# MrOlm/inStrain

Hardware: AMD Instinct MI355X
Metric: Gbp profiled/s (higher is better)
Workload: dtype u32

## Files before the change

### include/instrain_amd.h

```cpp
#ifndef INSTRAIN_AMD_H
#define INSTRAIN_AMD_H

#include <stdint.h>

#ifdef __cplusplus
extern "C" {
#endif

#define ISX_OK 0
#define ISX_ERR_ARG (-1)
#define ISX_ERR_HIP (-2)
#define ISX_ERR_CAPACITY (-3)
#define ISX_ERR_MM_RANGE (-4)
#define ISX_ERR_IO (-5)
#define ISX_ERR_STATE (-6)

#define ISX_ABI_VERSION 5


typedef struct isx_ctx isx_ctx;
typedef struct isx_batch isx_batch;
typedef struct isx_bam isx_bam;
struct isx_bam_params_s;
struct isx_bam_info_s;

typedef struct {
    uint32_t gpos;
    uint16_t mm;
    uint8_t base;
    uint8_t flags;
} isx_obs;

typedef struct {
    int32_t min_cov;
    int32_t min_snp;
    double min_freq;
    int32_t rarefied_coverage;
    int32_t n_mm_bins;
    int32_t enable_linkage;
    int32_t linkage_mode;
    int32_t window;
    uint64_t seed;
    int32_t layout;
    int32_t reserved;
} isx_params;

#define ISX_LAYOUT_WIDE_RECORDS 1
#define ISX_LAYOUT_NO_SHORT_RECORDS 2
#define ISX_LAYOUT_NO_PACKED_COUNTERS 4
#define ISX_LAYOUT_SEG64_RECORDS 8

#define ISX_LAYOUT_MM_ENTRIES 16

#define ISX_LAYOUT_MM_DELTA_RECORDS 32

#define ISX_LAYOUT_NO_STRIPES 64

typedef struct {
    uint32_t gpos;
    uint16_t mm;
    uint16_t flags;
    uint32_t cnt[4];
    float clon;
    float clon_rarefied;
} isx_entry;

typedef struct {
    uint32_t gpos;
    uint16_t mm;
    uint8_t con_base, var_base;
    uint8_t allele_count;
    uint8_t cls;
    uint8_t cryptic;
    uint8_t ref_base;
    uint32_t cnt[4];
} isx_snv;

typedef struct {
    uint32_t gpos_a, gpos_b;
    uint16_t mm;
    uint8_t allele_A, allele_a, allele_B, allele_b;
    uint16_t pad;
    uint32_t total, countAB, countAb, countaB, countab;
    uint32_t pad2;
    double r2, d_prime;
    double r2_normalized, d_prime_normalized;
} isx_ld;

typedef struct {
// ... 205 lines not shown
    const void *lev_mask;
    const void *lev_cov;
    const uint32_t *lev_win_off;
    const isx_rare *lev_clon, *lev_rare;
    const isx_sat *lev_sat;
    int64_t n_lev, n_lev_clon, n_lev_rare, n_lev_sat;
    int32_t lev_mask_bytes, lev_cov_bytes, lev_window, n_lev_windows, lev_min_cov, pad_lev;
    uint64_t rows_checksum;
} isx_pipe_result;

int isx_levels_expand(const isx_pipe_result *r, int32_t host_threads, uint32_t *gpos, uint32_t *mm_cov, float *clon, float *clon_rarefied);

int isx_pipe_create(isx_ctx *ctx, const isx_params *params, const isx_pipe_params *pp, isx_pipe **out);
void isx_pipe_destroy(isx_pipe *p);
int isx_pipe_submit(isx_pipe *p, int64_t n_pos, const uint8_t *ref, int32_t n_splits, const int64_t *split_bounds,
                    int64_t n_obs, const isx_obs *obs, const uint32_t *pair, int64_t *ticket);
int isx_pipe_submit_bam(isx_pipe *p, isx_bam *bam, const struct isx_bam_params_s *bp, const int32_t *refs, int32_t n_refs,
                        const uint8_t *ref, int32_t n_splits, const int64_t *split_bounds, struct isx_bam_info_s *info,
                        int64_t *ticket);
int isx_pipe_collect(isx_pipe *p, int64_t ticket, isx_pipe_result *out);
int isx_pipe_release(isx_pipe *p, int64_t ticket);
int isx_pipe_fetch_entries(isx_pipe *p, int64_t ticket, isx_entry *out);
int isx_pipe_fetch_entries_shrunk(isx_pipe *p, int64_t ticket, uint32_t *gpos, uint32_t *mm_cov, float *clon, float *clon_rarefied);


#define ISX_SEG_BASES 150
#define ISX_SEG_WORDS 15
#define ISX_SEG_SKIP_WORD 0x24924924u
#define ISX_DREC_WORDS 8
#define ISX_DREC_EXC 6
#define ISX_DREC_EXC_FULL 3
#define ISX_DREC_DUAL 0x80000000u
#define ISX_DREC_NO_EXC 0x3FFFFFFFu

typedef struct {
    int64_t n_seg;
    const uint32_t *gpos;
    const uint8_t *len;
    const uint8_t *mm;
    const uint32_t *pair;
    const uint32_t *bases;
} isx_segs;

int isx_batch_create_reads(isx_ctx *ctx, const isx_params *params, int64_t n_pos, const uint8_t *ref, int32_t n_splits,
                           const int64_t *split_bounds, const isx_segs *segs, isx_batch **out);
int isx_pipe_submit_reads(isx_pipe *p, int64_t n_pos, const uint8_t *ref, int32_t n_splits, const int64_t *split_bounds,
                          const isx_segs *segs, int64_t *ticket);

typedef struct isx_wire isx_wire;
int isx_pipe_stage_reads(isx_pipe *p, int64_t n_pos, const uint8_t *ref, int32_t n_splits, const int64_t *split_bounds,
                         const isx_segs *segs, isx_wire **out);
int isx_pipe_submit_wire(isx_pipe *p, const isx_wire *wire, int64_t *ticket);
int64_t isx_wire_bytes(const isx_wire *wire);
void isx_wire_free(isx_wire *wire);
int isx_wire_keep_reference(isx_pipe *p, isx_wire *wire);

#define ISX_PLANE_WORDS 8
typedef struct {
    int64_t n_seg;
    const uint32_t *gpos;
    const uint8_t *len;
    const uint32_t *pair;
    const uint64_t *planes;
    const uint8_t *mm;
} isx_read_planes;

typedef struct {
    const uint8_t *plane2;
    const uint8_t *nplane;
    uint64_t key;
} isx_ref_planes;

int isx_pack_ref_planes(const uint8_t *ref, int64_t n_pos, int32_t host_threads, uint8_t *plane2, uint8_t *nplane, int32_t *has_n);
int isx_planes_from_segs(const isx_segs *segs, int32_t host_threads, uint64_t *planes);
int isx_pack_read_planes(int64_t n_reads, const int64_t *ref_start, const int64_t *clip_lo, const int64_t *clip_hi,
                         const uint32_t *cigar, const int64_t *cigar_off, const char *seq, const uint8_t *qual, const int64_t *seq_off,
                         const uint32_t *pair, int32_t min_base_quality, int64_t cap_seg, uint32_t *seg_gpos,
                         uint8_t *seg_len, uint32_t *seg_pair, uint64_t *seg_planes, int64_t *n_seg);
int isx_pipe_submit_planes(isx_pipe *p, int64_t n_pos, const isx_ref_planes *ref, int32_t n_splits, const int64_t *split_bounds,
                           const isx_read_planes *reads, int64_t *ticket);
int isx_pipe_stage_planes(isx_pipe *p, int64_t n_pos, const isx_ref_planes *ref, int32_t n_splits, const int64_t *split_bounds,
                          const isx_read_planes *reads, isx_wire **out);
int isx_pipe_set_reference_budget(isx_pipe *p, int64_t mib);
int isx_host_register(const void *ptr, int64_t bytes);
int isx_host_unregister(const void *ptr);
int isx_encode_planes(const isx_read_planes *reads, const isx_ref_planes *ref, int64_t n_pos, int32_t host_threads, int32_t slack_groups,
                      int64_t cap_rec, int64_t ring_records, uint32_t *rec, uint32_t *gbase, int64_t *n_rec, int64_t *need_slack);
int isx_encode_planes_mm(const isx_read_planes *reads, const isx_ref_planes *ref, int64_t n_pos, int32_t n_mm_bins, int32_t host_threads, int32_t slack_groups,
                         int64_t cap_rec, int64_t ring_records, uint32_t *rec, uint32_t *gbase, int64_t *n_rec, int64_t *need_slack);

int isx_count_read_segs(int64_t n_reads, const uint32_t *cigar, const int64_t *cigar_off, const int64_t *ref_start,
                        const int64_t *clip_lo, const int64_t *clip_hi, int64_t *n_seg);
int isx_pack_reads(int64_t n_reads, const int64_t *ref_start, const int64_t *clip_lo, const int64_t *clip_hi,
                   const uint32_t *cigar, const int64_t *cigar_off, const char *seq, const uint8_t *qual, const int64_t *seq_off,
                   const uint8_t *mm, const uint32_t *pair, int32_t min_base_quality, int64_t cap_seg, uint32_t *seg_gpos,
                   uint8_t *seg_len, uint8_t *seg_mm, uint32_t *seg_pair, uint32_t *seg_bases, int64_t *n_seg);

int isx_encode_segs(const isx_segs *segs, int64_t n_pos, int32_t n_mm_bins, int32_t host_threads, int64_t cap_rec, uint32_t *rec,
                    uint32_t *gbase, uint32_t *pair_out, int64_t *n_rec);
int64_t isx_seg_records_needed(const uint32_t *gpos, int64_t n_seg, int32_t host_threads);
int isx_encode_segs_ring(const isx_segs *segs, int64_t n_pos, int32_t n_mm_bins, int32_t host_threads, int64_t cap_rec, int64_t ring_records,
                         uint32_t *rec, uint32_t *gbase, uint32_t *pair_out, int64_t *n_rec);

int isx_encode_delta(const isx_segs *segs, const uint8_t *ref, int64_t n_pos, int32_t n_mm_bins, int32_t host_threads, int32_t slack_groups,
                     int64_t cap_rec, int64_t ring_records, uint32_t *rec, uint32_t *gbase, uint32_t *pair_out, int64_t *n_rec, int64_t *need_slack);
int64_t isx_delta_records_needed(const uint32_t *gpos, int64_t n_seg, int32_t host_threads, int32_t slack_groups);

int isx_encode_obs(const isx_obs *obs, const uint32_t *pair, int64_t n_obs, int64_t n_pos, int32_t record_bytes,
                   int32_t host_threads, double slack, int64_t cap_rec, void *rec, uint32_t *gbase, uint32_t *pair_out,
                   int64_t *n_rec, int32_t *passes);
int isx_encode_obs_ring(const isx_obs *obs, const uint32_t *pair, int64_t n_obs, int64_t n_pos, int32_t record_bytes,
                        int32_t host_threads, double slack, int64_t cap_rec, int64_t ring_records, void *rec,
                        uint32_t *gbase, uint32_t *pair_out, int64_t *n_rec, int32_t *passes);

typedef struct {
    int64_t in_off;
    int32_t in_len;
    int32_t out_len;
    int64_t out_off;
} isx_bgzf_block;
int isx_bgzf_index(const uint8_t *image, int64_t n_bytes, int64_t cap_blocks, isx_bgzf_block *blocks, int64_t *n_blocks, int64_t *out_bytes);
int isx_bgzf_inflate_device(isx_ctx *ctx, const uint8_t *image, int64_t n_bytes, const isx_bgzf_block *blocks, int64_t n_blocks,
// ... 68 lines not shown
```

### instrain_amd/_lib.py

```python
import ctypes as C
import os

import numpy as np

_HERE = os.path.dirname(os.path.abspath(__file__))
LIB_PATH = os.path.join(_HERE, "libinstrain_amd.so")
if os.environ.get("ISX_LIB"):
    LIB_PATH = os.path.abspath(os.environ["ISX_LIB"])

BGZF_BLOCK_DT = np.dtype([("in_off", np.int64), ("in_len", np.int32), ("out_len", np.int32), ("out_off", np.int64)])
OBS_DT = np.dtype([("gpos", "<u4"), ("mm", "<u2"), ("base", "u1"), ("flags", "u1")])
ENTRY_DT = np.dtype([("gpos", "<u4"), ("mm", "<u2"), ("flags", "<u2"), ("cnt", "<u4", (4,)), ("clon", "<f4"),
                     ("clon_rarefied", "<f4")])
SNV_DT = np.dtype([("gpos", "<u4"), ("mm", "<u2"), ("con_base", "u1"), ("var_base", "u1"),
                   ("allele_count", "u1"), ("cls", "u1"), ("cryptic", "u1"), ("ref_base", "u1"),
                   ("cnt", "<u4", (4,))])
LD_DT = np.dtype([("gpos_a", "<u4"), ("gpos_b", "<u4"), ("mm", "<u2"), ("allele_A", "u1"), ("allele_a", "u1"),
                  ("allele_B", "u1"), ("allele_b", "u1"), ("pad", "<u2"), ("total", "<u4"), ("countAB", "<u4"),
                  ("countAb", "<u4"), ("countaB", "<u4"), ("countab", "<u4"), ("pad2", "<u4"),
                  ("r2", "<f8"), ("d_prime", "<f8"), ("r2_normalized", "<f8"), ("d_prime_normalized", "<f8")])
AO_DT = np.dtype([("pair", "<u4"), ("gpos", "<u4"), ("order", "<u4"), ("mm", "<u2"), ("base", "u1"), ("pad", "u1")])
assert AO_DT.itemsize == 16
assert OBS_DT.itemsize == 8 and ENTRY_DT.itemsize == 32 and SNV_DT.itemsize == 28 and LD_DT.itemsize == 72


class Params(C.Structure):
    _fields_ = [("min_cov", C.c_int32), ("min_snp", C.c_int32), ("min_freq", C.c_double),
                ("rarefied_coverage", C.c_int32), ("n_mm_bins", C.c_int32), ("enable_linkage", C.c_int32),
                ("linkage_mode", C.c_int32), ("window", C.c_int32), ("seed", C.c_uint64), ("layout", C.c_int32),
                ("reserved", C.c_int32)]


LAYOUT_WIDE_RECORDS, LAYOUT_NO_SHORT_RECORDS, LAYOUT_NO_PACKED_COUNTERS, LAYOUT_SEG64_RECORDS = 1, 2, 4, 8


class PipeParams(C.Structure):
    _fields_ = [("max_pos", C.c_int64), ("max_obs", C.c_int64), ("max_splits", C.c_int32), ("depth", C.c_int32),
                ("host_threads", C.c_int32), ("pin_threads", C.c_int32), ("jump_slack", C.c_double),
                ("want_counts", C.c_int32), ("ring_kib", C.c_int32), ("stage_async", C.c_int32), ("lean_output", C.c_int32),
                ("max_segs", C.c_int64)]


SEG_BASES, SEG_WORDS, SEG_SKIP_WORD = 150, 15, 0x24924924


class Segs(C.Structure):
    _fields_ = [("n_seg", C.c_int64), ("gpos", C.c_void_p), ("len", C.c_void_p), ("mm", C.c_void_p), ("pair", C.c_void_p),
                ("bases", C.c_void_p)]


PLANE_WORDS = 8
LAYOUT_MM_ENTRIES = 16
LAYOUT_MM_DELTA_RECORDS = 32
ABI_VERSION = 5


class ReadPlanes(C.Structure):
    _fields_ = [("n_seg", C.c_int64), ("gpos", C.c_void_p), ("len", C.c_void_p), ("pair", C.c_void_p), ("planes", C.c_void_p), ("mm", C.c_void_p)]


class RefPlanes(C.Structure):
    _fields_ = [("plane2", C.c_void_p), ("nplane", C.c_void_p), ("key", C.c_uint64)]


RARE_DT = np.dtype([("gpos", "<u4"), ("clon_rarefied", "<f4")])
CLON_DT = np.dtype([("gpos", "<u4"), ("clon", "<f4")])
SAT_DT = np.dtype([("gpos", "<u4"), ("coverage", "<u4")])


class Sizes(C.Structure):
    _fields_ = [(n, C.c_int64) for n in ("n_entries", "n_snv", "n_sites", "n_allele_obs", "n_increments",
                                         "n_edges", "n_ld")]


class Timings(C.Structure):
    _fields_ = [(n, C.c_float) for n in ("pileup_ms", "sites_ms", "allele_ms", "group_ms", "incr_ms", "ld_ms",
                                         "total_ms")] + \
               [(n, C.c_int32) for n in ("pileup_blocks", "pileup_threads", "pileup_lds_bytes", "pileup_window")] + \
               [("mfma_ms", C.c_float), ("dense_tiles", C.c_int32), ("dense_macs", C.c_int64), ("dense_bytes", C.c_int64),
                ("record_bytes", C.c_int32), ("pad", C.c_int32)]


class PipeResult(C.Structure):
    _fields_ = [("ticket", C.c_int64), ("n_pos", C.c_int64), ("n_obs", C.c_int64), ("sizes", Sizes),
                ("coverage16", C.c_void_p), ("clon", C.c_void_p), ("rare", C.c_void_p), ("n_rare", C.c_int64),
                ("n_saturated", C.c_int64), ("counts", C.c_void_p), ("clon_rarefied", C.c_void_p), ("snv", C.c_void_p),
# ... 39 lines not shown
COMPARE_LEVEL_DT = np.dtype([("both", "<i8"), ("either", "<i8"), ("mm", "<i4"), ("present_a", "<i4"),
                             ("present_b", "<i4"), ("pad", "<i4"), ("consensus_snps", "<i8"), ("population_snps", "<i8")])
assert COMPARE_LEVEL_DT.itemsize == 48
COMPARE_SNP_DT = np.dtype([("gpos", "<u4"), ("mm", "<u2"), ("consensus_snp", "u1"), ("population_snp", "u1"),
                           ("has_a", "u1"), ("has_b", "u1"), ("con_a", "u1"), ("ref_a", "u1"), ("var_a", "u1"),
                           ("con_b", "u1"), ("ref_b", "u1"), ("var_b", "u1"), ("cnt_a", "<u4", (4,)), ("cnt_b", "<u4", (4,))])
assert COMPARE_SNP_DT.itemsize == 48


GENE_DT = np.dtype([("start", "<i8"), ("end", "<i8"), ("seq_off", "<i8"), ("strand", "<i4"), ("pad", "<i4")])
GENE_COV_DT = np.dtype([("sum_cov", "<u8"), ("nonzero", "<u4"), ("counted", "<u4"), ("sum_clon", "<f8")])
GENE_SNV_COUNT_DT = np.dtype([(n, "<u4") for n in ("divergent", "sns", "sns_n", "sns_s", "snv", "snv_n", "snv_s")])
GENE_MUTATION_DT = np.dtype([("gene", "<i4"), ("k", "<i4"), ("type", "u1"), ("aa_old", "u1"), ("aa_new", "u1"), ("n_genes", "u1"),
                             ("pad", "<u4")])
assert GENE_DT.itemsize == 32 and GENE_COV_DT.itemsize == 24 and GENE_SNV_COUNT_DT.itemsize == 28 and GENE_MUTATION_DT.itemsize == 16
GENE_LEVEL_PRESENT, GENE_COV_ANY, GENE_CLON_ANY = 1, 2, 4


ERR_CAPACITY = -3


class IsxError(RuntimeError):
    def __init__(self, code, msg):
        super().__init__("libinstrain_amd error %d: %s" % (code, msg))
        self.code = code


SYMBOLS = ["isx_last_error", "isx_abi_version", "isx_ctx_create", "isx_ctx_destroy", "isx_ctx_reserve_cus", "isx_set_null_model",
           "isx_batch_create", "isx_batch_create_reads", "isx_batch_destroy", "isx_batch_run", "isx_batch_launch", "isx_batch_wait", "isx_batch_sizes", "isx_batch_timings",
           "isx_batch_fetch_entries", "isx_batch_fetch_dense", "isx_batch_fetch_snv", "isx_batch_fetch_ld", "isx_batch_fetch_allele_obs",
           "isx_batch_summarize", "isx_batch_summarize_genomes", "isx_compare_coverage", "isx_compare_scaffolds", "isx_compare_fetch_snps",
           "isx_genes_create", "isx_genes_destroy", "isx_genes_sites", "isx_batch_profile_genes", "isx_genes_profile_snvs",
           "isx_pipe_create", "isx_pipe_destroy", "isx_pipe_submit", "isx_pipe_submit_reads", "isx_pipe_stage_reads", "isx_pipe_submit_wire", "isx_wire_bytes", "isx_wire_free", "isx_wire_keep_reference", "isx_pipe_submit_bam", "isx_encode_segs", "isx_encode_segs_ring", "isx_seg_records_needed", "isx_encode_delta", "isx_delta_records_needed", "isx_count_read_segs", "isx_pack_reads", "isx_pipe_collect", "isx_pipe_release", "isx_pipe_fetch_entries", "isx_pipe_fetch_entries_shrunk", "isx_levels_expand", "isx_encode_obs", "isx_encode_obs_ring",
           "isx_pack_ref_planes", "isx_planes_from_segs", "isx_pack_read_planes", "isx_pipe_submit_planes", "isx_pipe_stage_planes", "isx_encode_planes", "isx_encode_planes_mm", "isx_pipe_set_reference_budget", "isx_host_register", "isx_host_unregister",
           "isx_bgzf_index", "isx_bgzf_inflate_device", "isx_bgzf_inflate_host", "isx_bgzf_inflate_fast",
           "isx_bam_open", "isx_bam_close", "isx_bam_close_wait", "isx_bam_set_threads", "isx_bam_ref", "isx_bam_set_priority_reads", "isx_bam_scan", "isx_bam_scan_part",
           "isx_bam_insert_sizes", "isx_bam_set_wanted_refs", "isx_bam_pair_keys", "isx_bam_set_cross_names", "isx_bam_filter_insert_sizes", "isx_bam_filter", "isx_bam_set_r2m", "isx_bam_r2m", "isx_bam_drop_names", "isx_bam_batch_pair_names", "isx_bam_set_mm_cap", "isx_bam_mm_levels", "isx_bam_set_mm_levels", "isx_bam_ref_counts",
           "isx_bam_expand_refs", "isx_bam_segment_refs", "isx_bam_copy_segs", "isx_bam_copy_read_planes", "isx_bam_expand_region", "isx_bam_expand", "isx_bam_copy", "isx_bam_view"]

_lib = None


def load():
    global _lib
    if _lib is not None:
        return _lib
    if not os.path.exists(LIB_PATH):
        raise IsxError(-2, "%s not built: run `python -c 'import __graft_entry__ as g; g.build()'` "
                           "(hipcc --offload-arch=gfx950)" % LIB_PATH)
    lib = C.CDLL(LIB_PATH)
    vp, i32, i64 = C.c_void_p, C.c_int32, C.c_int64
    lib.isx_last_error.restype = C.c_char_p
    lib.isx_abi_version.restype = C.c_int
    if lib.isx_abi_version() != ABI_VERSION:
        raise IsxError(-6, "%s has ABI version %d, this package binds version %d: rebuild it (python -c 'import __graft_entry__ as g; g.build()')"
                       % (LIB_PATH, lib.isx_abi_version(), ABI_VERSION))
    lib.isx_ctx_create.argtypes = [C.c_int, C.POINTER(vp)]
    lib.isx_ctx_destroy.argtypes = [vp]
    lib.isx_ctx_reserve_cus.argtypes = [vp, C.c_int]
    lib.isx_bgzf_index.argtypes = [vp, i64, i64, vp, C.POINTER(i64), C.POINTER(i64)]
    lib.isx_bgzf_inflate_device.argtypes = [vp, vp, i64, vp, i64, vp, i64, C.POINTER(C.c_float)]
    lib.isx_bgzf_inflate_host.argtypes = [vp, i64, vp, i64, vp, i64]
    lib.isx_bgzf_inflate_fast.argtypes = [vp, i64, vp, i64, vp, i64]
    lib.isx_ctx_destroy.restype = None
    lib.isx_set_null_model.argtypes = [vp, vp, i64, i32]
    lib.isx_batch_create.argtypes = [vp, C.POINTER(Params), i64, vp, i32, vp, i64, vp, vp, C.POINTER(vp)]
    lib.isx_batch_create_reads.argtypes = [vp, C.POINTER(Params), i64, vp, i32, vp, C.POINTER(Segs), C.POINTER(vp)]
# ... 56 lines not shown
    lib.isx_bam_set_threads.argtypes = [vp, i32]
    lib.isx_bam_set_priority_reads.argtypes = [vp, i64, C.c_char_p, vp]
    lib.isx_bam_scan.argtypes = [vp, C.POINTER(BamInfo)]
    lib.isx_bam_scan_part.argtypes = [vp, i32, i32, C.POINTER(BamInfo)]
    lib.isx_bam_set_wanted_refs.argtypes = [vp, vp, i32]
    lib.isx_bam_insert_sizes.argtypes = [vp, vp, i64, C.POINTER(i64)]
    lib.isx_bam_filter_insert_sizes.argtypes = [vp, vp, i64, C.POINTER(i64)]
    lib.isx_bam_pair_keys.argtypes = [vp, vp, vp, vp, vp, i64, C.POINTER(i64)]
    lib.isx_bam_set_cross_names.argtypes = [vp, i64, vp, vp, vp]
    lib.isx_bam_filter.argtypes = [vp, C.POINTER(BamParams), C.c_double, C.POINTER(BamInfo)]
    lib.isx_bam_set_r2m.argtypes = [vp, i32, i64, C.c_char_p, vp, vp]
    lib.isx_bam_drop_names.argtypes = [vp]
    lib.isx_bam_r2m.argtypes = [vp, i32, C.POINTER(i64), C.POINTER(i64), vp, vp, vp]
    lib.isx_bam_batch_pair_names.argtypes = [vp, C.POINTER(i64), C.POINTER(i64), vp, vp]
    lib.isx_bam_set_mm_cap.argtypes = [vp, i32]
    lib.isx_bam_mm_levels.argtypes = [vp, vp, i32, vp]
    lib.isx_bam_set_mm_levels.argtypes = [vp, vp, i32]
    lib.isx_bam_ref_counts.argtypes = [vp, vp, vp]
    lib.isx_bam_expand_region.argtypes = [vp, C.POINTER(BamParams), i32, i64, i64, C.POINTER(BamInfo)]
    lib.isx_bam_expand_refs.argtypes = [vp, C.POINTER(BamParams), vp, i32, C.POINTER(BamInfo)]
    lib.isx_bam_segment_refs.argtypes = [vp, C.POINTER(BamParams), vp, i32, C.POINTER(BamInfo), C.POINTER(i64)]
    lib.isx_bam_copy_segs.argtypes = [vp, vp, vp, vp, vp, vp, vp, vp]
    lib.isx_bam_copy_read_planes.argtypes = [vp, vp]
    lib.isx_pack_ref_planes.argtypes = [vp, i64, i32, vp, vp, C.POINTER(i32)]
    lib.isx_planes_from_segs.argtypes = [C.POINTER(Segs), i32, vp]
    lib.isx_pack_read_planes.argtypes = [i64, vp, vp, vp, vp, vp, vp, vp, vp, vp, i32, i64, vp, vp, vp, vp, C.POINTER(i64)]
    lib.isx_pipe_submit_planes.argtypes = [vp, i64, C.POINTER(RefPlanes), i32, vp, C.POINTER(ReadPlanes), C.POINTER(i64)]
    lib.isx_pipe_set_reference_budget.argtypes = [vp, i64]
    lib.isx_host_register.argtypes = [vp, i64]
    lib.isx_host_unregister.argtypes = [vp]
    lib.isx_pipe_stage_planes.argtypes = [vp, i64, C.POINTER(RefPlanes), i32, vp, C.POINTER(ReadPlanes), C.POINTER(vp)]
    lib.isx_encode_planes.argtypes = [C.POINTER(ReadPlanes), C.POINTER(RefPlanes), i64, i32, i32, i64, i64, vp, vp, C.POINTER(i64), C.POINTER(i64)]
    lib.isx_encode_planes_mm.argtypes = [C.POINTER(ReadPlanes), C.POINTER(RefPlanes), i64, i32, i32, i32, i64, i64, vp, vp, C.POINTER(i64), C.POINTER(i64)]
    lib.isx_bam_ref.argtypes = [vp, i32, C.POINTER(C.c_char_p), C.POINTER(i64), C.POINTER(i64)]
    lib.isx_bam_copy.argtypes = [vp, vp, vp, vp, vp]
    lib.isx_bam_view.argtypes = [vp, C.POINTER(vp), C.POINTER(vp)]
    _lib = lib
    return lib


def check(rc):
    if rc != 0:
        raise IsxError(rc, load().isx_last_error().decode(errors="replace"))
```

### instrain_amd/csrc/isx_api.hip

```cpp
#include <algorithm>
#include <atomic>
#include <cmath>
#include <chrono>
#include <cstdlib>
#include <cstring>
#include <map>
#include <mutex>
#include <string>
#include <unordered_map>
#include <thread>
#include <type_traits>
#include <vector>
#include <unistd.h>
#include <sys/prctl.h>
#include <time.h>

#include "isx_batch.h"
#include "seg_encode.h"

static thread_local std::string g_err;
void isx_set_error(const std::string &msg) { g_err = msg; }

namespace {
struct BlockCache {
// ... 1215 lines not shown

    PileupArgs a{};
    a.seg = b->d_seg; a.drec = b->d_drec; a.dlt_off = b->dlt_off;
    a.rec = b->d_rec; a.rec32 = b->d_rec32; a.rec16 = b->d_rec16; a.gbase = b->d_gbase; a.win_range = b->d_win; a.ref = b->d_ref; a.ref_packed = b->ref_packed; a.ref_n = b->d_ref_n;
    a.pair = b->d_pair; a.pair_runs = b->d_pair_runs; a.run_index = b->d_run_index; a.n_runs = b->n_runs; a.gpos = b->d_gpos; a.gpos16 = b->d_gpos16; a.chunk_base = b->d_rec32 ? b->d_gbase : b->d_cbase; a.gpos16_shift = b->gpos16_shift; a.thr = b->d_thr; a.lut_n = c->lut_n; a.fallback = c->fallback; a.qcap = b->qcap; a.rqcap = b->rqcap; a.stage_off = b->stage_off;
    a.n_pos = (uint32_t)b->n_pos; a.W = b->W; a.logW = b->logW; a.M = b->M; a.n_win = b->n_win;
    a.min_cov = b->prm.min_cov; a.min_freq = b->prm.min_freq;
#ifdef ISX_TUNING
    if (const char *e = getenv("ISX_DEBUG_MODE")) a.debug_mode = atoi(e);
#endif
    a.counts = b->d_counts; a.clon = b->d_clon; a.clon_r = b->d_clon_r;
    a.min_cov_r = b->prm.rarefied_coverage;
    a.cov16 = b->d_cov16; a.rare = b->d_rare; a.cap_rare = (uint32_t)std::min<size_t>(b->cap_rare, 0xFFFFFFFFu);
    a.cov8 = b->sparse_out && b->cov8_out ? b->d_cov8 : nullptr;
    a.sat = b->d_sat; a.cap_sat = (uint32_t)std::min<size_t>(b->cap_sat, 0xFFFFFFFFu); a.sat_thr = a.cov8 ? 255u : 65535u;
    b->nib_pass = false;
    if (b->sparse_out && b->nib_out && b->lean && b->drec && b->packed && b->M == 1 && b->d_cov_row_win && b->d_cov8 &&
        (size_t)b->n_win <= b->cap_cov_row_win) {
        b->nib_pass = true;
        a.cov4 = b->d_cov8; a.cov_rows = b->d_cov16; a.cov_row_win = b->d_cov_row_win;
        a.cap_cov_rows = (uint32_t)std::min<uint64_t>((uint64_t)(b->cap_pos ? b->cap_pos : b->n_pos), 0xFFFFFFFFu);
        a.cov8 = nullptr; a.cov16 = nullptr; a.sat_thr = 65535u;
    }
    a.clon_list = b->sparse_out ? b->d_clon_list : nullptr; a.cap_clon = (uint32_t)std::min<size_t>(b->cap_clon, 0xFFFFFFFFu);
    if (b->lean && b->sparse_out) {
        if (!b->clon_dense) a.clon = nullptr;
        if (!b->rare_dense && a.rare) a.clon_r = nullptr;
        if (a.cov8) a.cov16 = nullptr;
    }
#ifdef ISX_TUNING
    if (getenv("ISX_NO_COUNTS")) { a.counts = nullptr; if (atoi(getenv("ISX_NO_COUNTS")) > 1) a.clon = nullptr; }
#endif
    a.stripe = (b->drec && b->packed && b->M == 1 && !a.counts && !(b->prm.layout & ISX_LAYOUT_NO_STRIPES)) ? 1 : 0;
    a.seed_lo = (uint32_t)b->prm.seed; a.seed_hi = (uint32_t)(b->prm.seed >> 32);
    a.entries = b->d_entries; a.slab = b->slab; a.cap_ovf = (uint32_t)b->cap_ovf;
    a.ovf0 = (uint64_t)b->n_win * b->slab; a.win_nent = b->d_win_nent;
    if (b->lev_sparse) {
        a.lev_mask = b->d_lev_mask; a.lev_cov = b->d_lev_cov; a.lev_win_off = b->d_lev_win_off;
        a.lev_mask_bytes = b->lev_mask_bytes; a.lev_cov_bytes = b->lev_cov_bytes;
        a.cap_lev = (uint32_t)std::min<size_t>(b->cap_lev, 0xFFFFFFFEu);
        a.sat_thr = b->lev_cov_bytes == 1 ? 255u : 65535u;
        a.clon_list = b->d_clon_list; a.cap_clon = (uint32_t)std::min<size_t>(b->cap_clon, 0xFFFFFFFFu);
        a.cov16 = nullptr; a.cov8 = nullptr; a.clon = nullptr; a.clon_r = nullptr;
    }
    a.slev = b->d_slev; a.cap_slev = (uint32_t)std::min<size_t>(b->cap_slev, 0xFFFFFFFFu);
    a.snv = b->d_snv; a.cap_snv = (uint32_t)std::min<size_t>(b->cap_snv, 0xFFFFFFFFu);
    a.sites = b->d_sites; a.cap_sites = (uint32_t)std::min<size_t>(b->cap_sites, 0xFFFFFFFFu);
    a.ao = b->d_ao; a.cap_ao = (uint32_t)std::min<size_t>(b->cap_ao, 0xFFFFFFFFu); a.enable_linkage = b->prm.enable_linkage;
    a.cursors = b->d_cursors; a.flags = b->d_flags; a.host_state = b->d_host_state;
    memcpy(a.base, b->base, sizeof(a.base));

    if (c->unpublished[b->ps] && c->unpublished[b->ps] != b) {
        isx_batch *u = c->unpublished[b->ps];
        a.pub_cursors = u->d_cursors; a.pub_host_state = u->d_host_state; a.pub_epoch = u->epoch;
        u->publish_enqueued = true;
        c->unpublished[b->ps] = nullptr;
    }
    b->ordered = false;
    if (b->M == 1) {
        auto grow = [&](auto **p, size_t *cap, size_t want, size_t elem) -> hipError_t {
            if (*cap >= want && *p) return hipSuccess;
            if (*p) isx_dev_free(*p);
            *p = nullptr; *cap = 0;
            const hipError_t e = isx_dev_malloc(reinterpret_cast<void **>(p), std::max<size_t>(want, 1) * elem);
            if (e == hipSuccess) *cap = want;
            return e;
// ... 519 lines not shown
```

### instrain_amd/csrc/isx_batch.h

```cpp
#pragma once
#include <vector>

#include "isx_internal.h"
#include "isx_linkage.h"
#include "isx_summary.h"

namespace isxenc { class HostPool; }

struct isx_ctx {
    int device = 0;
    hipStream_t stream = nullptr;
    hipStream_t pstream[2] = {nullptr, nullptr};
    uint32_t side_mask[8] = {0, 0, 0, 0, 0, 0, 0, 0};
    int pass_cus = 256;
    struct isx_batch *unpublished[2] = {nullptr, nullptr};
    unsigned n_created = 0;
    unsigned n_pipes = 0;
    uint8_t *d_lut = nullptr;
    std::vector<int32_t> h_lut;
    int32_t lut_n = 0, fallback = 0;
    void *pin[2] = {nullptr, nullptr};
    hipEvent_t pin_ev[2] = {nullptr, nullptr};
    size_t pin_bytes = 0;
};

hipError_t isx_side_stream_create(isx_ctx *c, hipStream_t *s);

struct isx_batch {
    isx_ctx *ctx = nullptr;
    isx_params prm{};
    int64_t n_pos = 0, n_obs = 0;
    int64_t cap_pos = 0, cap_obs = 0;
    size_t slab_region = 0;
    bool arena = false;
    bool segs = false;
    bool drec = false;
    uint64_t n_rec = 0;
    uint64_t n_pairs = 0;
    int32_t n_splits = 0;
    int W = 0, logW = 0, M = 1, n_win = 0, block = 1024, grid = 0, packed = 0;
    size_t lds = 0;
    uint2 *d_rec = nullptr;
    uint32_t *d_rec32 = nullptr, *d_gbase = nullptr;
    uint16_t *d_rec16 = nullptr;
    uint4 *d_seg = nullptr;
    uint4 *d_drec = nullptr;
    int dlt_off = 0;
    uint32_t *d_pair = nullptr, *d_gpos = nullptr, *d_cbase = nullptr;
    uint2 *d_pair_runs = nullptr;
    uint32_t *d_run_index = nullptr;
    uint32_t n_runs = 0;
    uint16_t *d_gpos16 = nullptr;
    int gpos16_shift = 7;
    uint8_t *d_ref = nullptr;
    int ref_packed = 0;
    uint8_t *d_ref_n = nullptr;
    uint2 *d_win = nullptr;
    uint16_t *d_thr = nullptr;
    int qcap = 1024, rqcap = 0, stage_off = 0;
    bool in_flight = false, publish_enqueued = true, tim_pending = false;
    int ps = 0;
    int64_t *d_bounds = nullptr;
    uint4 *d_counts = nullptr;
    float *d_clon = nullptr;
    float *d_clon_r = nullptr;
    uint16_t *d_cov16 = nullptr;
    uint2 *d_rare = nullptr;
    size_t cap_rare = 0;
    uint32_t n_rare = 0, n_sat = 0;
// ... 82 lines not shown
```

### instrain_amd/csrc/isx_internal.h

```cpp
#pragma once
#include <hip/hip_runtime.h>
#include <stdint.h>
#include <string>

#include "../../include/instrain_amd.h"

#define ISX_PAD32 0x0700FFFFu
#define ISX_GROUP16 512
#define ISX_GROUP 256
#define ISX_CHUNK 1024
#define ISX_DENSE_PAD 8
#define ISX_SEG_GROUP 16
#define ISX_SEG_PAD 32
#define ISX_SEG_LM 16
#define ISX_PK16_MAX_W 3264
#define ISX_PAD 2048
#define ISX_SENTINEL 0xFFFFFFFFu
#define ISX_TAIL_BYTES 65536
#define ISX_TAIL_GROUPS 256

void isx_set_error(const std::string &msg);

hipError_t isx_dev_malloc(void **p, size_t bytes);
void isx_dev_free(void *p);
// ... 155 lines not shown
    uint32_t cap_clon;
    uint2 *rare;
    uint32_t cap_rare;
    int32_t min_cov_r;
    uint32_t seed_lo, seed_hi;
    isx_entry *entries;
    uint32_t slab;
    uint32_t cap_ovf;
    uint64_t ovf0;
    uint32_t *win_nent;
    uint32_t *win_site_base, *win_site_cnt;
    isx_slev *slev;
    uint32_t cap_slev;
    isx_snv *snv;
    uint32_t cap_snv;
    isx_site *sites;
    uint32_t cap_sites;
    isx_ao *ao;
    uint32_t cap_ao;
    int32_t enable_linkage;
    uint32_t *win_rec;
    uint32_t *cursors;
    uint32_t *flags;
    uint32_t base[CUR_N];
    uint32_t *host_state;
    const uint32_t *pub_cursors;
    uint32_t *pub_host_state;
    uint32_t pub_epoch;
    void *lev_mask;
    void *lev_cov;
    uint32_t *lev_win_off;
    uint32_t cap_lev;
    int32_t lev_mask_bytes, lev_cov_bytes;
};

void launch_pileup(const PileupArgs &a, int block, size_t lds, int grid, int packed, hipStream_t s, hipEvent_t ev_start,
                   hipEvent_t ev_stop);
void launch_publish_state(const PileupArgs &a, uint32_t epoch, hipStream_t s);
void launch_win_order(const uint32_t *win_rec, uint32_t *win_out, int n_win, int W, const isx_snv *snv_raw, isx_snv *snv, const isx_site *sites_raw,
                      isx_site *sites, const uint2 *clon_raw, uint2 *clon, const uint2 *rare_raw, uint2 *rare, uint32_t *scan_state, uint32_t epoch, hipStream_t s);
void launch_extract_gpos(const uint2 *rec, const uint32_t *rec32, const uint32_t *gbase, uint32_t *gpos, uint16_t *gpos16,
                         const uint32_t *base16, uint32_t base16_records, uint64_t n_rec, hipStream_t s);
size_t pileup_lds_bytes(int W, int M, int qcap, int rqcap, int linkage, int packed, int block, int segs, int *stage_off, int *dlt_off = nullptr);

struct LinkageBuffers;
```

### instrain_amd/csrc/isx_pileup.hip

```cpp
#include <hip/hip_ext.h>
#include "isx_internal.h"

#pragma clang fp contract(off)

namespace {

typedef uint32_t u32x4 __attribute__((ext_vector_type(4)));

#define THR_LDS 1024

enum { S_NQ = 0, S_ROWS, S_SITES, S_ROW_BASE, S_SITE_BASE, S_ROW_RANK, S_NAO, S_AO_BASE, S_ENT_TOT, S_ENT_BASE, S_SLEV, S_SLEV_BASE, S_NRARE, S_RARE_BASE, S_RARE_RANK,
       S_NCLON, S_CLON_BASE, S_CLON_RANK, S_COVX, S_COVX_BASE, S_N = 20 };
#define S_RNG 128

__device__ __forceinline__ uint32_t cur_add(const PileupArgs &a, int which, uint32_t n)
{
    return atomicAdd(&a.cursors[which], n) - a.base[which];
}

__device__ __forceinline__ void flag_or(const PileupArgs &a, uint32_t bit)
{
    if (atomicOr(a.flags, bit) == 0xFFFFFFFFu) a.flags[3] = 1;
}

// ... 391 lines not shown
        }
        return *reinterpret_cast<const uint32_t *>(a.ref + gpos);
    }
    uint32_t r = 0;
    for (int k = 0; k < 4; k++) r |= (gpos + k < a.n_pos ? (uint32_t)ref_at(a, gpos + k) : 4u) << (8 * k);
    return r;
}

__device__ __forceinline__ void ref4_raw(const PileupArgs &a, uint32_t gpos, uint32_t &raw, uint32_t &rawn)
{
    rawn = 0;
    if (gpos + 3u < a.n_pos) {
        if (a.ref_packed == 2) {
            raw = a.ref[gpos >> 2];
            if (a.ref_n) rawn = a.ref_n[gpos >> 3];
        } else if (a.ref_packed) raw = *reinterpret_cast<const uint16_t *>(a.ref + (gpos >> 1));
        else raw = *reinterpret_cast<const uint32_t *>(a.ref + gpos);
    } else raw = ref4_at(a, gpos);
}
__device__ __forceinline__ uint32_t ref4_expand(const PileupArgs &a, uint32_t gpos, uint32_t raw, uint32_t rawn)
{
    if (gpos + 3u >= a.n_pos) return raw;
    if (a.ref_packed == 2) {
        uint32_t r = (raw & 3u) | ((raw & 0xCu) << 6) | ((raw & 0x30u) << 12) | ((raw & 0xC0u) << 18);
        const uint32_t nb = (rawn >> (gpos & 4u)) & 0xFu;
#pragma unroll
        for (int k = 0; k < 4; k++) r = ((nb >> k) & 1u) ? ((r & ~(0xFFu << (8 * k))) | (4u << (8 * k))) : r;
        return r;
    }
    if (a.ref_packed) return (raw & 0xFu) | ((raw & 0xF0u) << 4) | ((raw & 0xF00u) << 8) | ((raw & 0xF000u) << 12);
    return raw;
}

__device__ __forceinline__ void allele_pass_delta(const PileupArgs &a, uint32_t lo16, uint32_t hi16, uint32_t w0, int W,
                                                  const uint8_t *maskl, uint32_t *slabc, uint32_t ao_base, uint32_t *stage,
                                                  int tid, int nthr)
{
    const int lane = tid & 63;
    uint32_t *st = stage + (tid >> 6) * 128;
    uint32_t *sitebits = stage + (nthr >> 6) * 128;
    for (int p = tid; p < W; p += nthr) {
        const uint64_t bal = __ballot(maskl[p] != 0);
        if (lane == 0) { sitebits[p >> 5] = (uint32_t)bal; sitebits[(p >> 5) + 1] = (uint32_t)(bal >> 32); }
    }
    if (tid < 2) sitebits[(W >> 5) + tid] = 0;
    __syncthreads();
    uint32_t nst = 0;
    auto drain = [&]() {
        __builtin_amdgcn_fence(__ATOMIC_ACQ_REL, "wavefront");
        __builtin_amdgcn_wave_barrier();
        if ((uint32_t)lane < nst) {
            const uint32_t half = st[2 * lane], info = st[2 * lane + 1];
            const uint32_t rel = info & 0xFFFFu;
            const uint32_t slot = atomicAdd(&slabc[rel], 1u);
            isx_ao o;
            o.pair = reinterpret_cast<const uint32_t *>(a.drec)[(info >> 20) & 1u ? ((half | 1u) << 2) + 3u : (half << 2) + 1u];
            o.site = w0 + rel; o.obs_idx = half;
            o.mm = (uint16_t)(info >> 24); o.base = (uint8_t)((info >> 16) & 7u); o.pad = 0;
            a.ao[ao_base + slot] = o;
        }
        __builtin_amdgcn_fence(__ATOMIC_ACQ_REL, "wavefront");
        __builtin_amdgcn_wave_barrier();
    };
    const uint32_t odd = (uint32_t)tid & 1u;
    for (uint32_t i0 = lo16; i0 < hi16; i0 += (uint32_t)nthr) {
        const uint32_t i = i0 + (uint32_t)tid;
        if ((uint32_t)__builtin_amdgcn_readfirstlane(i) >= hi16) break;
        const u32x4 v = __builtin_nontemporal_load(reinterpret_cast<const u32x4 *>(a.drec) + i);
        const uint32_t gb = a.gbase[__builtin_amdgcn_readfirstlane(i >> 6)];
// ... 2 lines not shown
        const uint32_t hdr = dual ? v.x : hdr0;
        const uint32_t len = (hdr >> 16) & 0xFFu;
        const uint32_t w3 = pair_first(v.w);
        const uint32_t e_a = dual ? v.z : w3, e_b = dual ? v.w : ISX_DREC_NO_EXC;
        const int32_t s = (int32_t)(gb + (hdr & 0xFFFFu) - w0);
#pragma unroll
        for (int k = 0; k < 5; k++) {
            const uint32_t c0 = 32u * (uint32_t)k;
            const int32_t r = s + (int32_t)c0;
            const uint32_t skw = dual ? 0u : (k == 0 ? v.y : (k == 1 ? v.z : (k == 2 ? v.x : (k == 3 ? v.y : v.z))));
            const bool mine = dual || (odd != 0u) == (k >= 2);
            uint32_t bits = 0;
            if (len > c0 && mine && (uint32_t)(r + 31) < (uint32_t)(W + 31)) {
                const uint32_t ncol = min(len - c0, 32u);
                const int32_t base = r < 0 ? 0 : r;
                const uint32_t wi = (uint32_t)base >> 5;
                const uint64_t b64 = (uint64_t)sitebits[wi] | ((uint64_t)sitebits[wi + 1] << 32);
                bits = (uint32_t)(b64 >> (base & 31)) << (base - r);
                bits &= ~skw & (ncol == 32u ? 0xFFFFFFFFu : (1u << ncol) - 1u);
            }
            while (__ballot(bits != 0)) {
                const bool has = bits != 0;
                const int j = has ? __ffs((int)bits) - 1 : 0;
                bits &= bits - 1u;
                const uint32_t col = c0 + (uint32_t)j;
                const uint32_t rel = has ? (uint32_t)(r + j) : 0u;
                uint32_t code = 8u;
#pragma unroll
                for (int f = 0; f < 3; f++) {
                    const uint32_t x = (e_a >> (10 * f)) & 0x3FFu, y = (e_b >> (10 * f)) & 0x3FFu;
                    if ((x & 0xFFu) == col) code = x >> 8;
                    if ((y & 0xFFu) == col) code = y >> 8;
                }
                if (has && code == 8u) code = ref_at(a, w0 + rel);
                const bool cand = has && code < 4u && ((maskl[rel] >> code) & 1u);
                const uint64_t bal = __ballot(cand);
                if (bal == 0) continue;
                const uint32_t n = (uint32_t)__popcll(bal);
                if (nst + n > 64u) { drain(); nst = 0; }
                if (cand) {
                    const uint32_t at = nst + __builtin_amdgcn_mbcnt_hi((uint32_t)(bal >> 32), __builtin_amdgcn_mbcnt_lo((uint32_t)bal, 0u));
                    st[2 * at] = dual ? i : (i & ~1u);
                    st[2 * at + 1] = rel | (code << 16) | (dual ? 0u : 1u << 20) | (((hdr >> 24) & 0x7Fu) << 24);
                }
                nst += n;
            }
        }
    }
    if (nst) drain();
}

#ifndef ISX_LB_WAVES
#define ISX_LB_WAVES 8
#endif
#ifdef ISX_TUNING
__device__ unsigned long long g_isx_ts[32 * 16];
extern "C" int isx_debug_read_ts(unsigned long long *out) { return (int)hipMemcpyFromSymbol(out, HIP_SYMBOL(g_isx_ts), sizeof(g_isx_ts)); }
#define ISX_TS(k) do { if ((dbg & 4096) && blockIdx.x == 0 && tid == 0 && ts_w < 32) g_isx_ts[ts_w * 16 + (k)] = wall_clock64(); } while (0)
#else
#define ISX_TS(k) do { } while (0)
#endif
template <bool LINKAGE, int FMT, bool PK16 = false>
__global__ void __launch_bounds__(1024, ISX_LB_WAVES) k_pileup_dense(const PileupArgs a_kernarg)
{
    extern __shared__ __attribute__((aligned(16))) uint32_t lds[];
    typedef const __attribute__((address_space(4))) PileupArgs KernArgs;
    KernArgs *kargs = (KernArgs *)__builtin_amdgcn_kernarg_segment_ptr();
#define a (*(const PileupArgs *)kargs)
    int tid = threadIdx.x;
    const int nthr = blockDim.x;
#define ISX_ARGS_FRESH() asm volatile("" : "+s"(kargs), "+v"(tid))
    publish_previous(a, tid);
    const int W = a.W;
    constexpr bool SEGS = FMT == 64;
    constexpr bool DREC = FMT == 32;
    constexpr bool PKL = DREC && PK16;
    constexpr int NR = PKL ? 2 : 4;
    const int S = W + (SEGS ? ISX_SEG_PAD : ISX_DENSE_PAD);
    uint32_t *cnt = lds + (SEGS ? ISX_SEG_LM : 0);
    uint32_t *queue = lds + NR * S;
    uint32_t *scratch = queue + S;
    uint2 *rngl = reinterpret_cast<uint2 *>(scratch + S_N);
    uint16_t *thr_lds = reinterpret_cast<uint16_t *>(scratch + S_N + S_RNG);
    uint32_t *slabc = scratch + S_N + S_RNG + THR_LDS / 2;
    uint8_t *maskl = reinterpret_cast<uint8_t *>(slabc + W);
    uint32_t *dlt = PKL ? queue : lds + a.dlt_off;
    uint32_t *wtot = lds + a.dlt_off + (PKL ? 0 : S);
    uint8_t *refl = reinterpret_cast<uint8_t *>(wtot + 16);
    auto ld4 = [&](int p, uint32_t *c) {
        if (PKL) {
            const uint32_t x = cnt[p], y = cnt[S + p];
            c[0] = x & 0xFFFFu; c[1] = x >> 16; c[2] = y & 0xFFFFu; c[3] = y >> 16;
        } else { c[0] = cnt[p]; c[1] = cnt[S + p]; c[2] = cnt[2 * S + p]; c[3] = cnt[3 * S + p]; }
    };
    constexpr bool linkage = LINKAGE;
    const int grid = gridDim.x, per = grid >> 3;
    const int slot = (blockIdx.x & 7) * per + (blockIdx.x >> 3);
    constexpr bool COMPACT = FMT != 8;
    const u32x4 *rec4 = reinterpret_cast<const u32x4 *>(SEGS ? (const void *)a.seg : (DREC ? (const void *)a.drec : (FMT == 2 ? (const void *)a.rec16 : (FMT == 4 ? (const void *)a.rec32 : (const void *)a.rec))));
    constexpr int RSH = FMT == 2 ? 3 : (FMT == 4 ? 2 : 1);
    const int dbg = a.debug_mode;
    const bool stripe_k = PKL && a.stripe != 0;

    {
        const int n = min(THR_LDS, a.lut_n);
        for (int i = tid; i < n; i += nthr) thr_lds[i] = a.thr[i];
    }

    u32x4 v[4];
    uint32_t gb[4] = {0, 0, 0, 0};
    bool live[4] = {false, false, false, false};
    uint32_t lo = 0, hi = 0;
    const uint32_t lane16 = (uint32_t)tid;
    auto issue_one = [&](int u, uint32_t i0) {
        const uint32_t j = i0 + tid + u * nthr;
        const uint32_t jw = __builtin_amdgcn_readfirstlane(j);
        if (COMPACT) live[u] = jw < hi;
        if (COMPACT ? jw < hi : j < hi) {
            const uint64_t ub = reinterpret_cast<uint64_t>(rec4 + (i0 + (uint32_t)(u * nthr)));
            typedef __attribute__((address_space(1))) const u32x4 gvec;
            const gvec *sb = reinterpret_cast<const gvec *>(((uint64_t)(uint32_t)__builtin_amdgcn_readfirstlane((uint32_t)(ub >> 32)) << 32) |
// ... 20 lines not shown

#ifdef ISX_TUNING
    int ts_w = -1;
#endif
    for (int w = slot; w < a.n_win; w += grid) {
        const uint32_t w0 = (uint32_t)w * (uint32_t)W;
        const uint32_t cur_lo = lo, cur_hi = hi;
        const bool stripe = stripe_k && (cur_hi - cur_lo) * 8u <= (uint32_t)W;
#ifdef ISX_TUNING
        ++ts_w;
#endif
        ISX_TS(0);
        ISX_ARGS_FRESH();
        if ((win_it & 63) == 0 && tid < 64) {
            const int wn = w + (tid + 1) * grid;
            rngl[tid] = wn < a.n_win ? a.win_range[wn] : make_uint2(0, 0);
        }
        const uint32_t dummy = 4u * (uint32_t)S + (uint32_t)(tid & 63);
#ifdef ISX_TUNING
        uint32_t ablate_acc = 0;
#endif
        {
            uint4 *z = reinterpret_cast<uint4 *>(cnt);
            const int nz = ((NR + (DREC ? 1 : 0)) * S) >> 2;
            for (int i = tid; i < nz; i += nthr) z[i] = make_uint4(0, 0, 0, 0);
            if (DREC && !PKL) {
                uint4 *zd = reinterpret_cast<uint4 *>(dlt);
                for (int i = tid; i < (S >> 2); i += nthr) zd[i] = make_uint4(0, 0, 0, 0);
            }
            if (linkage) {
                uint4 *zm = reinterpret_cast<uint4 *>(maskl);
                for (int i = tid; i < (W >> 4); i += nthr) zm[i] = make_uint4(0, 0, 0, 0);
            }
            if (tid < S_N) scratch[tid] = 0;
        }
        uint32_t ref4 = 0x04040404u, ref4b = 0x04040404u;
        uint32_t ref4n = 0, ref4bn = 0;
        if (PKL) {
            if (4 * tid < W) ref4_raw(a, w0 + 4u * (uint32_t)tid, ref4, ref4n);
            if (4 * (tid + nthr) < W) ref4_raw(a, w0 + 4u * (uint32_t)(tid + nthr), ref4b, ref4bn);
        } else if (DREC && 4 * tid < W) ref4 = ref4_at(a, w0 + 4u * (uint32_t)tid);
        uint8_t ref_raw[2];
#pragma unroll
        for (int it = 0; it < 2; it++) {
            const uint32_t gp = w0 + tid + it * nthr;
            ref_raw[it] = (!PKL && tid + it * nthr < W && gp < a.n_pos) ? ref_at(a, gp) : (uint8_t)4;
        }
        __syncthreads();
        ISX_TS(1);
        ISX_ARGS_FRESH();

        auto count_slot = [&](int u) {
            if (COMPACT && !live[u]) return;
            if (DREC) {
                const uint32_t odd = (uint32_t)tid & 1u;
                const uint32_t hdr0 = pair_first(v[u].x);
                const bool dual = (hdr0 >> 31) != 0u;
                const uint32_t hdr = dual ? v[u].x : hdr0;
                const uint32_t len = (hdr >> 16) & 0xFFu;
                const int32_t s = (int32_t)(gb[u] + (hdr & 0xFFFFu) - w0);
                const uint32_t uW = (uint32_t)W;
#ifdef ISX_TUNING
                if (dbg & 64) { ablate_acc += v[u].x ^ v[u].y ^ v[u].z ^ v[u].w ^ hdr; return; }
#endif
                if ((dual || !odd) && len) {
                    const int32_t hi_c = s + (int32_t)len;
                    if (hi_c > 0 && s < W) {
                        atomicAdd(&dlt[s < 0 ? 0 : s], PKL ? 0x00010000u : 1u);
                        if (hi_c < W) atomicAdd(&dlt[hi_c], PKL ? 0xFFFF0000u : 0xFFFFFFFFu);
                    }
                }
                uint32_t sk[3] = {odd ? v[u].x : v[u].y, odd ? v[u].y : v[u].z, odd ? v[u].z : 0u};
                if (dual) sk[0] = sk[1] = sk[2] = 0;
#ifdef ISX_TUNING
                if (dbg & 8) sk[0] = sk[1] = sk[2] = 0;
#endif
                const int32_t c0 = s + (odd ? 64 : 0);
#pragma unroll
                for (int k = 0; k < 3; k++) {
                    const int32_t r = c0 + 32 * k;
                    uint32_t bits = skip_bits_in_window(sk[k], r, uW);
                    while (__ballot(bits != 0)) {
                        if (bits != 0) atomicAdd(&queue[r + (int32_t)__builtin_ctz(bits)], 1u);
                        bits &= bits - 1u;
                    }
                }
                const uint32_t exw[2] = {dual ? v[u].z : (odd ? ISX_DREC_NO_EXC : v[u].w), dual ? v[u].w : ISX_DREC_NO_EXC};
                const int nf = __ballot(exw[1] != ISX_DREC_NO_EXC) ? 6 : 3;
#pragma unroll
                for (int f = 0; f < 6; f++) {
                    if (f == 3 && nf == 3) break;
                    const uint32_t ex = exw[f / 3];
                    const uint32_t off = (ex >> (10 * (f % 3))) & 0xFFu, code = (ex >> (10 * (f % 3) + 8)) & 3u;
                    const uint32_t rel = (uint32_t)(s + (int32_t)off);
                    if (off < len && rel < uW) {
                        if (PKL) atomicAdd(&cnt[__umul24(code >> 1, (uint32_t)S) + rel], 1u << (16 * (code & 1u)));
                        else atomicAdd(&cnt[__umul24(code, (uint32_t)S) + rel], 1u);
                    }
                }
                return;
            }
            if (SEGS) {
                const uint32_t q = (uint32_t)tid & 3u;
                const uint32_t hdr = quad_first(v[u].x);
                const int32_t r0 = (int32_t)(gb[u] + (hdr & 0xFFFFu) - w0) + (int32_t)(q * 40u) - 10;
                const uint32_t wd[4] = {q ? v[u].x : SEG_SKIPW, v[u].y, v[u].z, v[u].w};
                char *lds_b = reinterpret_cast<char *>(lds);
                const uint32_t S4 = (uint32_t)S * 4u;
#ifdef ISX_TUNING
                if (dbg & 64) { ablate_acc += wd[0] ^ wd[1] ^ wd[2] ^ wd[3] ^ hdr; return; }
#endif
#pragma unroll
                for (int k = 0; k < 4; k++) {
                    const int32_t r = r0 + 10 * k;
                    uint32_t w = wd[k];
                    if (w == SEG_SKIPW || (uint32_t)(r + 9) >= (uint32_t)(W + 9)) continue;
                    const uint32_t m = w & SEG_SKIPW;
                    w &= ~((m >> 1) | (m >> 2));
                    const uint32_t a0 = (uint32_t)(r + ISX_SEG_LM) << 2;
#pragma unroll
                    for (int j = 0; j < 10; j++) {
                        const uint32_t code = __builtin_amdgcn_ubfe(w, 3 * j, 3);
#ifdef ISX_TUNING
                        if (dbg & 8) { ablate_acc += __umul24(code, S4) + a0 + 4u * (uint32_t)j; continue; }
                        if (dbg & 16) { atomicAdd(reinterpret_cast<uint32_t *>(lds_b + ((dummy + (code & 0u)) << 2)), 1u); continue; }
#endif
                        atomicAdd(reinterpret_cast<uint32_t *>(lds_b + (__umul24(code, S4) + a0 + 4u * (uint32_t)j)), 1u);
                    }
                }
                return;
// ... 42 lines not shown
                    atomicAdd(&cnt[(r < (uint32_t)W && bb < 4) ? __umul24(bb, (uint32_t)S) + r : dummy], 1u);
                }
            } else if (FMT == 4) {
                const uint32_t bw = gb[u] - w0;
                const uint32_t x[4] = {v[u].x, v[u].y, v[u].z, v[u].w};
#pragma unroll
                for (int h = 0; h < 4; h++) {
                    const uint32_t r = (x[h] & 0xFFFFu) + bw, bb = __builtin_amdgcn_ubfe(x[h], 24, 3);
                    atomicAdd(&cnt[(r < (uint32_t)W && bb < 4) ? __umul24(bb, (uint32_t)S) + r : dummy], 1u);
                }
            } else {
                const uint32_t g0 = v[u].x, a0 = v[u].y, g1 = v[u].z, a1 = v[u].w;
                const uint32_t r0 = g0 - w0, r1 = g1 - w0;
                const uint32_t b0 = (a0 >> 16) & 0xFFu, b1 = (a1 >> 16) & 0xFFu;
                if (r0 < (uint32_t)W && b0 < 4) atomicAdd(&cnt[b0 * S + r0], 1u);
                if (r1 < (uint32_t)W && b1 < 4) atomicAdd(&cnt[b1 * S + r1], 1u);
            }
        };
        if (DREC) {
            for (uint32_t i0 = lo; i0 < hi; i0 += 2 * nthr) {
                count_slot(0); count_slot(1);
                if (i0 + 2 * nthr < hi) { issue_one(0, i0 + 2 * nthr); issue_one(1, i0 + 2 * nthr); }
            }
        } else
        for (uint32_t i0 = lo; i0 < hi; i0 += 4 * nthr) {
            issue_one(2, i0); issue_one(3, i0);
            count_slot(0); count_slot(1);
            if (i0 + 4 * nthr < hi) { issue_one(0, i0 + 4 * nthr); issue_one(1, i0 + 4 * nthr); }
            count_slot(2); count_slot(3);
        }
#ifdef ISX_TUNING
        if (ablate_acc == 0xDEADBEEFu) cnt[dummy] = ablate_acc;
#endif
        if (PKL) {
            if (4 * tid < W) reinterpret_cast<uint32_t *>(refl)[tid] = ref4_expand(a, w0 + 4u * (uint32_t)tid, ref4, ref4n);
            if (4 * (tid + nthr) < W) reinterpret_cast<uint32_t *>(refl)[tid + nthr] = ref4_expand(a, w0 + 4u * (uint32_t)(tid + nthr), ref4b, ref4bn);
        }
        __syncthreads();
        ISX_TS(2);
        ISX_ARGS_FRESH();

        if (!linkage) { rng_next = rngl[win_it & 63]; prefetch_window(w + grid); }

        if (PKL && !stripe && !(dbg & 16)) {
            const int lane = tid & 63;
            const int PT = ((W + nthr - 1) / nthr) | 1, p0 = tid * PT;
            int32_t sum = 0;
            for (int k = 0; k < PT; k++) if (p0 + k < W) sum += (int32_t)dlt[p0 + k] >> 16;
            const int32_t inc = (int32_t)wave_scan_incl((uint32_t)sum);
            if (lane == 63) wtot[tid >> 6] = (uint32_t)inc;
            __syncthreads();
            ISX_TS(3);
            int32_t run = inc - sum;
            for (int k = 0; k < (tid >> 6); k++) run += (int32_t)wtot[k];
            bool beyond15 = false;
            for (int k = 0; k < PT; k++) {
                const int p = p0 + k;
                if (p >= W) break;
                const uint32_t x = dlt[p], a01 = cnt[p], a23 = cnt[S + p];
                run += (int32_t)x >> 16;
                beyond15 |= run - (int32_t)(x & 0xFFFFu) > 15;
                const uint32_t r = refl[p];
                if (r < 4u) {
                    const uint32_t v = (uint32_t)run - (x & 0xFFFFu) - ((a01 & 0xFFFFu) + (a01 >> 16) + (a23 & 0xFFFFu) + (a23 >> 16));
                    cnt[(r >> 1) * S + p] = ((r >> 1) ? a23 : a01) + (v << (16 * (r & 1u)));
                }
            }
            if (a.cov4 && __ballot(beyond15) && lane == 0) scratch[S_COVX] = 1u;
            __syncthreads();
            ISX_TS(4);
            ISX_ARGS_FRESH();
// ... 385 lines not shown
            const uint32_t e = q < nit ? queue[fl ? (uint32_t)flist[q] : q] : 0u;
            if (!((e >> 14) & 1u)) continue;
            const uint32_t my_row = atomicAdd(&scratch[S_ROW_RANK], 1u);
            const int p = (int)(e & 0x1FFFu);
            const uint32_t gpos = w0 + p;
            uint32_t c[4];
            ld4(p, c);
            const uint32_t total = c[0] + c[1] + c[2] + c[3];
            const int ref_base = PKL ? (int)refl[p] : (int)ref_at(a, gpos);
            const SiteCall sc = call_level(a, nullptr, c, total, ref_base, true);
            isx_snv r;
            r.gpos = gpos; r.mm = 0;
            r.con_base = (uint8_t)sc.snp; r.var_base = (uint8_t)sc.var;
            r.allele_count = (uint8_t)sc.morphia; r.cls = (uint8_t)sc.cls;
            r.cryptic = 0;
            r.ref_base = (uint8_t)ref_base;
            r.cnt[0] = c[0]; r.cnt[1] = c[1]; r.cnt[2] = c[2]; r.cnt[3] = c[3];
            a.snv[row_base + my_row] = r;
            const uint32_t ss = e >> 17;
            if (ss) {
                isx_site st;
                st.gpos = gpos; st.entry_off = row_base + my_row; st.n_levels = 1;
                st.mask = (uint8_t)((1u << sc.snp) | (1u << sc.var)); st.pad = 0;
                a.sites[site_base + ss - 1] = st;
            }
        }
        }
        ISX_TS(8);
        ISX_ARGS_FRESH();
        if (linkage) {
            if (ok && nao) {
                __syncthreads();
                if (SEGS) allele_pass_segs(a, cur_lo, cur_hi, w0, W, maskl, slabc, ao_base, lds + a.stage_off, tid, nthr);
                else if (DREC) allele_pass_delta(a, cur_lo, cur_hi, w0, W, maskl, slabc, ao_base, lds + a.stage_off, tid, nthr);
                else allele_pass(a, cur_lo << (RSH - 1), cur_hi << (RSH - 1), w0, W, maskl, slabc, ao_base, lds + a.stage_off, tid, nthr);
            }
            ISX_TS(9);
            rng_next = rngl[win_it & 63];
            prefetch_window(w + grid);
        }
        win_it++;
        __syncthreads();
        ISX_TS(10);
    }
}
#undef a
#undef ISX_ARGS_FRESH

template <bool PACKED, bool LINKAGE, bool COMPACT, bool SEGS = false, bool SPARSE = false, bool DREC = false>
__global__ void __launch_bounds__(1024) k_pileup_mm(const PileupArgs a_kernarg)
{
    extern __shared__ __attribute__((aligned(16))) uint32_t lds[];
    typedef const __attribute__((address_space(4))) PileupArgs KernArgs;
    KernArgs *kargs = (KernArgs *)__builtin_amdgcn_kernarg_segment_ptr();
#define a (*(const PileupArgs *)kargs)
    int tid = threadIdx.x;
    const int nthr = blockDim.x;
#define ISX_ARGS_FRESH() asm volatile("" : "+s"(kargs), "+v"(tid))
    publish_previous(a, tid);
    const int W = a.W, M = a.M;
#ifdef ISX_TUNING
    int ts_w = -1;
#endif
    const int n_cnt = M * (PACKED ? 2 : 4) * W + (DREC ? M * (PACKED ? 1 : 2) * W : 0);
    const int pres_words = (M + 31) >> 5;
    uint32_t *cnt = lds;
    uint32_t *aux = lds + M * (PACKED ? 2 : 4) * W;
// ... 755 lines not shown
        case 4: launch_one(k_pileup_mm<true, false, true, true, false, true>, a, l); break;
        case 5: launch_one(k_pileup_mm<true, true, true, true, false, true>, a, l); break;
        case 6: launch_one(k_pileup_mm<true, false, true, true, true, true>, a, l); break;
        default: launch_one(k_pileup_mm<true, true, true, true, true, true>, a, l); break;
        }
    } else if (a.M > 1 && a.seg && a.lev_cov) {
        switch (sel & 5) {
        case 0: launch_one(k_pileup_mm<false, false, true, true, true>, a, l); break;
        case 1: launch_one(k_pileup_mm<false, true, true, true, true>, a, l); break;
        case 4: launch_one(k_pileup_mm<true, false, true, true, true>, a, l); break;
        default: launch_one(k_pileup_mm<true, true, true, true, true>, a, l); break;
        }
    } else if (a.M > 1 && a.seg) {
        switch (sel & 5) {
        case 0: launch_one(k_pileup_mm<false, false, true, true>, a, l); break;
        case 1: launch_one(k_pileup_mm<false, true, true, true>, a, l); break;
        case 4: launch_one(k_pileup_mm<true, false, true, true>, a, l); break;
        default: launch_one(k_pileup_mm<true, true, true, true>, a, l); break;
        }
    } else if (a.M > 1) {
        switch (sel) {
        case 0: launch_one(k_pileup_mm<false, false, false>, a, l); break;
        case 1: launch_one(k_pileup_mm<false, true, false>, a, l); break;
        case 2: launch_one(k_pileup_mm<false, false, true>, a, l); break;
        case 3: launch_one(k_pileup_mm<false, true, true>, a, l); break;
        case 4: launch_one(k_pileup_mm<true, false, false>, a, l); break;
        case 5: launch_one(k_pileup_mm<true, true, false>, a, l); break;
        case 6: launch_one(k_pileup_mm<true, false, true>, a, l); break;
        default: launch_one(k_pileup_mm<true, true, true>, a, l); break;
        }
    } else {
        const bool link = a.enable_linkage != 0;
        if (a.seg) { if (link) launch_one(k_pileup_dense<true, 64>, a, l); else launch_one(k_pileup_dense<false, 64>, a, l); return; }
        if (a.drec && packed) { if (link) launch_one(k_pileup_dense<true, 32, true>, a, l); else launch_one(k_pileup_dense<false, 32, true>, a, l); return; }
        if (a.drec) { if (link) launch_one(k_pileup_dense<true, 32>, a, l); else launch_one(k_pileup_dense<false, 32>, a, l); return; }
#ifndef ISX_NO_PK16
        if (a.rec16 && a.W <= ISX_PK16_MAX_W) { if (link) launch_one(k_pileup_dense<true, 2, true>, a, l); else launch_one(k_pileup_dense<false, 2, true>, a, l); }
        else
#endif
        if (a.rec16) { if (link) launch_one(k_pileup_dense<true, 2>, a, l); else launch_one(k_pileup_dense<false, 2>, a, l); }
        else if (a.rec32) { if (link) launch_one(k_pileup_dense<true, 4>, a, l); else launch_one(k_pileup_dense<false, 4>, a, l); }
        else { if (link) launch_one(k_pileup_dense<true, 8>, a, l); else launch_one(k_pileup_dense<false, 8>, a, l); }
    }
}

__global__ void k_extract_gpos(const uint2 *rec, const uint32_t *rec32, const uint32_t *gbase, uint32_t *gpos, uint16_t *gpos16,
                               const uint32_t *base16, uint32_t base16_records, uint64_t n)
{
    const uint64_t i = (uint64_t)blockIdx.x * blockDim.x + threadIdx.x;
    if (i >= n) return;
    uint32_t g;
    if (rec32) { const uint32_t x = rec32[i]; g = x == ISX_PAD32 ? ISX_SENTINEL : gbase[i / ISX_GROUP] + (x & 0xFFFFu); }
    else g = rec[i].x;
    if (gpos16) gpos16[i] = g == ISX_SENTINEL ? (uint16_t)0xFFFFu : (uint16_t)(g - base16[i / base16_records]);
    else gpos[i] = g;
}

void launch_extract_gpos(const uint2 *rec, const uint32_t *rec32, const uint32_t *gbase, uint32_t *gpos, uint16_t *gpos16,
                         const uint32_t *base16, uint32_t base16_records, uint64_t n_rec, hipStream_t s)
{
    hipLaunchKernelGGL(k_extract_gpos, dim3((unsigned)((n_rec + 255) / 256)), dim3(256), 0, s, rec, rec32, gbase, gpos, gpos16,
                       base16, base16_records, n_rec);
}

void launch_win_order(const uint32_t *win_rec, uint32_t *win_out, int n_win, int W, const isx_snv *snv_raw, isx_snv *snv, const isx_site *sites_raw,
                      isx_site *sites, const uint2 *clon_raw, uint2 *clon, const uint2 *rare_raw, uint2 *rare, uint32_t *scan_state, uint32_t epoch, hipStream_t s)
// ... 12 lines not shown
```

### instrain_amd/csrc/isx_pipe.hip

```cpp
#include <atomic>
#include <algorithm>
#include <chrono>
#include <cmath>
#include <condition_variable>
#include <cstring>
#include <deque>
#include <mutex>
#include <memory>
#include <string>
#include <thread>
#include <vector>

#include "bam_front.h"
#include "isx_batch.h"
#include "obs_encode.h"
#include "seg_encode.h"
#include "isx_summary.h"
#include <unordered_map>

namespace {

constexpr size_t ALIGN = 256;
inline size_t up(size_t v, size_t a = ALIGN) { return (v + a - 1) / a * a; }

// ... 69 lines not shown
    std::string err;
    float finish_wait_ms = 0.f;
    float encode_ms = 0.f;
    int encode_passes = 0;
    int64_t h2d_bytes = 0, d2h_bytes = 0;
    uint16_t *d_gpos16 = nullptr;
};

static uint64_t bytes_checksum(const void *p, size_t bytes, uint64_t seed)
{
    const uint8_t *b = static_cast<const uint8_t *>(p);
    uint64_t a[4] = {seed ^ 0x9E3779B97F4A7C15ull, seed + 0xC2B2AE3D27D4EB4Full, seed ^ 0x165667B19E3779F9ull, seed + 0x27D4EB2F165667C5ull};
    const size_t n8 = bytes / 8;
    size_t i = 0;
    for (; i + 4 <= n8; i += 4) {
        uint64_t w[4];
        memcpy(w, b + 8 * i, 32);
        for (int k = 0; k < 4; k++) a[k] = a[k] * 0x100000001B3ull + w[k];
    }
    uint64_t h = (uint64_t)bytes;
    for (; i < n8; i++) { uint64_t w; memcpy(&w, b + 8 * i, 8); h = h * 0x100000001B3ull + w; }
    for (size_t j = n8 * 8; j < bytes; j++) h = h * 0x100000001B3ull + b[j];
    for (int k = 0; k < 4; k++) { h ^= a[k]; h *= 0xFF51AFD7ED558CCDull; h ^= h >> 33; }
    return h;
}

static inline size_t ref2_bytes(int64_t n_pos) { return (((size_t)n_pos + 3) / 4 + 15) & ~(size_t)15; }
static inline size_t refn_bytes(int64_t n_pos) { return (((size_t)n_pos + 7) / 8 + 15) & ~(size_t)15; }

static bool copy_ref_planes(isxenc::HostPool &pool, const isx_ref_planes *rp, int64_t n_pos, uint8_t *plane2, uint8_t *nplane)
{
    const size_t b2 = ((size_t)n_pos + 3) / 4, bn = ((size_t)n_pos + 7) / 8;
    const size_t piece = (size_t)1 << 20;
    const int t2 = (int)((b2 + piece - 1) / piece), tn = rp->nplane ? (int)((bn + piece - 1) / piece) : 0;
    std::atomic<int> any{0};
    pool.run(t2 + tn, [&](int t) {
        if (t < t2) { const size_t a = (size_t)t * piece; memcpy(plane2 + a, rp->plane2 + a, std::min(piece, b2 - a)); return; }
        const size_t a = (size_t)(t - t2) * piece, n = std::min(piece, bn - a);
        const uint8_t *src = rp->nplane + a;
        uint8_t acc = 0;
        for (size_t i = 0; i < n; i++) acc |= src[i];
        memcpy(nplane + a, src, n);
        if (acc) any.store(1, std::memory_order_relaxed);
    });
    return any.load() != 0;
}

static bool plane_any(isxenc::HostPool &pool, const uint8_t *pl, size_t bytes)
{
    const size_t piece = (size_t)1 << 20;
    const int nt = (int)((bytes + piece - 1) / piece);
    std::atomic<int> any{0};
    pool.run(nt, [&](int t) {
        const size_t a = (size_t)t * piece, n = std::min(piece, bytes - a);
        uint64_t acc = 0;
        size_t i = 0;
        for (; i + 8 <= n; i += 8) { uint64_t v; memcpy(&v, pl + a + i, 8); acc |= v; }
        for (; i < n; i++) acc |= pl[a + i];
        if (acc) any.store(1, std::memory_order_relaxed);
    });
    return any.load() != 0;
}

static uint64_t ref_plane_checksum(const uint8_t *plane2, int64_t n_pos)
{
    const size_t words = (((size_t)n_pos + 3) / 4) / 8;
    uint64_t h = 0x9E3779B97F4A7C15ull ^ (uint64_t)n_pos;
// ... 22 lines not shown

int gpu_numa_node(int device)
{
    char bus[64] = {0};
    if (hipDeviceGetPCIBusId(bus, sizeof bus, device) != hipSuccess) return -1;
    std::string id(bus);
    std::transform(id.begin(), id.end(), id.begin(), [](unsigned char ch) { return (char)std::tolower(ch); });
    int node = -1;
    if (FILE *f = fopen(("/sys/bus/pci/devices/" + id + "/numa_node").c_str(), "r")) {
        if (fscanf(f, "%d", &node) != 1) node = -1;
        fclose(f);
    }
    return node;
}

}

struct isx_pipe {
    isx_ctx *ctx = nullptr;
    isx_params prm{};
    isx_pipe_params pp{};
    std::unique_ptr<isxenc::HostPool> pool;
    std::vector<Slot> slots;
    hipStream_t s_h2d = nullptr, s_d2h = nullptr;
    hipStream_t s_h2d2 = nullptr;
    hipStream_t s_fin = nullptr;
    hipStream_t s_fin2 = nullptr;
    int64_t next_ticket = 0;
    int64_t cap_rec = 0;
    int64_t ring_half = 0;
    int rb = 2;
    bool segs = false;
    bool drec = false;
    int64_t dslack = 1;
    uint32_t G = ISX_GROUP16;
    size_t snv_prefix = 0;
    size_t rare_prefix = 0, cap_rare = 0;
    double slack = 0.0;
    std::thread finisher;
    std::thread finisher2;
    std::vector<std::thread> more_finishers;
    std::vector<hipStream_t> extra_fin;
    std::mutex bounce_mu;
    std::mutex mu;
    std::condition_variable cv_work, cv_done;
    std::deque<int64_t> work;
    bool stop = false;
    std::mutex launch_mu;
    uint8_t *bounce[2] = {nullptr, nullptr};
    hipEvent_t bounce_ev[2] = {nullptr, nullptr};
    size_t bounce_bytes = 0;
    std::unique_ptr<isxenc::HostPool> fin_pool;
    struct StageJob {
        int64_t ticket, n_pos;
        const uint8_t *ref;
        std::vector<int64_t> bounds;
        isx_segs segs;
        bool planes = false;
        isx_read_planes reads{};
        isx_ref_planes rp{};
    };
    struct RefEntry { uint8_t *d = nullptr; size_t bytes = 0; int64_t n_pos = 0; bool has_n = false; hipEvent_t ready = nullptr; uint64_t sum = 0; };
    std::unordered_map<uint64_t, RefEntry> ref_cache;
    size_t ref_cache_bytes = 0;
    std::atomic<size_t> ref_cache_budget{(size_t)4096 << 20};
    std::thread stager;
    std::deque<StageJob> stage_q;
    std::condition_variable cv_stage;
    int64_t next_promise = 0;
    bool stage_stop = false;
};

static int bounce_d2h(isx_pipe *p, void *hdst, const void *dsrc, size_t bytes, hipStream_t st)
{
    if (!bytes) return ISX_OK;
    std::lock_guard<std::mutex> bounce_lk(p->bounce_mu);
    const size_t piece = p->bounce_bytes;
    const size_t n_pieces = (bytes + piece - 1) / piece;
    auto issue = [&](size_t k) -> hipError_t {
        const size_t off = k * piece, len = std::min(piece, bytes - off);
        hipError_t e = isx_copy_to_host(p->bounce[k & 1], static_cast<const uint8_t *>(dsrc) + off, len, st);
        return e == hipSuccess ? hipEventRecord(p->bounce_ev[k & 1], st) : e;
    };
    HIP_TRY(issue(0));
    for (size_t k = 0; k < n_pieces; k++) {
        if (k + 1 < n_pieces) HIP_TRY(issue(k + 1));
        HIP_TRY(isx_wait_event(p->bounce_ev[k & 1]));
        const size_t off = k * piece, len = std::min(piece, bytes - off);
        const size_t sub = (size_t)1 << 20;
        const uint8_t *src = p->bounce[k & 1];
        uint8_t *dst = static_cast<uint8_t *>(hdst) + off;
        p->fin_pool->run((int)((len + sub - 1) / sub), [&](int t) {
            const size_t a = (size_t)t * sub;
            memcpy(dst + a, src + a, std::min(sub, len - a));
        });
    }
    return ISX_OK;
}

static void pipe_free(isx_pipe *p)
{
    if (!p) return;
    if (p->stager.joinable()) {
        { std::lock_guard<std::mutex> lk(p->mu); p->stage_stop = true; }
        p->cv_stage.notify_all();
        p->stager.join();
    }
    if (p->finisher.joinable()) {
        { std::lock_guard<std::mutex> lk(p->mu); p->stop = true; }
        p->cv_work.notify_all();
        p->finisher.join();
        if (p->finisher2.joinable()) p->finisher2.join();
        for (auto &t : p->more_finishers) if (t.joinable()) t.join();
    }
    (void)hipSetDevice(p->ctx->device);
    if (p->s_h2d) (void)isx_wait_stream(p->s_h2d);
    if (p->s_h2d2) (void)isx_wait_stream(p->s_h2d2);
    if (p->s_d2h) (void)isx_wait_stream(p->s_d2h);
    if (p->s_fin) (void)isx_wait_stream(p->s_fin);
    if (p->s_fin2) (void)isx_wait_stream(p->s_fin2);
    for (hipStream_t st : p->extra_fin) (void)isx_wait_stream(st);
    for (int i = 0; i < 2; i++) if (p->ctx->pstream[i]) (void)isx_wait_stream(p->ctx->pstream[i]);
    const double t_f0 = now_ms();
    double t_batch = 0, t_dev = 0, t_pin = 0;
    for (Slot &s : p->slots) {
        double t_x = now_ms();
        if (s.b) {
            isx_batch *b = s.b;
            b->d_seg = nullptr; b->d_drec = nullptr;
            b->d_rec = nullptr; b->d_rec32 = nullptr; b->d_rec16 = nullptr; b->d_gbase = nullptr; b->d_pair = nullptr;
            b->d_pair_runs = nullptr; b->d_run_index = nullptr;
            b->d_gpos = nullptr; b->d_gpos16 = nullptr; b->d_cbase = nullptr; b->d_ref = nullptr; b->d_win = nullptr;
            b->d_bounds = nullptr;
            isx_batch_destroy(b);
        }
        t_batch += now_ms() - t_x; t_x = now_ms();
        if (s.sort_temp) isx_dev_free(s.sort_temp);
        if (s.d_gpos16) isx_dev_free(s.d_gpos16);
        if (s.d_in) isx_dev_free(s.d_in);
// ... 400 lines not shown

static int submit_segs_common(isx_pipe *p, int64_t n_pos, const uint8_t *ref, int32_t n_splits, const int64_t *split_bounds,
                              isxenc::SegJob &J, int64_t *ticket, const isx_ref_planes *rp = nullptr);

static void stager_main(isx_pipe *p)
{
    for (;;) {
        isx_pipe::StageJob job;
        {
            std::unique_lock<std::mutex> lk(p->mu);
            p->cv_stage.wait(lk, [&] { return p->stage_stop || !p->stage_q.empty(); });
            if (p->stage_q.empty()) return;
            job = std::move(p->stage_q.front());
            p->stage_q.pop_front();
        }
        isxenc::SegJob J;
        if (job.planes) { J.in2 = job.reads; J.n_seg = job.reads.n_seg; }
        else { J.in = job.segs; J.n_seg = job.segs.n_seg; }
        int64_t got = -1;
        const int rc = submit_segs_common(p, job.n_pos, job.ref, (int32_t)job.bounds.size() - 1, job.bounds.data(), J, &got, job.planes ? &job.rp : nullptr);
        if (rc != ISX_OK) {
            Slot &s = p->slots[(size_t)(job.ticket % (int64_t)p->slots.size())];
            std::string err(isx_last_error());
            std::lock_guard<std::mutex> lk(p->mu);
            s.ticket = job.ticket; s.rc = rc; s.err.swap(err); s.state = 2;
            p->next_ticket = job.ticket + 1;
        }
        p->cv_done.notify_all();
    }
}

static void drain_stager(isx_pipe *p)
{
    if (!p->stager.joinable()) return;
    std::unique_lock<std::mutex> lk(p->mu);
    p->cv_done.wait(lk, [&] { return p->next_ticket == p->next_promise; });
}

extern "C" {

int isx_pipe_create(isx_ctx *c, const isx_params *prm, const isx_pipe_params *pp, isx_pipe **out)
{
    if (!c || !prm || !pp || !out) { isx_set_error("isx_pipe_create: bad argument"); return ISX_ERR_ARG; }
    *out = nullptr;
    if (!c->d_lut) { isx_set_error("isx_pipe_create: call isx_set_null_model first"); return ISX_ERR_STATE; }
    if (prm->n_mm_bins < 1 || prm->n_mm_bins > 128) { isx_set_error("n_mm_bins must be in [1, 128]"); return ISX_ERR_ARG; }
    if (pp->max_pos <= 0 || pp->max_obs < 0 || pp->max_splits <= 0 || pp->depth < 1 || pp->depth > 64 || pp->max_segs < 0) {
        isx_set_error("isx_pipe_create: max_pos > 0, max_obs >= 0, max_segs >= 0, max_splits > 0, 1 <= depth <= 64");
        return ISX_ERR_ARG;
    }
    if (pp->max_segs > 0 && prm->linkage_mode == 2) { isx_set_error("isx_pipe_create: the dense MFMA linkage path takes observation batches only"); return ISX_ERR_ARG; }
    if (pp->max_pos >= (int64_t)0xFFFF0000ll) { isx_set_error("flat position space must be < 2^32 - 65536"); return ISX_ERR_ARG; }
    if (prm->window && (prm->window < 64 || (prm->window & 63) || prm->window > 8192)) { isx_set_error("window must be a multiple of 64 in [64, 8192]"); return ISX_ERR_ARG; }
    if (prm->layout & ISX_LAYOUT_WIDE_RECORDS) { isx_set_error("a pipe streams 2- / 4-byte records only"); return ISX_ERR_ARG; }
    HIP_TRY(hipSetDevice(c->device));
    isx_pipe *p = new isx_pipe();
    p->ctx = c; p->prm = *prm; p->pp = *pp;
    p->segs = pp->max_segs > 0;
    p->drec = p->segs && !(prm->layout & ISX_LAYOUT_SEG64_RECORDS) && (prm->n_mm_bins == 1 || (prm->layout & ISX_LAYOUT_MM_DELTA_RECORDS));
    p->rb = p->segs ? (p->drec ? 32 : 64) : ((prm->n_mm_bins == 1 && !(prm->layout & ISX_LAYOUT_NO_SHORT_RECORDS)) ? 2 : 4);
    p->G = p->segs ? (p->drec ? ISX_DREC_GROUP : ISX_SEG_GROUP) : (p->rb == 2 ? ISX_GROUP16 : ISX_GROUP);
    const double js = pp->jump_slack > 0 ? pp->jump_slack : 0.25;
    if (p->segs) {
        if (p->pp.max_obs == 0) p->pp.max_obs = pp->max_segs * ISX_SEG_BASES;
        const uint64_t G = p->G;
        const uint64_t groups = (uint64_t)(pp->max_segs + G - 1) / G + (uint64_t)pp->max_segs / 4096 * (p->drec ? 3 : 1) + (uint64_t)pp->max_pos / 65536 +
                                (uint64_t)pp->max_splits + 64 + (uint64_t)((double)pp->max_segs / G * js * (p->drec ? 1.0 : 0.25));
        p->cap_rec = (int64_t)(groups * G);
        if ((uint64_t)p->cap_rec >= (1ull << 26)) { delete p; isx_set_error("more than 2^26 segment records in one batch (4 GiB of records)"); return ISX_ERR_ARG; }
        const size_t rec_bytes = (size_t)p->cap_rec * (size_t)p->rb;
        size_t ring = 0;
        if (pp->ring_kib > 0) ring = (size_t)pp->ring_kib << 10;
        else if (pp->ring_kib == 0 && rec_bytes > ((size_t)(pp->depth == 1 ? 96 : 256) << 20)) ring = (size_t)64 << 20;
        if (ring && ring < rec_bytes) {
            p->ring_half = (int64_t)(ring / 2 / (size_t)p->rb) / (int64_t)p->G * (int64_t)p->G;
            if (p->ring_half * p->rb < (4096 + 16 * ISX_SEG_GROUP) * 64) { delete p; isx_set_error("isx_pipe_create: ring_kib too small for a read-level pipe (at least 1024)"); return ISX_ERR_ARG; }
        }
    } else {
        const uint64_t want = (uint64_t)((double)pp->max_obs * (1.0 + js)) + 4 * ISX_PAD;
        p->cap_rec = (int64_t)((want + ISX_PAD - 1) / ISX_PAD * ISX_PAD);
        if ((uint64_t)p->cap_rec >= 0xFFFFFFFFull) { delete p; isx_set_error("more than 2^32 records in one batch"); return ISX_ERR_ARG; }
    }
    if (!p->segs) {
        const size_t rec_bytes = (size_t)p->cap_rec * p->rb;
        size_t ring = 0;
        if (pp->ring_kib > 0) ring = (size_t)pp->ring_kib << 10;
        else if (pp->ring_kib == 0 && pp->depth == 1 && rec_bytes > ((size_t)128 << 20)) ring = (size_t)64 << 20;
        else if (pp->ring_kib == 0 && rec_bytes > ((size_t)512 << 20)) ring = (size_t)256 << 20;
        if (ring && ring < rec_bytes) {
            p->ring_half = (int64_t)(ring / 2 / p->rb) / ISX_PAD * ISX_PAD;
            if (p->ring_half < 2 * ISX_PAD) { delete p; isx_set_error("isx_pipe_create: ring_kib too small (at least 32)"); return ISX_ERR_ARG; }
        }
// ... 118 lines not shown
        if (p->pp.want_counts) {
            HIP_TRY(isx_copy_to_host(s.h_out + s.o_counts, b->d_counts, (size_t)n_pos * 16, p->s_d2h));
            s.d2h_bytes += (int64_t)n_pos * 16;
            if (p->prm.rarefied_coverage > 0) {
                HIP_TRY(isx_copy_to_host(s.h_out + s.o_clonr, b->d_clon_r, (size_t)n_pos * 4, p->s_d2h));
                s.d2h_bytes += (int64_t)n_pos * 4;
            }
        }
    }
    HIP_TRY(hipEventRecord(s.ev_d2h1, p->s_d2h));
    launch_lk.unlock();
    {
        std::lock_guard<std::mutex> lk(p->mu);
        s.ticket = p->next_ticket++;
        if (p->next_promise < p->next_ticket) p->next_promise = p->next_ticket;
        s.state = 1; s.rc = ISX_OK;
        *ticket = s.ticket;
        p->work.push_back(s.ticket);
    }
    p->cv_work.notify_one();
    return ISX_OK;
}


static int check_capacity(const isx_pipe *p, const char *who, int64_t n_pos, int64_t n_items, int64_t max_items, int32_t n_splits)
{
    if (n_pos > p->pp.max_pos || n_items > max_items || n_splits > p->pp.max_splits) {
        isx_set_error(std::string(who) + ": batch larger than the pipe was created for");
        return ISX_ERR_CAPACITY;
    }
    return ISX_OK;
}

static int slot_acquire(isx_pipe *p, const char *who, Slot **out)
{
    Slot &s = p->slots[(size_t)(p->next_ticket % (int64_t)p->slots.size())];
    {
        std::lock_guard<std::mutex> lk(p->mu);
        if (s.state != 0) { isx_set_error(std::string(who) + ": every slot is in use (collect + release the oldest batch first)"); return ISX_ERR_STATE; }
    }
    HIP_TRY(hipSetDevice(p->ctx->device));
    *out = &s;
    return ISX_OK;
}

static int queue_for_stager(isx_pipe *p, isx_pipe::StageJob &&job, const char *who, int64_t *ticket)
{
    const int rc = check_capacity(p, who, job.n_pos, job.planes ? job.reads.n_seg : job.segs.n_seg, p->pp.max_segs, (int32_t)job.bounds.size() - 1);
    if (rc != ISX_OK) return rc;
    {
        std::lock_guard<std::mutex> lk(p->mu);
        const int64_t t = p->next_promise, n = (int64_t)p->slots.size();
        const Slot &s = p->slots[(size_t)(t % n)];
        if (t - n >= p->next_ticket || s.state != 0) { isx_set_error(std::string(who) + ": every slot is in use (collect + release the oldest batch first)"); return ISX_ERR_STATE; }
        job.ticket = t;
        p->next_promise = t + 1;
        *ticket = t;
        p->stage_q.push_back(std::move(job));
    }
    p->cv_stage.notify_one();
    return ISX_OK;
}

struct RingFeed { hipError_t err = hipSuccess; size_t bytes = 0; };

static int ring_feed_install(isx_pipe *p, Slot &s, RingFeed &r, int64_t &ring_groups, std::function<void(int)> &wave_begin,
                             std::function<void(int, int64_t, int64_t)> &wave_flush)
{
    if (p->ring_half <= 0) return ISX_OK;
    HIP_TRY(hipEventRecord(s.ev_h2d0, H2D(p, s)));
    const size_t half_bytes = (size_t)p->ring_half * (size_t)p->rb, grp_bytes = (size_t)p->G * (size_t)p->rb;
    uint8_t *d_rec = s.d_in + s.off_rec;
    ring_groups = p->ring_half / (int64_t)p->G;
    wave_begin = [&s, &r](int h) {
        if (s.ring_busy[h]) { const hipError_t e = isx_wait_event(s.ev_ring[h]); if (e != hipSuccess && r.err == hipSuccess) r.err = e; s.ring_busy[h] = false; }
// ... 63 lines not shown
    if (p->segs) {
        b->d_seg = p->drec ? nullptr : reinterpret_cast<uint4 *>(rec);
        b->d_drec = p->drec ? reinterpret_cast<uint4 *>(rec) : nullptr;
        b->d_pair = linkage && !p->drec ? reinterpret_cast<uint32_t *>(s.d_in + s.off_pairs) : nullptr;
        b->d_pair_runs = nullptr; b->d_run_index = nullptr; b->n_runs = 0;
    } else {
        b->d_pair = nullptr;
        b->d_pair_runs = linkage ? s.d_runs : nullptr;
        b->d_run_index = linkage ? reinterpret_cast<uint32_t *>(s.d_in + s.off_ridx) : nullptr;
        b->d_gpos16 = s.d_gpos16; b->gpos16_shift = 5;
    }
}

static void ref_cache_insert(isx_pipe *p, Slot &s, const isx_ref_planes *rp, int64_t n_pos)
{
    const size_t rb_all = ref2_bytes(n_pos) + (s.ref_has_n ? refn_bytes(n_pos) : 0);
    if (p->ref_cache_bytes + rb_all > p->ref_cache_budget.load(std::memory_order_relaxed)) return;
    isx_pipe::RefEntry e;
    bool ok = isx_dev_malloc(reinterpret_cast<void **>(&e.d), rb_all + 64) == hipSuccess && hipEventCreateWithFlags(&e.ready, hipEventDisableTiming) == hipSuccess;
    ok = ok && hipMemcpyAsync(e.d, s.d_in + s.off_ref, rb_all, hipMemcpyDeviceToDevice, H2D(p, s)) == hipSuccess && hipEventRecord(e.ready, H2D(p, s)) == hipSuccess;
    if (ok) {
        e.bytes = rb_all; e.n_pos = n_pos; e.has_n = s.ref_has_n; e.sum = ref_plane_checksum(rp->plane2, n_pos);
        p->ref_cache_bytes += rb_all;
        p->ref_cache.emplace(rp->key, e);
    } else {
        if (e.d) isx_dev_free(e.d);
        if (e.ready) (void)hipEventDestroy(e.ready);
        (void)hipGetLastError();
    }
}

struct RefStage {
    bool early = false;
    uint8_t *resident = nullptr;
    double host_ms = 0.0;
};

static int stage_reference(isx_pipe *p, Slot &s, int64_t n_pos, const uint8_t *ref, const isx_ref_planes *rp, isxenc::SegJob &J, RefStage *out)
{
    const bool ring = p->ring_half > 0;
    const double t_r = now_ms();
    const size_t b2 = ((size_t)n_pos + 3) / 4, bn = ((size_t)n_pos + 7) / 8;
    hipStream_t st = H2D(p, s);

    const auto hit = rp && rp->key ? p->ref_cache.find(rp->key) : p->ref_cache.end();
    if (hit != p->ref_cache.end()) {
        const isx_pipe::RefEntry &e = hit->second;
        if (e.n_pos != n_pos || e.has_n != (rp->nplane != nullptr && e.has_n) || e.sum != ref_plane_checksum(rp->plane2, n_pos)) {
            isx_set_error("isx_pipe_submit_planes: the reference key stands for other planes (positions / non-ACGT plane / content differ)");
            return ISX_ERR_ARG;
        }
        s.ref_has_n = e.has_n;
        J.ref2 = rp->plane2; J.refn = e.has_n ? rp->nplane : nullptr;
        out->resident = e.d;
        HIP_TRY(hipStreamWaitEvent(st, e.ready, 0));
        if (!ring) HIP_TRY(hipEventRecord(s.ev_h2d0, st));
        HIP_TRY(hipEventRecord(s.ev_h2da, st));
        out->early = true;
        out->host_ms = now_ms() - t_r;
        return ISX_OK;
    }

    const bool first_trip = rp && rp->key && p->ref_cache_budget.load(std::memory_order_relaxed) > 0;
    if (rp && !first_trip && isx_host_is_registered(rp->plane2, b2) && (!rp->nplane || isx_host_is_registered(rp->nplane, bn))) {
        const bool any_n = rp->nplane && plane_any(*p->pool, rp->nplane, bn);
        s.ref_has_n = any_n;
        J.ref2 = rp->plane2; J.refn = any_n ? rp->nplane : nullptr;
        out->host_ms = now_ms() - t_r;
        if (!ring) HIP_TRY(hipEventRecord(s.ev_h2d0, st));
        HIP_TRY(hipMemcpyAsync(s.d_in + s.off_ref, rp->plane2, b2, hipMemcpyHostToDevice, st));
        if (any_n) HIP_TRY(hipMemcpyAsync(s.d_in + s.off_ref + ref2_bytes(n_pos), rp->nplane, bn, hipMemcpyHostToDevice, st));
        if (!ring) HIP_TRY(hipEventRecord(s.ev_h2da, st));
        out->early = true;
        return ISX_OK;
    }

    uint8_t *h2 = s.h_in + s.off_ref, *hn = h2 + ref2_bytes(n_pos);
    s.ref_has_n = rp ? copy_ref_planes(*p->pool, rp, n_pos, h2, hn) : isxenc::pack_ref_planes(*p->pool, ref, n_pos, h2, hn);
    J.ref2 = h2; J.refn = s.ref_has_n ? hn : nullptr;
    out->host_ms = now_ms() - t_r;
    static const bool late_dma = getenv("ISX_PIPE_LATE_DMA") != nullptr;
    if (late_dma) return ISX_OK;
    if (!ring) HIP_TRY(hipEventRecord(s.ev_h2d0, st));
    HIP_TRY(hipMemcpyAsync(s.d_in + s.off_ref, h2, ref2_bytes(n_pos) + (s.ref_has_n ? refn_bytes(n_pos) : 0), hipMemcpyHostToDevice, st));
    if (!ring) HIP_TRY(hipEventRecord(s.ev_h2da, st));
    out->early = true;
    if (rp && rp->key) ref_cache_insert(p, s, rp, n_pos);
    return ISX_OK;
}

static int submit_common(isx_pipe *p, int64_t n_pos, const uint8_t *ref, int32_t n_splits, const int64_t *split_bounds,
                         int64_t n_obs, isxenc::EncodeJob &J, int64_t *ticket)
{
    static const char who[] = "isx_pipe_submit";
    int rc;
    if ((rc = check_capacity(p, who, n_pos, n_obs, p->pp.max_obs, n_splits)) != ISX_OK) return rc;
    if ((rc = check_split_bounds(n_pos, n_splits, split_bounds)) != ISX_OK) return rc;
    Slot *slot = nullptr;
    if ((rc = slot_acquire(p, who, &slot)) != ISX_OK) return rc;
    Slot &s = *slot;
    isx_batch *b = s.b;
    const bool linkage = p->prm.enable_linkage != 0;

    const double t0 = now_ms();
    const bool ring = p->ring_half > 0;
    uint8_t *d_rec = s.d_in + s.off_rec;
    RingFeed feed;
    J.n_obs = n_obs; J.n_pos = n_pos; J.record_bytes = p->rb;
    J.rec = s.h_in + s.off_rec; J.gbase = reinterpret_cast<uint32_t *>(s.h_in + s.off_gbase);
    J.pair_out = nullptr;
    J.cmin = s.cmin.data(); J.cmax = s.cmax.data(); J.cany = s.cany.data();
    J.cap_rec = p->cap_rec;
    if ((rc = ring_feed_install(p, s, feed, J.ring_groups, J.wave_begin, J.wave_flush)) != ISX_OK) return rc;
    int erc = 0;
    for (int attempt = 0;; attempt++) {
        if (linkage) {
            J.runs_out = s.h_runs; J.cap_runs = s.cap_runs;
            J.run_index_out = reinterpret_cast<uint32_t *>(s.h_in + s.off_ridx);
        }
        J.slack = p->slack;
        feed.bytes = 0;
        erc = isxenc::encode_obs(*p->pool, J);
        if (erc != isxenc::ENC_OK || !linkage || J.n_runs <= s.cap_runs || attempt == 1) break;
        HIP_TRY(isx_wait_stream(H2D(p, s)));
        host_block_free(s.h_runs, s.runs_pinned); s.h_runs = nullptr;
        isx_dev_free(s.d_runs); s.d_runs = nullptr;
        s.cap_runs = J.n_runs + J.n_runs / 4 + 4096;
        { const int hrc = host_block_alloc(reinterpret_cast<void **>(&s.h_runs), s.cap_runs * sizeof(isxenc::PairRun), s.runs_pinned); if (hrc != ISX_OK) return hrc; }
        HIP_TRY(isx_dev_malloc(reinterpret_cast<void **>(&s.d_runs), s.cap_runs * sizeof(uint2)));
    }
    const double t_enc = now_ms();
    if (feed.err != hipSuccess) { isx_set_error(std::string("isx_pipe_submit: staging ring: ") + hipGetErrorString(feed.err)); return ISX_ERR_HIP; }
    if (erc == isxenc::ENC_CAPACITY) { isx_set_error("isx_pipe_submit: the stream jumps too often for the pipe's record capacity (raise jump_slack)"); return ISX_ERR_CAPACITY; }
    if (erc == isxenc::ENC_MM_RANGE) { isx_set_error("an observation has mm >= 256"); return ISX_ERR_MM_RANGE; }
// ... 51 lines not shown

static int encode_reads(isx_pipe *p, Slot &s, isxenc::SegJob &J, bool planes_in, RingFeed &feed)
{
    s.encode_passes = 1;
    if (!p->drec) return isxenc::encode_segs(*p->pool, J);
    std::vector<int64_t> exact;
    for (int attempt = 0;; attempt++) {
        J.slack_groups = p->dslack;
        J.task_groups = exact.empty() ? nullptr : exact.data();
        feed.bytes = 0;
        const int erc = planes_in ? isxenc::encode_planes(*p->pool, J) : isxenc::encode_delta(*p->pool, J);
        if (erc != isxenc::SEG_CAPACITY || J.need_slack <= p->dslack || attempt != 0) return erc;
        exact = J.task_need;
        int64_t tot = 0;
        for (int64_t v : exact) tot += v;
        const int64_t n_t = (int64_t)exact.size(), base_tot = J.n_rec / ISX_DREC_GROUP - n_t * p->dslack;
        p->dslack = std::max<int64_t>(p->dslack, 1 + (tot - base_tot + n_t - 1) / std::max<int64_t>(n_t, 1));
        s.encode_passes = 2;
    }
}

static int submit_segs_common(isx_pipe *p, int64_t n_pos, const uint8_t *ref, int32_t n_splits, const int64_t *split_bounds,
                              isxenc::SegJob &J, int64_t *ticket, const isx_ref_planes *rp)
{
    static const char who[] = "isx_pipe_submit_reads";
    const bool planes_in = J.in2.planes != nullptr || (bool)J.produce_planes || (J.n_seg == 0 && rp != nullptr);
    int rc;
    if ((rc = check_capacity(p, who, n_pos, J.n_seg, p->pp.max_segs, n_splits)) != ISX_OK) return rc;
    if ((rc = check_split_bounds(n_pos, n_splits, split_bounds)) != ISX_OK) return rc;
    Slot *slot = nullptr;
    if ((rc = slot_acquire(p, who, &slot)) != ISX_OK) return rc;
    Slot &s = *slot;
    isx_batch *b = s.b;
    const bool linkage = p->prm.enable_linkage != 0;

    const double t0 = now_ms();
    J.n_pos = n_pos; J.n_mm_bins = b->M;
    J.rec = reinterpret_cast<uint32_t *>(s.h_in + s.off_rec);
    J.gbase = reinterpret_cast<uint32_t *>(s.h_in + s.off_gbase);
    J.pair_out = linkage && !p->drec ? reinterpret_cast<uint32_t *>(s.h_in + s.off_pairs) : nullptr;
    J.cmin = s.cmin.data(); J.cmax = s.cmax.data(); J.cany = s.cany.data();
    J.cap_rec = p->cap_rec;
    const bool ring = p->ring_half > 0;
    RingFeed feed;
    if ((rc = ring_feed_install(p, s, feed, J.ring_groups, J.wave_begin, J.wave_flush)) != ISX_OK) return rc;
    RefStage rs;
    if (planes_in) {
        if (!p->drec) { isx_set_error("bit-plane reads need a pipe whose batches travel as reference-delta records (one mm bin, or ISX_LAYOUT_MM_DELTA_RECORDS)"); return ISX_ERR_STATE; }
        if ((rc = stage_reference(p, s, n_pos, ref, rp, J, &rs)) != ISX_OK) return rc;
    }
    if (p->drec) J.ref = ref;
    const int erc = encode_reads(p, s, J, planes_in, feed);
    const double t_enc = now_ms();
    if (feed.err != hipSuccess) { isx_set_error(std::string("isx_pipe_submit_reads: staging ring: ") + hipGetErrorString(feed.err)); return ISX_ERR_HIP; }
    if ((rc = seg_status_error(erc, "isx_pipe_submit_reads: the stream jumps too often for the pipe's record capacity (raise jump_slack)", ISX_ERR_CAPACITY)) != ISX_OK) return rc;
    if (J.n_bases > p->pp.max_obs) { isx_set_error("isx_pipe_submit_reads: more bases than the pipe's max_obs"); return ISX_ERR_CAPACITY; }
    bool early_rec = false;
    if (rs.early && !ring) {
        const size_t gb_bytes0 = (size_t)(J.n_rec / (int64_t)p->G) * sizeof(uint32_t), rec_bytes0 = (size_t)J.n_rec * (size_t)p->rb;
        HIP_TRY(hipEventRecord(s.ev_h2db, H2D(p, s)));
        if (s.off_pairs == s.off_rec && s.off_ridx == s.off_rec && s.off_rec - s.off_gbase < ((size_t)2 << 20)) {
            HIP_TRY(hipMemcpyAsync(s.d_in + s.off_gbase, s.h_in + s.off_gbase, (s.off_rec - s.off_gbase) + rec_bytes0, hipMemcpyHostToDevice, H2D(p, s)));
        } else {
            HIP_TRY(hipMemcpyAsync(s.d_in + s.off_gbase, s.h_in + s.off_gbase, gb_bytes0, hipMemcpyHostToDevice, H2D(p, s)));
            HIP_TRY(hipMemcpyAsync(s.d_in + s.off_rec, s.h_in + s.off_rec, rec_bytes0, hipMemcpyHostToDevice, H2D(p, s)));
        }
        early_rec = true;
    }
    if (!planes_in) s.ref_has_n = isxenc::pack_ref_planes(*p->pool, ref, n_pos, s.h_in + s.off_ref, s.h_in + s.off_ref + ref2_bytes(n_pos));
    const double t_ref = now_ms();
    memcpy(s.h_in + s.off_bounds, split_bounds, (size_t)(n_splits + 1) * sizeof(int64_t));

    b->n_pos = n_pos; b->n_obs = J.n_bases; b->n_splits = n_splits; b->n_rec = (uint64_t)J.n_rec;
    b->n_pairs = (uint64_t)J.max_pair + 1;
    if ((rc = slot_choose_windows(p, s, p->G, true)) != ISX_OK) return rc;
    if ((rc = slot_shape_pass(p, s)) != ISX_OK) return rc;
    slot_bind_inputs(p, s, rs.resident);
    s.encode_ms = (float)(now_ms() - t0);
    if (pipe_timing)
        fprintf(stderr, "[isx_pipe_submit_reads] records %.2f ms, reference %.2f ms, bounds + windows %.2f ms; %lld segments, %lld records%s\n",
                t_enc - t0 - rs.host_ms, t_ref - t_enc + rs.host_ms, now_ms() - t_ref, (long long)J.n_seg, (long long)J.n_rec, planes_in ? " (bit planes)" : "");
    const double t_q0 = now_ms();

    if (!ring && !rs.early) HIP_TRY(hipEventRecord(s.ev_h2d0, H2D(p, s)));
    const size_t ref_bytes = ref2_bytes(n_pos) + (s.ref_has_n ? refn_bytes(n_pos) : 0);
    const size_t head = (size_t)(n_splits + 1) * sizeof(int64_t) + s.win.size() * sizeof(uint2) + ref_bytes;
    const size_t gb_bytes = (size_t)(b->n_rec / p->G) * sizeof(uint32_t), rec_bytes = (size_t)b->n_rec * (size_t)p->rb;
    if (s.off_win - s.off_bounds < ((size_t)1 << 20)) {
        HIP_TRY(hipMemcpyAsync(s.d_in + s.off_bounds, s.h_in + s.off_bounds, (s.off_win - s.off_bounds) + s.win.size() * sizeof(uint2), hipMemcpyHostToDevice, H2D(p, s)));
    } else {
        HIP_TRY(hipMemcpyAsync(s.d_in + s.off_bounds, s.h_in + s.off_bounds, (size_t)(n_splits + 1) * sizeof(int64_t), hipMemcpyHostToDevice, H2D(p, s)));
        HIP_TRY(hipMemcpyAsync(s.d_in + s.off_win, s.h_in + s.off_win, s.win.size() * sizeof(uint2), hipMemcpyHostToDevice, H2D(p, s)));
    }
    if (!rs.early) HIP_TRY(hipMemcpyAsync(s.d_in + s.off_ref, s.h_in + s.off_ref, ref_bytes, hipMemcpyHostToDevice, H2D(p, s)));
    if (!early_rec) HIP_TRY(hipMemcpyAsync(s.d_in + s.off_gbase, s.h_in + s.off_gbase, gb_bytes, hipMemcpyHostToDevice, H2D(p, s)));
    if (ring) { if (feed.bytes != rec_bytes) { isx_set_error("internal: the staging ring did not carry the whole stream"); return ISX_ERR_STATE; } }
    else if (!early_rec) HIP_TRY(hipMemcpyAsync(s.d_in + s.off_rec, s.h_in + s.off_rec, rec_bytes, hipMemcpyHostToDevice, H2D(p, s)));
    s.h2d_bytes = (int64_t)(head + gb_bytes + rec_bytes) - (rs.resident ? (int64_t)ref_bytes : 0);
    if (linkage && !p->drec) {
        HIP_TRY(hipMemcpyAsync(s.d_in + s.off_pairs, s.h_in + s.off_pairs, (size_t)b->n_rec * sizeof(uint32_t), hipMemcpyHostToDevice, H2D(p, s)));
        s.h2d_bytes += (int64_t)b->n_rec * 4;
    }
    HIP_TRY(hipEventRecord(s.ev_h2d1, H2D(p, s)));
    s.h2d_split = early_rec;
    const double t_q1 = now_ms();
    rc = enqueue_pass(p, s, n_pos, ticket);
    if (pipe_timing) fprintf(stderr, "[isx_pipe_submit_reads] copy-in queue %.2f ms, pass + copy-out queue %.2f ms\n", t_q1 - t_q0, now_ms() - t_q1);
    return rc;
}

struct isx_wire {
    isx_pipe *pipe = nullptr;
    uint8_t *h = nullptr;
    size_t bytes = 0;
    size_t o_bounds = 0, o_win = 0, o_ref = 0, o_gbase = 0, o_pairs = 0, o_rec = 0;
    size_t bounds_bytes = 0, win_bytes = 0, ref_bytes = 0, gbase_bytes = 0, pairs_bytes = 0, rec_bytes = 0;
    int64_t n_pos = 0, n_bases = 0, n_rec = 0, n_seg = 0;
    int32_t n_splits = 0;
    uint64_t n_pairs = 0;
    int W = 0, packed = 0;
    bool ref_has_n = false;
    float stage_ms = 0.f;
    int encode_passes = 1;
    uint8_t *d_ref = nullptr;
    int device = 0;
};

static int stage_common(isx_pipe *p, int64_t n_pos, const uint8_t *ref, const isx_ref_planes *rp, int32_t n_splits, const int64_t *split_bounds,
                        const isx_segs *segs, const isx_read_planes *reads, isx_wire **out)
{
    isx_segs as_segs{};
    if (reads) { as_segs.n_seg = reads->n_seg; as_segs.gpos = reads->gpos; as_segs.len = reads->len; as_segs.pair = reads->pair; segs = &as_segs; }
    *out = nullptr;
    if (!p->segs) { isx_set_error("isx_pipe_stage_reads: not a read-level pipe (isx_pipe_params.max_segs == 0)"); return ISX_ERR_STATE; }
    const bool linkage = p->prm.enable_linkage != 0;
    if (linkage && segs->n_seg && !segs->pair) { isx_set_error("linkage needs the pair array"); return ISX_ERR_ARG; }
    int rc;
    if ((rc = check_capacity(p, "isx_pipe_stage_reads", n_pos, segs->n_seg, p->pp.max_segs, n_splits)) != ISX_OK) return rc;
    if ((rc = check_split_bounds(n_pos, n_splits, split_bounds)) != ISX_OK) return rc;
    HIP_TRY(hipSetDevice(p->ctx->device));
    const double t0 = now_ms();
    std::unique_ptr<isx_wire, void (*)(isx_wire *)> w(new isx_wire(), isx_wire_free);
    w->pipe = p; w->n_pos = n_pos; w->n_splits = n_splits; w->n_seg = segs->n_seg;
    const isx_batch *b0 = p->slots[0].b;
    const int M = b0->M;
    const size_t G = p->G, rb = (size_t)p->rb;
    auto up = [](size_t v) { return (v + 255) & ~(size_t)255; };
    isxenc::SegJob J;
    std::vector<uint32_t> cmin, cmax;
    std::vector<uint8_t> cany;
    std::vector<int64_t> exact;
    for (int attempt = 0;; attempt++) {
        int64_t cap = p->drec ? isxenc::delta_groups_needed(*p->pool, segs->gpos, segs->n_seg, p->dslack) * ISX_DREC_GROUP
                              : isxenc::seg_groups_needed(*p->pool, segs->gpos, segs->n_seg) * ISX_SEG_GROUP;
        if (!exact.empty()) { cap = 0; for (int64_t v : exact) cap += std::max<int64_t>(v, 1) * ISX_DREC_GROUP; }
        if (cap > p->cap_rec) { isx_set_error("isx_pipe_stage_reads: the stream needs more records than the pipe's capacity (raise jump_slack)"); return ISX_ERR_CAPACITY; }
        const size_t n_groups = (size_t)cap / G;
        w->bounds_bytes = (size_t)(n_splits + 1) * sizeof(int64_t);
        w->ref_bytes = ref2_bytes(n_pos) + refn_bytes(n_pos);
        const size_t win_cap = ((size_t)n_pos / 64 + 2) * sizeof(uint2);
        size_t o = 0;
        w->o_bounds = o; o = up(o + w->bounds_bytes);
        w->o_win = o; o = up(o + win_cap);
        w->o_ref = o; o = up(o + w->ref_bytes);
        w->o_gbase = o; o = up(o + n_groups * sizeof(uint32_t));
        w->o_pairs = o; if (linkage && !p->drec) o = up(o + (size_t)cap * sizeof(uint32_t));
        w->o_rec = o; o = up(o + (size_t)cap * rb);
        if (w->h) { isx_pin_free(w->h); w->h = nullptr; }
        HIP_TRY(isx_pin_malloc(reinterpret_cast<void **>(&w->h), o));
        w->bytes = o;
        cmin.assign(n_groups + 2, 0xFFFFFFFFu); cmax.assign(n_groups + 2, 0u); cany.assign(n_groups + 2, 0);
        J = isxenc::SegJob();
        J.n_seg = segs->n_seg; J.n_pos = n_pos; J.n_mm_bins = M;
        if (reads) { J.in2 = *reads; if (!linkage) J.in2.pair = nullptr; }
        else { J.in = *segs; if (!linkage) J.in.pair = nullptr; }
        J.rec = reinterpret_cast<uint32_t *>(w->h + w->o_rec);
        J.gbase = reinterpret_cast<uint32_t *>(w->h + w->o_gbase);
        J.pair_out = linkage && !p->drec ? reinterpret_cast<uint32_t *>(w->h + w->o_pairs) : nullptr;
        J.cmin = cmin.data(); J.cmax = cmax.data(); J.cany = cany.data();
        J.cap_rec = cap;
        int erc;
        if (reads) {
            uint8_t *h2 = w->h + w->o_ref, *hn = h2 + ref2_bytes(n_pos);
            w->ref_has_n = rp ? copy_ref_planes(*p->pool, rp, n_pos, h2, hn) : isxenc::pack_ref_planes(*p->pool, ref, n_pos, h2, hn);
            J.ref2 = h2; J.refn = w->ref_has_n ? hn : nullptr;
        }
        if (p->drec) {
            J.ref = ref; J.slack_groups = p->dslack;
            J.task_groups = exact.empty() ? nullptr : exact.data();
            erc = reads ? isxenc::encode_planes(*p->pool, J) : isxenc::encode_delta(*p->pool, J);
            if (erc == isxenc::SEG_CAPACITY && J.need_slack > p->dslack && attempt == 0) { exact = J.task_need; w->encode_passes = 2; continue; }
        } else erc = isxenc::encode_segs(*p->pool, J);
        if ((rc = seg_status_error(erc, "isx_pipe_stage_reads: the stream does not fit the record capacity", ISX_ERR_CAPACITY)) != ISX_OK) return rc;
        break;
    }
    if (J.n_bases > p->pp.max_obs) { isx_set_error("isx_pipe_stage_reads: more bases than the pipe's max_obs"); return ISX_ERR_CAPACITY; }
    w->n_rec = J.n_rec; w->n_bases = J.n_bases; w->n_pairs = (uint64_t)J.max_pair + 1;
    w->gbase_bytes = (size_t)(J.n_rec / (int64_t)G) * sizeof(uint32_t);
    w->rec_bytes = (size_t)J.n_rec * rb;
    w->pairs_bytes = linkage && !p->drec ? (size_t)J.n_rec * sizeof(uint32_t) : 0;
    if (!reads) w->ref_has_n = isxenc::pack_ref_planes(*p->pool, ref, n_pos, w->h + w->o_ref, w->h + w->o_ref + ref2_bytes(n_pos));
    if (!w->ref_has_n) w->ref_bytes = ref2_bytes(n_pos);
    memcpy(w->h + w->o_bounds, split_bounds, w->bounds_bytes);
    {
        std::vector<uint2> win;
        std::vector<uint32_t> dir_pmax, dir_smin;
        DirThreads mt{*p->pool, dir_pmax, dir_smin};
        w->W = choose_windows(b0, n_pos, ChunkDir{cmin.data(), cmax.data(), cany.data(), (uint64_t)J.n_rec / G, (uint32_t)G}, &mt, win, &w->packed);
        w->win_bytes = win.size() * sizeof(uint2);
        if (w->win_bytes > ((size_t)n_pos / 64 + 2) * sizeof(uint2) || win.size() > (size_t)p->pp.max_pos / 64 + 2) { isx_set_error("internal: window directory larger than its region"); return ISX_ERR_STATE; }
        memcpy(w->h + w->o_win, win.data(), w->win_bytes);
    }
    w->stage_ms = (float)(now_ms() - t0);
    *out = w.release();
    return ISX_OK;
}

int isx_pipe_stage_reads(isx_pipe *p, int64_t n_pos, const uint8_t *ref, int32_t n_splits, const int64_t *split_bounds,
                         const isx_segs *segs, isx_wire **out)
{
    if (!p || !ref || !split_bounds || !out || n_pos <= 0 || n_splits <= 0 || !segs || segs->n_seg < 0 ||
        (segs->n_seg && (!segs->gpos || !segs->len || !segs->bases))) {
        isx_set_error("isx_pipe_stage_reads: bad argument");
        return ISX_ERR_ARG;
    }
    return stage_common(p, n_pos, ref, nullptr, n_splits, split_bounds, segs, nullptr, out);
}

int isx_pipe_stage_planes(isx_pipe *p, int64_t n_pos, const isx_ref_planes *ref, int32_t n_splits, const int64_t *split_bounds,
                          const isx_read_planes *reads, isx_wire **out)
{
    if (!p || !ref || !ref->plane2 || !split_bounds || !out || n_pos <= 0 || n_splits <= 0 || !reads || reads->n_seg < 0 ||
        (reads->n_seg && (!reads->gpos || !reads->len || !reads->planes))) {
        isx_set_error("isx_pipe_stage_planes: bad argument");
        return ISX_ERR_ARG;
    }
    if (!p->drec) { isx_set_error("isx_pipe_stage_planes: bit-plane reads need a read-level pipe with one mm bin or ISX_LAYOUT_MM_DELTA_RECORDS"); return ISX_ERR_STATE; }
    return stage_common(p, n_pos, nullptr, ref, n_splits, split_bounds, nullptr, reads, out);
}

void isx_wire_free(isx_wire *w)
{
    if (!w) return;
    if (w->h) isx_pin_free(w->h);
    if (w->d_ref) { (void)hipSetDevice(w->device); isx_dev_free(w->d_ref); }
    delete w;
}

int isx_wire_keep_reference(isx_pipe *p, isx_wire *w)
{
    if (!p || !w || w->pipe != p) { isx_set_error("isx_wire_keep_reference: bad argument"); return ISX_ERR_ARG; }
    if (w->d_ref || !w->ref_bytes) return ISX_OK;
    isx_ctx *c = p->ctx;
    HIP_TRY(hipSetDevice(c->device));
    uint8_t *d = nullptr;
    HIP_TRY(isx_dev_malloc(reinterpret_cast<void **>(&d), w->ref_bytes + 64));
    const hipError_t e = hipMemcpy(d, w->h + w->o_ref, w->ref_bytes, hipMemcpyHostToDevice);
    if (e != hipSuccess) { isx_dev_free(d); isx_set_error(std::string("isx_wire_keep_reference: ") + hipGetErrorString(e)); return ISX_ERR_HIP; }
    w->d_ref = d; w->device = c->device;
    return ISX_OK;
}

int64_t isx_wire_bytes(const isx_wire *w) { return w ? (int64_t)(w->bounds_bytes + w->win_bytes + (w->d_ref ? 0 : w->ref_bytes) + w->gbase_bytes + w->pairs_bytes + w->rec_bytes) : 0; }

int isx_pipe_submit_wire(isx_pipe *p, const isx_wire *w, int64_t *ticket)
{
    if (!p || !w || !ticket) { isx_set_error("isx_pipe_submit_wire: bad argument"); return ISX_ERR_ARG; }
    if (w->pipe != p) { isx_set_error("isx_pipe_submit_wire: the batch was staged for another pipe"); return ISX_ERR_ARG; }
    drain_stager(p);
    Slot *slot = nullptr;
    int rc = slot_acquire(p, "isx_pipe_submit_wire", &slot);
    if (rc != ISX_OK) return rc;
    Slot &s = *slot;
    isx_batch *b = s.b;
    const double t0 = now_ms();
    b->n_pos = w->n_pos; b->n_obs = w->n_bases; b->n_splits = w->n_splits; b->n_rec = (uint64_t)w->n_rec;
    b->n_pairs = w->n_pairs;
    s.ref_has_n = w->ref_has_n;
    b->packed = w->packed; b->W = w->W;
    b->n_win = (int)(w->win_bytes / sizeof(uint2));
    if ((rc = slot_shape_pass(p, s)) != ISX_OK) return rc;
    slot_bind_inputs(p, s, w->d_ref);
    HIP_TRY(hipEventRecord(s.ev_h2d0, H2D(p, s)));
    HIP_TRY(hipMemcpyAsync(s.d_in + s.off_bounds, w->h + w->o_bounds, w->bounds_bytes, hipMemcpyHostToDevice, H2D(p, s)));
    HIP_TRY(hipMemcpyAsync(s.d_in + s.off_win, w->h + w->o_win, w->win_bytes, hipMemcpyHostToDevice, H2D(p, s)));
    if (!w->d_ref) HIP_TRY(hipMemcpyAsync(s.d_in + s.off_ref, w->h + w->o_ref, w->ref_bytes, hipMemcpyHostToDevice, H2D(p, s)));
    HIP_TRY(hipMemcpyAsync(s.d_in + s.off_gbase, w->h + w->o_gbase, w->gbase_bytes, hipMemcpyHostToDevice, H2D(p, s)));
    if (w->pairs_bytes) HIP_TRY(hipMemcpyAsync(s.d_in + s.off_pairs, w->h + w->o_pairs, w->pairs_bytes, hipMemcpyHostToDevice, H2D(p, s)));
    HIP_TRY(hipMemcpyAsync(s.d_in + s.off_rec, w->h + w->o_rec, w->rec_bytes, hipMemcpyHostToDevice, H2D(p, s)));
    HIP_TRY(hipEventRecord(s.ev_h2d1, H2D(p, s)));
    s.h2d_split = false;
    s.h2d_bytes = isx_wire_bytes(w);
    s.encode_ms = (float)(now_ms() - t0);
    s.encode_passes = 0;
    return enqueue_pass(p, s, w->n_pos, ticket);
}

int isx_pipe_submit_reads(isx_pipe *p, int64_t n_pos, const uint8_t *ref, int32_t n_splits, const int64_t *split_bounds,
                          const isx_segs *segs, int64_t *ticket)
{
    if (!p || !ref || !split_bounds || !ticket || n_pos <= 0 || n_splits <= 0 || !segs || segs->n_seg < 0 ||
        (segs->n_seg && (!segs->gpos || !segs->len || !segs->bases))) {
        isx_set_error("isx_pipe_submit_reads: bad argument");
        return ISX_ERR_ARG;
    }
    if (!p->segs) { isx_set_error("isx_pipe_submit_reads: not a read-level pipe (isx_pipe_params.max_segs == 0)"); return ISX_ERR_STATE; }
    if (p->prm.enable_linkage && segs->n_seg && !segs->pair) { isx_set_error("linkage needs the pair array"); return ISX_ERR_ARG; }
    if (p->stager.joinable()) {
        isx_pipe::StageJob job;
        job.n_pos = n_pos; job.ref = ref; job.segs = *segs;
        if (!p->prm.enable_linkage) job.segs.pair = nullptr;
        job.bounds.assign(split_bounds, split_bounds + n_splits + 1);
        return queue_for_stager(p, std::move(job), "isx_pipe_submit_reads", ticket);
    }
    isxenc::SegJob J;
    J.in = *segs; J.n_seg = segs->n_seg;
    if (!p->prm.enable_linkage) J.in.pair = nullptr;
    return submit_segs_common(p, n_pos, ref, n_splits, split_bounds, J, ticket);
}
// ... 298 lines not shown
```

### instrain_amd/csrc/seg_encode.cpp

```cpp
#include "seg_encode.h"

#include <immintrin.h>

#include <algorithm>
#include <atomic>
#include <cstdlib>
#include <cstring>
#include <string>
#include <vector>

void isx_set_error(const std::string &msg);

namespace isxenc {

namespace {

constexpr int64_t TASK = 4096;
constexpr uint32_t SPAN = 65535u;

inline int64_t count_groups(const uint32_t *gpos, int64_t a, int64_t e, int64_t group = ISX_SEG_GROUP)
{
    int64_t n = 0;
    for (int64_t i = a; i < e;) {
        uint32_t lo = gpos[i], hi = gpos[i];
// ... 998 lines not shown
int isx_pack_ref_planes(const uint8_t *ref, int64_t n_pos, int32_t host_threads, uint8_t *plane2, uint8_t *nplane, int32_t *has_n)
{
    if (!ref || n_pos <= 0 || !plane2 || !nplane) { isx_set_error("isx_pack_ref_planes: bad argument"); return ISX_ERR_ARG; }
    isxenc::HostPool pool(std::max(1, host_threads), -1, false);
    const bool any = isxenc::pack_ref_planes(pool, ref, n_pos, plane2, nplane);
    if (has_n) *has_n = any ? 1 : 0;
    return ISX_OK;
}

int isx_planes_from_segs(const isx_segs *segs, int32_t host_threads, uint64_t *planes)
{
    if (!segs || segs->n_seg < 0 || (segs->n_seg && (!segs->len || !segs->bases || !planes))) { isx_set_error("isx_planes_from_segs: bad argument"); return ISX_ERR_ARG; }
    const int64_t n = segs->n_seg, piece = 8192;
    std::atomic<bool> bad{false};
    isxenc::HostPool pool(std::max(1, host_threads), -1, false);
    pool.run((int)((n + piece - 1) / piece), [&](int t) {
        const int64_t a = (int64_t)t * piece, e = std::min<int64_t>(n, a + piece);
        for (int64_t i = a; i < e; i++) {
            const uint32_t L = segs->len[i];
            if (L == 0 || L > ISX_SEG_BASES) { bad.store(true); return; }
            isxenc::planes_from_words(segs->bases + (size_t)i * ISX_SEG_WORDS, L, planes + (size_t)i * ISX_PLANE_WORDS);
        }
    });
    if (bad.load()) { isx_set_error("a segment's length is not in [1, 150]"); return ISX_ERR_ARG; }
    return ISX_OK;
}

int isx_encode_planes(const isx_read_planes *reads, const isx_ref_planes *ref, int64_t n_pos, int32_t host_threads, int32_t slack_groups,
                      int64_t cap_rec, int64_t ring_records, uint32_t *rec, uint32_t *gbase, int64_t *n_rec, int64_t *need_slack)
{
    return isx_encode_planes_mm(reads, ref, n_pos, 1, host_threads, slack_groups, cap_rec, ring_records, rec, gbase, n_rec, need_slack);
}

int isx_encode_planes_mm(const isx_read_planes *reads, const isx_ref_planes *ref, int64_t n_pos, int32_t n_mm_bins, int32_t host_threads, int32_t slack_groups,
                         int64_t cap_rec, int64_t ring_records, uint32_t *rec, uint32_t *gbase, int64_t *n_rec, int64_t *need_slack)
{
    if (n_mm_bins < 1 || n_mm_bins > 128) { isx_set_error("isx_encode_planes: n_mm_bins must be in [1, 128]"); return ISX_ERR_ARG; }
    if (!reads || !ref || !ref->plane2 || !rec || !gbase || !n_rec || reads->n_seg < 0 || cap_rec < ISX_DREC_GROUP || (cap_rec % ISX_DREC_GROUP) || n_pos <= 0 ||
        (reads->n_seg && (!reads->gpos || !reads->len || !reads->planes)) || ring_records < 0 ||
        (ring_records % (2 * ISX_DREC_GROUP)) || slack_groups < 0) {
        isx_set_error("isx_encode_planes: bad argument");
        return ISX_ERR_ARG;
    }
    std::vector<uint32_t> ring;
    isxenc::HostPool pool(std::max(1, host_threads), -1, false);
    std::vector<uint32_t> cmin((size_t)(cap_rec / ISX_DREC_GROUP)), cmax(cmin.size());
    std::vector<uint8_t> cany(cmin.size());
    isxenc::SegJob J;
    J.in2 = *reads; J.n_seg = reads->n_seg; J.n_pos = n_pos; J.n_mm_bins = n_mm_bins;
    J.ref2 = ref->plane2; J.refn = ref->nplane; J.slack_groups = std::max(1, slack_groups);
    J.rec = rec; J.gbase = gbase; J.pair_out = nullptr;
    J.cmin = cmin.data(); J.cmax = cmax.data(); J.cany = cany.data(); J.cap_rec = cap_rec;
    if (ring_records) {
        const int64_t half = ring_records / 2;
        ring.assign((size_t)ring_records * ISX_DREC_WORDS + 16, 0xABABABABu);
        uint32_t *r0 = reinterpret_cast<uint32_t *>((reinterpret_cast<uintptr_t>(ring.data()) + 63) & ~(uintptr_t)63);
        J.rec = r0;
        J.ring_groups = half / ISX_DREC_GROUP;
        J.wave_begin = [](int) {};
        J.wave_flush = [&, r0](int h, int64_t g0, int64_t g1) {
            const size_t gw = (size_t)ISX_DREC_GROUP * ISX_DREC_WORDS;
            memcpy(rec + (size_t)g0 * gw, r0 + (size_t)h * half * ISX_DREC_WORDS, (size_t)(g1 - g0) * gw * 4);
            std::fill_n(r0 + (size_t)h * half * ISX_DREC_WORDS, (size_t)half * ISX_DREC_WORDS, 0xABABABABu);
        };
    }
    const int rc = isxenc::encode_planes(pool, J);
    if (need_slack) *need_slack = J.need_slack;
    *n_rec = J.n_rec;
    if (rc == isxenc::SEG_CAPACITY) {
        isx_set_error(J.need_slack > J.slack_groups ? "isx_encode_planes: a task needs more spare groups than slack_groups (see *need_slack)"
                                                    : "isx_encode_planes: the stream does not fit cap_rec records");
        return ISX_ERR_CAPACITY;
    }
    if (rc == isxenc::SEG_BAD_POS) { isx_set_error("a segment reaches beyond n_pos"); return ISX_ERR_ARG; }
    if (rc == isxenc::SEG_BAD_LEN) { isx_set_error("a segment's length is not in [1, 150]"); return ISX_ERR_ARG; }
    if (rc == isxenc::SEG_MM_RANGE) { isx_set_error("a segment has mm >= n_mm_bins"); return ISX_ERR_MM_RANGE; }
    return ISX_OK;
}

int isx_pack_read_planes(int64_t n_reads, const int64_t *ref_start, const int64_t *clip_lo, const int64_t *clip_hi,
                         const uint32_t *cigar, const int64_t *cigar_off, const char *seq, const uint8_t *qual, const int64_t *seq_off,
                         const uint32_t *pair, int32_t min_base_quality, int64_t cap_seg, uint32_t *seg_gpos,
                         uint8_t *seg_len, uint32_t *seg_pair, uint64_t *seg_planes, int64_t *n_seg)
// ... 43 lines not shown
```

### instrain_amd/csrc/seg_encode.h

```cpp
#pragma once
#include <stdint.h>

#include <functional>
#include <vector>

#include "../../include/instrain_amd.h"
#include "obs_encode.h"

#define ISX_SEG_GROUP 16
#define ISX_SEG_REC_WORDS 16
#define ISX_DREC_GROUP 32

namespace isxenc {

struct SegJob {
    isx_segs in{};
    std::function<void(int64_t first, int64_t count, uint32_t *gpos, uint8_t *len, uint8_t *mm, uint32_t *pair, uint32_t *bases)> produce;
    const uint32_t *gpos_all = nullptr;
    isx_read_planes in2{};
    std::function<void(int64_t first, int64_t count, uint32_t *gpos, uint8_t *len, uint8_t *mm, uint32_t *pair, uint64_t *planes)> produce_planes;
    const uint8_t *ref2 = nullptr, *refn = nullptr;
    int64_t n_seg = 0, n_pos = 0;
    int n_mm_bins = 1;
    bool want_pairs = false;
    uint32_t *rec = nullptr;
    uint32_t *gbase = nullptr;
    uint32_t *pair_out = nullptr;
    uint32_t *cmin = nullptr, *cmax = nullptr;
    uint8_t *cany = nullptr;
    int64_t cap_rec = 0;
    int64_t ring_groups = 0;
    std::function<void(int half)> wave_begin;
    std::function<void(int half, int64_t g0, int64_t g1)> wave_flush;
    const uint8_t *ref = nullptr;
    int64_t slack_groups = 1;
    int64_t need_slack = 0;
    std::vector<int64_t> task_need;
    const int64_t *task_groups = nullptr;
    int64_t n_pieces = 0;
    int64_t n_rec = 0;
    int64_t n_bases = 0;
    uint32_t max_pair = 0;
};

enum { SEG_OK = 0, SEG_CAPACITY = 1, SEG_MM_RANGE = 2, SEG_BAD_POS = 3, SEG_BAD_LEN = 4 };

int encode_segs(HostPool &pool, SegJob &job);
int encode_delta(HostPool &pool, SegJob &job);
int encode_planes(HostPool &pool, SegJob &job);
int64_t delta_groups_needed(HostPool &pool, const uint32_t *gpos, int64_t n, int64_t slack_groups);
int64_t seg_groups_needed(HostPool &pool, const uint32_t *gpos, int64_t n);
bool pack_ref_planes(HostPool &pool, const uint8_t *ref, int64_t n_pos, uint8_t *plane2, uint8_t *nplane);
void planes_from_words(const uint32_t *words, uint32_t len, uint64_t *planes);

// ... 2 lines not shown
```

### instrain_amd/csrc/seg_planes.inc

```

#if ISX_PLANES_VARIANT == 2
static inline __attribute__((always_inline)) __m256i ISX_DIFFERS_FN(const uint8_t *q, uint32_t sh, __m512i P)
{
    const __m512i lo = _mm512_maskz_loadu_epi64((__mmask8)0x1F, q), hi = _mm512_maskz_loadu_epi64((__mmask8)0x1F, q + 8);
    const __m512i r = _mm512_shrdv_epi64(lo, hi, _mm512_set1_epi64((long long)sh));
    const __m512i x = _mm512_xor_si512(r, P);
    const __m512i m = _mm512_or_si512(x, _mm512_srli_epi64(x, 1));
    const __m512i nib = _mm512_gf2p8affine_epi64_epi8(m, _mm512_set1_epi64((long long)0x0104104000000000ull), 0);
    const __m512i t = _mm512_or_si512(nib, _mm512_srli_epi16(nib, 4));
    return _mm512_cvtepi16_epi8(t);
}
#else
static inline __attribute__((always_inline)) void ISX_DIFFERS_FN(const uint8_t *q, uint32_t sh, const uint64_t *P, uint64_t d[3])
{
    uint64_t w[6];
    memcpy(w, q, 48);
    uint64_t e[5];
    for (int i = 0; i < 5; i++) {
        const uint64_t r = (w[i] >> sh) | ((w[i + 1] << 1) << (63 - sh));
        const uint64_t x = r ^ P[i];
        const uint64_t m = x | (x >> 1);
#if ISX_PLANES_VARIANT == 1
        e[i] = _pext_u64(m, 0x5555555555555555ull);
#else
// ... 35 lines not shown
#define ISX_TZ64(x) ((uint32_t)_tzcnt_u64(x))
#endif
static void ISX_PLANES_FN(SegJob &J, std::atomic<int> &err, PlaneTask &K)
{
    static const LenMasks LM;
    PlaneGroup G;
    G.g = K.ga;
    const uint8_t *const ref2 = J.ref2, *const refn = J.refn;
    const int64_t n_pos = J.n_pos;
    const int64_t safe_pos = n_pos - 200;
    const uint32_t *const gp = K.gp, *const pr = K.pr, *const ga = K.gpos_all;
    const uint8_t *const ln = K.ln;
    int64_t nb = 0, np = 0;
    uint32_t maxp = 0;
    auto place = [&](uint32_t start, uint32_t len, bool plain, bool &fill) __attribute__((always_inline)) -> uint32_t * {
        fill = plain && G.open >= 0;
        if (G.n) {
            const uint32_t nlo = std::min(G.lo, start), nhi = std::max(G.hi, start);
            if (__builtin_expect(nhi - nlo > SPAN || (!fill && G.n == ISX_DREC_GROUP), 0)) { ISX_CLOSE_FN(J, K, G); fill = false; }
        }
        if (!G.n) { G.lo = G.hi = start; G.last = start + len - 1; }
        else {
            if (__builtin_expect(start < G.lo, 0)) rebase_drecs(G, start);
            G.hi = std::max(G.hi, start); G.last = std::max(G.last, start + len - 1);
        }
        np++;
        if (fill) { uint32_t *o = G.rec[G.open] + 4; G.open = -1; return o; }
        uint32_t *o = G.rec[G.n];
        G.open = plain ? G.n : -1;
        G.n++;
        return o;
    };
    uint32_t hdr_hi = 0;
    auto add_full = [&](uint32_t start, uint32_t len, uint32_t pid, uint64_t s0, uint64_t s1, uint64_t s2, uint32_t exc) __attribute__((always_inline)) {
        bool fill;
        uint32_t *o = place(start, len, false, fill);
        const uint64_t v0 = (uint64_t)((start - G.lo) | (len << 16) | hdr_hi) | (s0 << 32), v1 = (s0 >> 32) | ((uint64_t)exc << 32);
        const uint64_t v3 = (s2 & 0xFFFFFFFFull) | ((uint64_t)pid << 32);
        memcpy(o, &v0, 8); memcpy(o + 2, &v1, 8); memcpy(o + 4, &s1, 8); memcpy(o + 6, &v3, 8);
    };
    auto add_plain = [&](uint32_t start, uint32_t len, uint32_t pid, uint32_t exc0, uint32_t exc1) __attribute__((always_inline)) {
        bool fill;
        uint32_t *o = place(start, len, true, fill);
        const uint64_t v0 = (uint64_t)((start - G.lo) | (len << 16) | hdr_hi | ISX_DREC_DUAL) | ((uint64_t)pid << 32), v1 = (uint64_t)exc0 | ((uint64_t)exc1 << 32);
        memcpy(o, &v0, 8); memcpy(o + 2, &v1, 8);
        if (!fill) {
            const uint64_t v2 = (uint64_t)ISX_DREC_DUAL, v3 = (uint64_t)ISX_DREC_NO_EXC | ((uint64_t)ISX_DREC_NO_EXC << 32);
            memcpy(o + 4, &v2, 8); memcpy(o + 6, &v3, 8);
        }
    };
#if ISX_PLANES_VARIANT == 2
    const __m256i rec_idx = _mm256_setr_epi32(8, 0, 1, 8, 2, 3, 4, 8);
#endif
    const bool mm_on = J.n_mm_bins > 1;
    const int64_t pf_end = K.e - PLANES_PREFETCH;
    for (int64_t s = K.a; s < K.e; s++) {
        const uint32_t L = ln[s], p = gp[s];
        const uint64_t *P = K.pl + (size_t)s * ISX_PLANE_WORDS;
        if (s < pf_end) {
            _mm_prefetch(reinterpret_cast<const char *>(P + (size_t)PLANES_PREFETCH * ISX_PLANE_WORDS), _MM_HINT_T0);
            _mm_prefetch(reinterpret_cast<const char *>(ref2 + (gp[s + PLANES_PREFETCH] >> 2) + 40), _MM_HINT_T0);
        }
        if (__builtin_expect(L == 0 || L > ISX_SEG_BASES, 0)) { err.store(SEG_BAD_LEN); return; }
        if (__builtin_expect((int64_t)p + (int64_t)L > n_pos || p != ga[s], 0)) { err.store(SEG_BAD_POS); return; }
        const uint32_t pid = pr ? pr[s] : 0u;
        maxp = pid > maxp ? pid : maxp;
        nb += L;
        const uint64_t *lm = LM.m[L];
        uint64_t s0, s1, s2, ex[3];
        bool n_marked = false;
        if (mm_on) {
            const uint32_t mv = K.mm ? K.mm[s] : 0u;
            if (__builtin_expect((int)mv >= J.n_mm_bins || mv > 127u, 0)) { err.store(SEG_MM_RANGE); return; }
            hdr_hi = mv << 24;
            n_marked = (P[7] >> 63) != 0;
        }
#if ISX_PLANES_VARIANT == 2
        __m256i skv = _mm256_setzero_si256();
        const bool in_regs = (int64_t)p < safe_pos && !refn && !n_marked;
        if (__builtin_expect(in_regs, 1)) {
            const __m512i Pv = _mm512_loadu_si512(P);
            const __m256i lmv = _mm256_loadu_si256(reinterpret_cast<const __m256i *>(lm));
            skv = _mm256_and_si256(_mm256_maskz_loadu_epi64((__mmask8)0x7, P + 5), lmv);
            const __m256i dv = ISX_DIFFERS_FN(ref2 + (p >> 2), (p & 3u) * 2u, Pv);
            const __m256i exv = _mm256_and_si256(dv, _mm256_xor_si256(skv, lmv));
            alignas(32) uint64_t t[8];
            _mm256_store_si256(reinterpret_cast<__m256i *>(t), skv);
// ... 23 lines not shown
                        bits160(bn, p & 7u, nn);
                    }
                    d[0] |= nn[0]; d[1] |= nn[1]; d[2] |= nn[2];
                }
            } else {
                alignas(64) uint8_t buf[64] = {0};
                const int64_t have2 = (n_pos + 3) / 4 - (int64_t)(p >> 2);
                memcpy(buf, ref2 + (p >> 2), (size_t)std::min<int64_t>(48, have2));
                ISX_DIFFERS_AT(buf, (p & 3u) * 2u);
                if (refn) {
                    uint8_t bn[32] = {0};
                    const int64_t haven = (n_pos + 7) / 8 - (int64_t)(p >> 3);
                    memcpy(bn, refn + (p >> 3), (size_t)std::min<int64_t>(32, haven));
                    uint64_t nn[3];
                    bits160(bn, p & 7u, nn);
                    d[0] |= nn[0]; d[1] |= nn[1]; d[2] |= nn[2];
                }
            }
#undef ISX_DIFFERS_AT
            ex[0] = d[0] & (lm[0] ^ s0); ex[1] = d[1] & (lm[1] ^ s1); ex[2] = d[2] & (lm[2] ^ s2);
            if (__builtin_expect(n_marked, 0)) {
                ex[0] |= (even_bits_portable(P[0]) | (even_bits_portable(P[1]) << 32)) & s0;
                ex[1] |= (even_bits_portable(P[2]) | (even_bits_portable(P[3]) << 32)) & s1;
                ex[2] |= even_bits_portable(P[4]) & s2;
            }
        }
        const bool plain = (s0 | s1 | s2) == 0;
        const uint32_t n_exc = (uint32_t)(__builtin_popcountll(ex[0]) + __builtin_popcountll(ex[1]) + __builtin_popcountll(ex[2]));
        if (__builtin_expect(n_exc <= 1, 1)) {
            const uint32_t t0 = ISX_TZ64(ex[0]), t1 = ISX_TZ64(ex[1]), t2 = ISX_TZ64(ex[2] | ((uint64_t)1 << 63));
            const uint32_t m0 = 0u - (uint32_t)(ex[0] == 0), m01 = m0 & (0u - (uint32_t)(ex[1] == 0));
            const uint32_t col = t0 + (t1 & m0) + (t2 & m01);
            const uint32_t code = (uint32_t)(P[col >> 5] >> (2 * (col & 31u))) & 3u;
            const uint32_t w0 = 0x3FFFFC00u | ((col | (code << 8) | (0u - (uint32_t)(n_exc == 0))) & 0x3FFu);
            if (__builtin_expect(plain, 0)) { add_plain(p, L, pid, w0, ISX_DREC_NO_EXC); continue; }
#if ISX_PLANES_VARIANT == 2
            if (__builtin_expect(in_regs, 1)) {
                bool fill;
                uint32_t *o = place(p, L, false, fill);
                __m256i v = _mm256_permutex2var_epi32(skv, rec_idx, _mm256_set1_epi32((int)w0));
                v = _mm256_mask_set1_epi32(v, (__mmask8)0x01, (int)((p - G.lo) | (L << 16) | hdr_hi));
                v = _mm256_mask_set1_epi32(v, (__mmask8)0x80, (int)pid);
                _mm256_store_si256(reinterpret_cast<__m256i *>(o), v);
                continue;
            }
#endif
            add_full(p, L, pid, s0, s1, s2, w0);
            continue;
        }
        const uint32_t max_exc = plain ? ISX_DREC_EXC : ISX_DREC_EXC_FULL;
        if (__builtin_expect(n_exc <= max_exc, 1)) {
            uint64_t fields = 0;
            for (uint32_t i = 0; i < n_exc; i++) {
                const int k = ex[0] ? 0 : (ex[1] ? 1 : 2);
                const uint32_t col = (uint32_t)(64 * k + __builtin_ctzll(ex[k]));
                ex[k] &= ex[k] - 1;
                const uint64_t code = (P[col >> 5] >> (2 * (col & 31u))) & 3u;
                fields |= ((uint64_t)col | (code << 8)) << (10 * i);
            }
            const uint64_t all = (fields | (0x0FFFFFFFFFFFFFFFull << (10 * n_exc))) & 0x0FFFFFFFFFFFFFFFull;
            const uint32_t w0 = (uint32_t)all & ISX_DREC_NO_EXC, w1 = (uint32_t)(all >> 30) & ISX_DREC_NO_EXC;
            if (plain) add_plain(p, L, pid, w0, w1);
            else add_full(p, L, pid, s0, s1, s2, w0);
            continue;
        }
        const uint64_t sk[3] = {s0, s1, s2};
        uint32_t b = 0;
        while (b < L) {
            uint32_t w[2] = {ISX_DREC_NO_EXC, ISX_DREC_NO_EXC};
            uint32_t nf = 0, end = L;
            for (int k = 0; k < 3; k++) {
                while (ex[k]) {
                    const uint32_t col = (uint32_t)(64 * k + __builtin_ctzll(ex[k]));
                    if (nf == max_exc) { end = col; goto cut; }
                    ex[k] &= ex[k] - 1;
                    const uint32_t code = (uint32_t)(P[col >> 5] >> (2 * (col & 31u))) & 3u;
                    const uint32_t f = ((col - b) & 0xFFu) | (code << 8);
                    const int wi = (int)(nf / 3), shf = 10 * (int)(nf % 3);
                    w[wi] = (w[wi] & ~(0x3FFu << shf)) | (f << shf);
                    nf++;
                }
            }
        cut:
            if (plain) add_plain(p + b, end - b, pid, w[0], w[1]);
            else if (b == 0 && end == L) add_full(p, L, pid, s0, s1, s2, w[0]);
            else {
                uint64_t msk[3];
                window160(sk, b, end - b, msk);
                add_full(p + b, end - b, pid, msk[0], msk[1], msk[2], w[0]);
            }
            b = end;
        }
    }
    ISX_CLOSE_FN(J, K, G);
    for (; G.g < K.ge; G.g++) {
        uint32_t *o = K.rec0 + (size_t)(G.g - K.g0) * (size_t)ISX_DREC_GROUP * ISX_DREC_WORDS;
        for (int r = 0; r < ISX_DREC_GROUP; r++) put_empty_drec(o + (size_t)r * ISX_DREC_WORDS);
        J.gbase[G.g] = 0; J.cmin[G.g] = 0xFFFFFFFFu; J.cmax[G.g] = 0; J.cany[G.g] = 0;
    }
    if (K.fast_store) _mm_sfence();
    K.used = G.used; K.np = np; K.nb = nb; K.maxp = maxp;
}
#undef ISX_TZ64
```

### instrain_amd/engine.py

```python
import ctypes as C
import os

import numpy as np

from . import _lib
from ._lib import (ENTRY_DT, LD_DT, OBS_DT, SNV_DT, BamInfo, BamParams, IsxError, Params, Sizes,
                   Timings, check)


def pack_obs(gpos, base, mm):
    o = np.empty(len(gpos), dtype=OBS_DT)
    o["gpos"] = gpos
    o["mm"] = mm
    o["base"] = base
    o["flags"] = 0
    return o


class SegBatch:

    def __init__(self, gpos, length, bases, mm=None, pair=None):
        self.gpos = np.ascontiguousarray(gpos, dtype=np.uint32)
        self.len = np.ascontiguousarray(length, dtype=np.uint8)
        self.bases = np.ascontiguousarray(bases, dtype=np.uint32).reshape(-1, _lib.SEG_WORDS)
# ... 709 lines not shown
    lib = _lib.load()
    if cap_rec is None:
        cap_rec = int(lib.isx_seg_records_needed(segs.gpos.ctypes.data if segs.n_seg else None, segs.n_seg, int(threads)))
    rec = np.empty((cap_rec, 16), dtype=np.uint32)
    gbase = np.empty(cap_rec // 16, dtype=np.uint32)
    pout = np.empty(cap_rec, dtype=np.uint32) if segs.pair is not None else None
    n_rec = C.c_int64(0)
    cs = segs.c()
    check(lib.isx_encode_segs_ring(C.byref(cs), int(n_pos), int(n_mm_bins), int(threads), int(cap_rec), int(ring_records), rec.ctypes.data,
                                   gbase.ctypes.data, pout.ctypes.data if pout is not None else None, C.byref(n_rec)))
    n = n_rec.value
    return rec[:n], gbase[:n // 16], (pout[:n] if pout is not None else None)


def encode_delta(segs, ref_codes, n_mm_bins=1, threads=1, slack_groups=1, cap_rec=None, ring_records=0, retry=True):
    lib = _lib.load()
    ref = np.ascontiguousarray(ref_codes, dtype=np.uint8)
    while True:
        cap = cap_rec if cap_rec is not None else int(lib.isx_delta_records_needed(segs.gpos.ctypes.data if segs.n_seg else None, segs.n_seg, int(threads), int(slack_groups)))
        rec = np.empty((cap, 8), dtype=np.uint32)
        gbase = np.empty(cap // 32, dtype=np.uint32)
        n_rec, need = C.c_int64(0), C.c_int64(0)
        cs = segs.c()
        rc = lib.isx_encode_delta(C.byref(cs), ref.ctypes.data, len(ref), int(n_mm_bins), int(threads), int(slack_groups), cap, int(ring_records),
                                  rec.ctypes.data, gbase.ctypes.data, None, C.byref(n_rec), C.byref(need))
        if rc == _lib.ERR_CAPACITY and retry and need.value > slack_groups and cap_rec is None:
            slack_groups = int(need.value)
            continue
        check(rc)
        n = n_rec.value
        return rec[:n], gbase[:n // 32], None, slack_groups


def encode_planes(reads, ref_planes, threads=1, slack_groups=1, cap_rec=None, ring_records=0, retry=True, n_mm_bins=1):
    lib = _lib.load()
    while True:
        cap = cap_rec if cap_rec is not None else int(lib.isx_delta_records_needed(reads.gpos.ctypes.data if reads.n_seg else None, reads.n_seg, int(threads), int(slack_groups)))
        rec = _aligned((cap, 8), np.uint32)
        gbase = np.empty(cap // 32, dtype=np.uint32)
        n_rec, need = C.c_int64(0), C.c_int64(0)
        cr, cf = reads.c(), ref_planes.c()
        rc = lib.isx_encode_planes_mm(C.byref(cr), C.byref(cf), ref_planes.n_pos, int(n_mm_bins), int(threads), int(slack_groups), cap, int(ring_records),
                                      rec.ctypes.data, gbase.ctypes.data, C.byref(n_rec), C.byref(need))
        if rc == _lib.ERR_CAPACITY and retry and need.value > slack_groups and cap_rec is None:
            slack_groups = int(need.value)
            continue
        check(rc)
        n = n_rec.value
        return rec[:n], gbase[:n // 32], None, slack_groups


def dense_cov(res, n_pos=None):
    if "cov16" in res:
        return res["cov16"]
    if "cov8" in res:
        cov = res["cov8"].astype(np.uint16)
    else:
        nib = res["cov4"]
        n_pos = 2 * len(nib) if n_pos is None else int(n_pos)
        cov = np.empty(2 * len(nib), dtype=np.uint16)
        cov[0::2] = nib & 15
        cov[1::2] = nib >> 4
        cov = cov[:n_pos]
        W = int(res["cov_window"])
        for k, w in enumerate(res["cov_row_win"].tolist()):
            lo = w * W
            hi = min(lo + W, n_pos)
            cov[lo:hi] = res["cov_rows"][k, :hi - lo]
    if "saturated" in res:
        cov[res["saturated"]["gpos"]] = np.minimum(res["saturated"]["coverage"], 65535)
    return cov


DREC_DUAL = 0x80000000
DREC_NO_EXC = 0x3FFFFFFF

# ... 374 lines not shown
```

Before: 169.7.

## Embed reference codes in delta records instead of uploading reference plane

Measured after the change: 152.0. 0.896x the previous value.

```diff
diff --git a/include/instrain_amd.h b/include/instrain_amd.h
--- a/include/instrain_amd.h
+++ b/include/instrain_amd.h
@@ -55,6 +55,8 @@
 #define ISX_LAYOUT_MM_DELTA_RECORDS 32
 
 #define ISX_LAYOUT_NO_STRIPES 64
+
+#define ISX_LAYOUT_REF_PLANE 128
 
 typedef struct {
     uint32_t gpos;
@@ -326,6 +328,11 @@
 #define ISX_DREC_EXC_FULL 3
 #define ISX_DREC_DUAL 0x80000000u
 #define ISX_DREC_NO_EXC 0x3FFFFFFFu
+#define ISX_DREC_EXC_REF 5
+#define ISX_DREC_REF_SHIFT0 30
+#define ISX_DREC_REF_SHIFT1 24
+#define ISX_DREC_REF_SHIFT2 26
+#define ISX_DREC_REF_SHIFT4 28
 
 typedef struct {
     int64_t n_seg;
@@ -382,6 +389,8 @@
                       int64_t cap_rec, int64_t ring_records, uint32_t *rec, uint32_t *gbase, int64_t *n_rec, int64_t *need_slack);
 int isx_encode_planes_mm(const isx_read_planes *reads, const isx_ref_planes *ref, int64_t n_pos, int32_t n_mm_bins, int32_t host_threads, int32_t slack_groups,
                          int64_t cap_rec, int64_t ring_records, uint32_t *rec, uint32_t *gbase, int64_t *n_rec, int64_t *need_slack);
+int isx_encode_planes_ref(const isx_read_planes *reads, const isx_ref_planes *ref, int64_t n_pos, int32_t host_threads, int32_t slack_groups,
+                          int64_t cap_rec, int64_t ring_records, uint32_t *rec, uint32_t *gbase, int64_t *n_rec, int64_t *need_slack);
 
 int isx_count_read_segs(int64_t n_reads, const uint32_t *cigar, const int64_t *cigar_off, const int64_t *ref_start,
                         const int64_t *clip_lo, const int64_t *clip_hi, int64_t *n_seg);
diff --git a/instrain_amd/_lib.py b/instrain_amd/_lib.py
--- a/instrain_amd/_lib.py
+++ b/instrain_amd/_lib.py
@@ -52,6 +52,7 @@
 PLANE_WORDS = 8
 LAYOUT_MM_ENTRIES = 16
 LAYOUT_MM_DELTA_RECORDS = 32
+LAYOUT_REF_PLANE = 128
 ABI_VERSION = 5
 
 
@@ -157,7 +158,7 @@
            "isx_batch_summarize", "isx_batch_summarize_genomes", "isx_compare_coverage", "isx_compare_scaffolds", "isx_compare_fetch_snps",
            "isx_genes_create", "isx_genes_destroy", "isx_genes_sites", "isx_batch_profile_genes", "isx_genes_profile_snvs",
            "isx_pipe_create", "isx_pipe_destroy", "isx_pipe_submit", "isx_pipe_submit_reads", "isx_pipe_stage_reads", "isx_pipe_submit_wire", "isx_wire_bytes", "isx_wire_free", "isx_wire_keep_reference", "isx_pipe_submit_bam", "isx_encode_segs", "isx_encode_segs_ring", "isx_seg_records_needed", "isx_encode_delta", "isx_delta_records_needed", "isx_count_read_segs", "isx_pack_reads", "isx_pipe_collect", "isx_pipe_release", "isx_pipe_fetch_entries", "isx_pipe_fetch_entries_shrunk", "isx_levels_expand", "isx_encode_obs", "isx_encode_obs_ring",
-           "isx_pack_ref_planes", "isx_planes_from_segs", "isx_pack_read_planes", "isx_pipe_submit_planes", "isx_pipe_stage_planes", "isx_encode_planes", "isx_encode_planes_mm", "isx_pipe_set_reference_budget", "isx_host_register", "isx_host_unregister",
+           "isx_pack_ref_planes", "isx_planes_from_segs", "isx_pack_read_planes", "isx_pipe_submit_planes", "isx_pipe_stage_planes", "isx_encode_planes", "isx_encode_planes_mm", "isx_encode_planes_ref", "isx_pipe_set_reference_budget", "isx_host_register", "isx_host_unregister",
            "isx_bgzf_index", "isx_bgzf_inflate_device", "isx_bgzf_inflate_host", "isx_bgzf_inflate_fast",
            "isx_bam_open", "isx_bam_close", "isx_bam_close_wait", "isx_bam_set_threads", "isx_bam_ref", "isx_bam_set_priority_reads", "isx_bam_scan", "isx_bam_scan_part",
            "isx_bam_insert_sizes", "isx_bam_set_wanted_refs", "isx_bam_pair_keys", "isx_bam_set_cross_names", "isx_bam_filter_insert_sizes", "isx_bam_filter", "isx_bam_set_r2m", "isx_bam_r2m", "isx_bam_drop_names", "isx_bam_batch_pair_names", "isx_bam_set_mm_cap", "isx_bam_mm_levels", "isx_bam_set_mm_levels", "isx_bam_ref_counts",
@@ -280,6 +281,7 @@
     lib.isx_pipe_stage_planes.argtypes = [vp, i64, C.POINTER(RefPlanes), i32, vp, C.POINTER(ReadPlanes), C.POINTER(vp)]
     lib.isx_encode_planes.argtypes = [C.POINTER(ReadPlanes), C.POINTER(RefPlanes), i64, i32, i32, i64, i64, vp, vp, C.POINTER(i64), C.POINTER(i64)]
     lib.isx_encode_planes_mm.argtypes = [C.POINTER(ReadPlanes), C.POINTER(RefPlanes), i64, i32, i32, i32, i64, i64, vp, vp, C.POINTER(i64), C.POINTER(i64)]
+    lib.isx_encode_planes_ref.argtypes = [C.POINTER(ReadPlanes), C.POINTER(RefPlanes), i64, i32, i32, i64, i64, vp, vp, C.POINTER(i64), C.POINTER(i64)]
     lib.isx_bam_ref.argtypes = [vp, i32, C.POINTER(C.c_char_p), C.POINTER(i64), C.POINTER(i64)]
     lib.isx_bam_copy.argtypes = [vp, vp, vp, vp, vp]
     lib.isx_bam_view.argtypes = [vp, C.POINTER(vp), C.POINTER(vp)]
diff --git a/instrain_amd/csrc/isx_api.hip b/instrain_amd/csrc/isx_api.hip
--- a/instrain_amd/csrc/isx_api.hip
+++ b/instrain_amd/csrc/isx_api.hip
@@ -1271,6 +1271,11 @@
     if (getenv("ISX_NO_COUNTS")) { a.counts = nullptr; if (atoi(getenv("ISX_NO_COUNTS")) > 1) a.clon = nullptr; }
 #endif
     a.stripe = (b->drec && b->packed && b->M == 1 && !a.counts && !(b->prm.layout & ISX_LAYOUT_NO_STRIPES)) ? 1 : 0;
+    if (b->ref_inline && !(b->drec && b->packed && b->M == 1 && !a.counts)) {
+        isx_set_error("internal: records with reference codes need packed reference-delta rows without a count table");
+        return ISX_ERR_STATE;
+    }
+    a.ref_inline = b->ref_inline ? 1 : 0;
     a.seed_lo = (uint32_t)b->prm.seed; a.seed_hi = (uint32_t)(b->prm.seed >> 32);
     a.entries = b->d_entries; a.slab = b->slab; a.cap_ovf = (uint32_t)b->cap_ovf;
     a.ovf0 = (uint64_t)b->n_win * b->slab; a.win_nent = b->d_win_nent;
diff --git a/instrain_amd/csrc/isx_batch.h b/instrain_amd/csrc/isx_batch.h
--- a/instrain_amd/csrc/isx_batch.h
+++ b/instrain_amd/csrc/isx_batch.h
@@ -35,6 +35,7 @@
     bool arena = false;
     bool segs = false;
     bool drec = false;
+    bool ref_inline = false;
     uint64_t n_rec = 0;
     uint64_t n_pairs = 0;
     int32_t n_splits = 0;
diff --git a/instrain_amd/csrc/isx_internal.h b/instrain_amd/csrc/isx_internal.h
--- a/instrain_amd/csrc/isx_internal.h
+++ b/instrain_amd/csrc/isx_internal.h
@@ -211,6 +211,7 @@
     uint32_t *lev_win_off;
     uint32_t cap_lev;
     int32_t lev_mask_bytes, lev_cov_bytes;
+    int32_t ref_inline;
 };
 
 void launch_pileup(const PileupArgs &a, int block, size_t lds, int grid, int packed, hipStream_t s, hipEvent_t ev_start,
diff --git a/instrain_amd/csrc/isx_pileup.hip b/instrain_amd/csrc/isx_pileup.hip
--- a/instrain_amd/csrc/isx_pileup.hip
+++ b/instrain_amd/csrc/isx_pileup.hip
@@ -447,9 +447,10 @@
     return raw;
 }
 
+template <bool ONE_BIN = false, bool RX = false>
 __device__ __forceinline__ void allele_pass_delta(const PileupArgs &a, uint32_t lo16, uint32_t hi16, uint32_t w0, int W,
                                                   const uint8_t *maskl, uint32_t *slabc, uint32_t ao_base, uint32_t *stage,
-                                                  int tid, int nthr)
+                                                  int tid, int nthr, const uint8_t *refl = nullptr)
 {
     const int lane = tid & 63;
     uint32_t *st = stage + (tid >> 6) * 128;
@@ -518,7 +519,7 @@
                     if ((x & 0xFFu) == col) code = x >> 8;
                     if ((y & 0xFFu) == col) code = y >> 8;
                 }
-                if (has && code == 8u) code = ref_at(a, w0 + rel);
+                if (has && code == 8u) code = RX ? (uint32_t)refl[rel] : (uint32_t)ref_at(a, w0 + rel);
                 const bool cand = has && code < 4u && ((maskl[rel] >> code) & 1u);
                 const uint64_t bal = __ballot(cand);
                 if (bal == 0) continue;
@@ -527,7 +528,7 @@
                 if (cand) {
                     const uint32_t at = nst + __builtin_amdgcn_mbcnt_hi((uint32_t)(bal >> 32), __builtin_amdgcn_mbcnt_lo((uint32_t)bal, 0u));
                     st[2 * at] = dual ? i : (i & ~1u);
-                    st[2 * at + 1] = rel | (code << 16) | (dual ? 0u : 1u << 20) | (((hdr >> 24) & 0x7Fu) << 24);
+                    st[2 * at + 1] = rel | (code << 16) | (dual ? 0u : 1u << 20) | (ONE_BIN ? 0u : ((hdr >> 24) & 0x7Fu) << 24);
                 }
                 nst += n;
             }
@@ -546,7 +547,7 @@
 #else
 #define ISX_TS(k) do { } while (0)
 #endif
-template <bool LINKAGE, int FMT, bool PK16 = false>
+template <bool LINKAGE, int FMT, bool PK16 = false, bool RX = false>
 __global__ void __launch_bounds__(1024, ISX_LB_WAVES) k_pileup_dense(const PileupArgs a_kernarg)
 {
     extern __shared__ __attribute__((aligned(16))) uint32_t lds[];
@@ -573,6 +574,7 @@
     uint32_t *dlt = PKL ? queue : lds + a.dlt_off;
     uint32_t *wtot = lds + a.dlt_off + (PKL ? 0 : S);
     uint8_t *refl = reinterpret_cast<uint8_t *>(wtot + 16);
+    static_assert(!RX || (DREC && PK16), "reference codes beside the exceptions: packed reference-delta rows only");
     auto ld4 = [&](int p, uint32_t *c) {
         if (PKL) {
             const uint32_t x = cnt[p], y = cnt[S + p];
@@ -659,11 +661,20 @@
                 uint4 *zm = reinterpret_cast<uint4 *>(maskl);
                 for (int i = tid; i < (W >> 4); i += nthr) zm[i] = make_uint4(0, 0, 0, 0);
             }
+            if (RX) {
+                uint4 *zr = reinterpret_cast<uint4 *>(refl);
+                for (int i = tid; i < (W >> 4); i += nthr) zr[i] = make_uint4(0, 0, 0, 0);
+            }
             if (tid < S_N) scratch[tid] = 0;
         }
         uint32_t ref4 = 0x04040404u, ref4b = 0x04040404u;
         uint32_t ref4n = 0, ref4bn = 0;
-        if (PKL) {
+        if (RX) {
+            if (a.ref_n) {
+                if (4 * tid < W && w0 + 4u * (uint32_t)tid < a.n_pos) ref4n = a.ref_n[(w0 + 4u * (uint32_t)tid) >> 3];
+                if (4 * (tid + nthr) < W && w0 + 4u * (uint32_t)(tid + nthr) < a.n_pos) ref4bn = a.ref_n[(w0 + 4u * (uint32_t)(tid + nthr)) >> 3];
+            }
+        } else if (PKL) {
             if (4 * tid < W) ref4_raw(a, w0 + 4u * (uint32_t)tid, ref4, ref4n);
             if (4 * (tid + nthr) < W) ref4_raw(a, w0 + 4u * (uint32_t)(tid + nthr), ref4b, ref4bn);
         } else if (DREC && 4 * tid < W) ref4 = ref4_at(a, w0 + 4u * (uint32_t)tid);
@@ -723,6 +734,8 @@
                     if (off < len && rel < uW) {
                         if (PKL) atomicAdd(&cnt[__umul24(code >> 1, (uint32_t)S) + rel], 1u << (16 * (code & 1u)));
                         else atomicAdd(&cnt[__umul24(code, (uint32_t)S) + rel], 1u);
+                        if (RX) refl[rel] = (uint8_t)(((f % 3 == 0) ? ex >> ISX_DREC_REF_SHIFT0
+                                                                    : hdr >> (f == 1 ? ISX_DREC_REF_SHIFT1 : (f == 2 ? ISX_DREC_REF_SHIFT2 : ISX_DREC_REF_SHIFT4))) & 3u);
                     }
                 }
                 return;
@@ -831,11 +844,19 @@
 #ifdef ISX_TUNING
         if (ablate_acc == 0xDEADBEEFu) cnt[dummy] = ablate_acc;
 #endif
-        if (PKL) {
+        if (PKL && !RX) {
             if (4 * tid < W) reinterpret_cast<uint32_t *>(refl)[tid] = ref4_expand(a, w0 + 4u * (uint32_t)tid, ref4, ref4n);
             if (4 * (tid + nthr) < W) reinterpret_cast<uint32_t *>(refl)[tid + nthr] = ref4_expand(a, w0 + 4u * (uint32_t)(tid + nthr), ref4b, ref4bn);
         }
         __syncthreads();
+        if (RX && (ref4n | ref4bn)) {
+            const uint32_t nb = (ref4n >> ((w0 + 4u * (uint32_t)tid) & 4u)) & 0xFu, nbb = (ref4bn >> ((w0 + 4u * (uint32_t)(tid + nthr)) & 4u)) & 0xFu;
+#pragma unroll
+            for (int k = 0; k < 4; k++) {
+                if ((nb >> k) & 1u) refl[4 * tid + k] = 4;
+                if ((nbb >> k) & 1u) refl[4 * (tid + nthr) + k] = 4;
+            }
+        }
         ISX_TS(2);
         ISX_ARGS_FRESH();
 
@@ -1287,7 +1308,7 @@
             if (ok && nao) {
                 __syncthreads();
                 if (SEGS) allele_pass_segs(a, cur_lo, cur_hi, w0, W, maskl, slabc, ao_base, lds + a.stage_off, tid, nthr);
-                else if (DREC) allele_pass_delta(a, cur_lo, cur_hi, w0, W, maskl, slabc, ao_base, lds + a.stage_off, tid, nthr);
+                else if (DREC) allele_pass_delta<true, RX>(a, cur_lo, cur_hi, w0, W, maskl, slabc, ao_base, lds + a.stage_off, tid, nthr, refl);
                 else allele_pass(a, cur_lo << (RSH - 1), cur_hi << (RSH - 1), w0, W, maskl, slabc, ao_base, lds + a.stage_off, tid, nthr);
             }
             ISX_TS(9);
@@ -2109,6 +2130,7 @@
     } else {
         const bool link = a.enable_linkage != 0;
         if (a.seg) { if (link) launch_one(k_pileup_dense<true, 64>, a, l); else launch_one(k_pileup_dense<false, 64>, a, l); return; }
+        if (a.drec && packed && a.ref_inline) { if (link) launch_one(k_pileup_dense<true, 32, true, true>, a, l); else launch_one(k_pileup_dense<false, 32, true, true>, a, l); return; }
         if (a.drec && packed) { if (link) launch_one(k_pileup_dense<true, 32, true>, a, l); else launch_one(k_pileup_dense<false, 32, true>, a, l); return; }
         if (a.drec) { if (link) launch_one(k_pileup_dense<true, 32>, a, l); else launch_one(k_pileup_dense<false, 32>, a, l); return; }
 #ifndef ISX_NO_PK16
diff --git a/instrain_amd/csrc/isx_pipe.hip b/instrain_amd/csrc/isx_pipe.hip
--- a/instrain_amd/csrc/isx_pipe.hip
+++ b/instrain_amd/csrc/isx_pipe.hip
@@ -125,7 +125,7 @@
 {
     const size_t b2 = ((size_t)n_pos + 3) / 4, bn = ((size_t)n_pos + 7) / 8;
     const size_t piece = (size_t)1 << 20;
-    const int t2 = (int)((b2 + piece - 1) / piece), tn = rp->nplane ? (int)((bn + piece - 1) / piece) : 0;
+    const int t2 = plane2 ? (int)((b2 + piece - 1) / piece) : 0, tn = rp->nplane ? (int)((bn + piece - 1) / piece) : 0;
     std::atomic<int> any{0};
     pool.run(t2 + tn, [&](int t) {
         if (t < t2) { const size_t a = (size_t)t * piece; memcpy(plane2 + a, rp->plane2 + a, std::min(piece, b2 - a)); return; }
@@ -214,6 +214,7 @@
     int rb = 2;
     bool segs = false;
     bool drec = false;
+    bool ref_codes = false;
     int64_t dslack = 1;
     uint32_t G = ISX_GROUP16;
     size_t snv_prefix = 0;
@@ -251,6 +252,20 @@
     std::condition_variable cv_stage;
     int64_t next_promise = 0;
     bool stage_stop = false;
+    struct TailJob {
+        int64_t ticket = -1, n_pos = 0, n_rec = 0, n_bases = 0, n_seg = 0;
+        int32_t n_splits = 0;
+        uint32_t max_pair = 0;
+        bool planes_in = false, ref_codes = false, early_rec = false, early_ref = false;
+        const uint8_t *plane2 = nullptr;
+        uint8_t *resident = nullptr;
+        size_t ring_bytes = 0;
+        double t0 = 0, t_front = 0, ref_ms = 0, rec_ms = 0;
+    };
+    std::thread tailer;
+    std::deque<TailJob> tail_q;
+    std::condition_variable cv_tail;
+    bool tail_stop = false;
 };
 
 static int bounce_d2h(isx_pipe *p, void *hdst, const void *dsrc, size_t bytes, hipStream_t st)
@@ -287,6 +302,11 @@
         { std::lock_guard<std::mutex> lk(p->mu); p->stage_stop = true; }
         p->cv_stage.notify_all();
         p->stager.join();
+    }
+    if (p->tailer.joinable()) {
+        { std::lock_guard<std::mutex> lk(p->mu); p->tail_stop = true; }
+        p->cv_tail.notify_all();
+        p->tailer.join();
     }
     if (p->finisher.joinable()) {
         { std::lock_guard<std::mutex> lk(p->mu); p->stop = true; }
@@ -753,7 +773,7 @@
 
 static void drain_stager(isx_pipe *p)
 {
-    if (!p->stager.joinable()) return;
+    if (!p->stager.joinable() && !p->tailer.joinable()) return;
     std::unique_lock<std::mutex> lk(p->mu);
     p->cv_done.wait(lk, [&] { return p->next_ticket == p->next_promise; });
 }
@@ -779,6 +799,7 @@
     p->ctx = c; p->prm = *prm; p->pp = *pp;
     p->segs = pp->max_segs > 0;
     p->drec = p->segs && !(prm->layout & ISX_LAYOUT_SEG64_RECORDS) && (prm->n_mm_bins == 1 || (prm->layout & ISX_LAYOUT_MM_DELTA_RECORDS));
+    p->ref_codes = p->drec && prm->n_mm_bins == 1 && pp->lean_output != 0 && !pp->want_counts && !(prm->layout & ISX_LAYOUT_REF_PLANE);
     p->rb = p->segs ? (p->drec ? 32 : 64) : ((prm->n_mm_bins == 1 && !(prm->layout & ISX_LAYOUT_NO_SHORT_RECORDS)) ? 2 : 4);
     p->G = p->segs ? (p->drec ? ISX_DREC_GROUP : ISX_SEG_GROUP) : (p->rb == 2 ? ISX_GROUP16 : ISX_GROUP);
     const double js = pp->jump_slack > 0 ? pp->jump_slack : 0.25;
@@ -963,15 +984,17 @@
     return ISX_OK;
 }
 
-static int slot_acquire(isx_pipe *p, const char *who, Slot **out)
-{
-    Slot &s = p->slots[(size_t)(p->next_ticket % (int64_t)p->slots.size())];
+static int slot_acquire(isx_pipe *p, const char *who, Slot **out, bool ahead = false)
+{
+    Slot *s = nullptr;
     {
         std::lock_guard<std::mutex> lk(p->mu);
-        if (s.state != 0) { isx_set_error(std::string(who) + ": every slot is in use (collect + release the oldest batch first)"); return ISX_ERR_STATE; }
+        const int64_t t = ahead ? p->next_promise : p->next_ticket, n = (int64_t)p->slots.size();
+        s = &p->slots[(size_t)(t % n)];
+        if (s->state != 0 || (ahead && t - n >= p->next_ticket)) { isx_set_error(std::string(who) + ": every slot is in use (collect + release the oldest batch first)"); return ISX_ERR_STATE; }
     }
     HIP_TRY(hipSetDevice(p->ctx->device));
-    *out = &s;
+    *out = s;
     return ISX_OK;
 }
 
@@ -1101,6 +1124,7 @@
 
 struct RefStage {
     bool early = false;
+    const uint8_t *plane2 = nullptr;
     uint8_t *resident = nullptr;
     double host_ms = 0.0;
 };
@@ -1158,6 +1182,30 @@
     return ISX_OK;
 }
 
+static int stage_reference_codes(isx_pipe *p, Slot &s, int64_t n_pos, const isx_ref_planes *rp, isxenc::SegJob &J, RefStage *out)
+{
+    const bool ring = p->ring_half > 0;
+    const double t_r = now_ms();
+    const size_t b2 = ((size_t)n_pos + 3) / 4, bn = ((size_t)n_pos + 7) / 8;
+    hipStream_t st = H2D(p, s);
+    uint8_t *h2 = s.h_in + s.off_ref, *hn = h2 + ref2_bytes(n_pos);
+    const uint8_t *np = rp->nplane;
+    if (isx_host_is_registered(rp->plane2, b2) && (!rp->nplane || isx_host_is_registered(rp->nplane, bn))) {
+        s.ref_has_n = rp->nplane && plane_any(*p->pool, rp->nplane, bn);
+        out->plane2 = rp->plane2;
+    } else {
+        s.ref_has_n = copy_ref_planes(*p->pool, rp, n_pos, h2, hn);
+        out->plane2 = h2; np = hn;
+    }
+    J.ref2 = out->plane2; J.refn = s.ref_has_n ? np : nullptr; J.ref_codes = true;
+    out->host_ms = now_ms() - t_r;
+    if (!ring) HIP_TRY(hipEventRecord(s.ev_h2d0, st));
+    if (s.ref_has_n) HIP_TRY(hipMemcpyAsync(s.d_in + s.off_ref + ref2_bytes(n_pos), np, bn, hipMemcpyHostToDevice, st));
+    if (!ring) HIP_TRY(hipEventRecord(s.ev_h2da, st));
+    out->early = true;
+    return ISX_OK;
+}
+
 static int submit_common(isx_pipe *p, int64_t n_pos, const uint8_t *ref, int32_t n_splits, const int64_t *split_bounds,
                          int64_t n_obs, isxenc::EncodeJob &J, int64_t *ticket)
 {
@@ -1169,6 +1217,7 @@
     if ((rc = slot_acquire(p, who, &slot)) != ISX_OK) return rc;
     Slot &s = *slot;
     isx_batch *b = s.b;
+    b->ref_inline = false;
     const bool linkage = p->prm.enable_linkage != 0;
 
     const double t0 = now_ms();
@@ -1286,7 +1335,9 @@
     if ((rc = slot_acquire(p, who, &slot)) != ISX_OK) return rc;
     Slot &s = *slot;
     isx_batch *b = s.b;
+    b->ref_inline = false;
     const bool linkage = p->prm.enable_linkage != 0;
+    const bool ref_codes = planes_in && rp && p->ref_codes;
 
     const double t0 = now_ms();
     J.n_pos = n_pos; J.n_mm_bins = b->M;
@@ -1301,7 +1352,7 @@
     RefStage rs;
     if (planes_in) {
         if (!p->drec) { isx_set_error("bit-plane reads need a pipe whose batches travel as reference-delta records (one mm bin, or ISX_LAYOUT_MM_DELTA_RECORDS)"); return ISX_ERR_STATE; }
-        if ((rc = stage_reference(p, s, n_pos, ref, rp, J, &rs)) != ISX_OK) return rc;
+        if ((rc = ref_codes ? stage_reference_codes(p, s, n_pos, rp, J, &rs) : stage_reference(p, s, n_pos, ref, rp, J, &rs)) != ISX_OK) return rc;
     }
     if (p->drec) J.ref = ref;
     const int erc = encode_reads(p, s, J, planes_in, feed);
@@ -1328,6 +1379,7 @@
     b->n_pos = n_pos; b->n_obs = J.n_bases; b->n_splits = n_splits; b->n_rec = (uint64_t)J.n_rec;
     b->n_pairs = (uint64_t)J.max_pair + 1;
     if ((rc = slot_choose_windows(p, s, p->G, true)) != ISX_OK) return rc;
+    b->ref_inline = ref_codes && b->packed != 0;
     if ((rc = slot_shape_pass(p, s)) != ISX_OK) return rc;
     slot_bind_inputs(p, s, rs.resident);
     s.encode_ms = (float)(now_ms() - t0);
@@ -1337,7 +1389,7 @@
     const double t_q0 = now_ms();
 
     if (!ring && !rs.early) HIP_TRY(hipEventRecord(s.ev_h2d0, H2D(p, s)));
-    const size_t ref_bytes = ref2_bytes(n_pos) + (s.ref_has_n ? refn_bytes(n_pos) : 0);
+    const size_t ref_bytes = (b->ref_inline ? 0 : ref2_bytes(n_pos)) + (s.ref_has_n ? refn_bytes(n_pos) : 0);
     const size_t head = (size_t)(n_splits + 1) * sizeof(int64_t) + s.win.size() * sizeof(uint2) + ref_bytes;
     const size_t gb_bytes = (size_t)(b->n_rec / p->G) * sizeof(uint32_t), rec_bytes = (size_t)b->n_rec * (size_t)p->rb;
     if (s.off_win - s.off_bounds < ((size_t)1 << 20)) {
@@ -1347,6 +1399,7 @@
         HIP_TRY(hipMemcpyAsync(s.d_in + s.off_win, s.h_in + s.off_win, s.win.size() * sizeof(uint2), hipMemcpyHostToDevice, H2D(p, s)));
     }
     if (!rs.early) HIP_TRY(hipMemcpyAsync(s.d_in + s.off_ref, s.h_in + s.off_ref, ref_bytes, hipMemcpyHostToDevice, H2D(p, s)));
+    if (ref_codes && !b->ref_inline) HIP_TRY(hipMemcpyAsync(s.d_in + s.off_ref, rs.plane2, ((size_t)n_pos + 3) / 4, hipMemcpyHostToDevice, H2D(p, s)));
     if (!early_rec) HIP_TRY(hipMemcpyAsync(s.d_in + s.off_gbase, s.h_in + s.off_gbase, gb_bytes, hipMemcpyHostToDevice, H2D(p, s)));
     if (ring) { if (feed.bytes != rec_bytes) { isx_set_error("internal: the staging ring did not carry the whole stream"); return ISX_ERR_STATE; } }
     else if (!early_rec) HIP_TRY(hipMemcpyAsync(s.d_in + s.off_rec, s.h_in + s.off_rec, rec_bytes, hipMemcpyHostToDevice, H2D(p, s)));
@@ -1374,6 +1427,7 @@
     uint64_t n_pairs = 0;
     int W = 0, packed = 0;
     bool ref_has_n = false;
+    bool ref_inline = false;
     float stage_ms = 0.f;
     int encode_passes = 1;
     uint8_t *d_ref = nullptr;
@@ -1388,6 +1442,7 @@
     *out = nullptr;
     if (!p->segs) { isx_set_error("isx_pipe_stage_reads: not a read-level pipe (isx_pipe_params.max_segs == 0)"); return ISX_ERR_STATE; }
     const bool linkage = p->prm.enable_linkage != 0;
+    const bool ref_codes = reads && rp && p->ref_codes;
     if (linkage && segs->n_seg && !segs->pair) { isx_set_error("linkage needs the pair array"); return ISX_ERR_ARG; }
     int rc;
     if ((rc = check_capacity(p, "isx_pipe_stage_reads", n_pos, segs->n_seg, p->pp.max_segs, n_splits)) != ISX_OK) return rc;
@@ -1434,7 +1489,11 @@
         J.cmin = cmin.data(); J.cmax = cmax.data(); J.cany = cany.data();
         J.cap_rec = cap;
         int erc;
-        if (reads) {
+        if (reads && ref_codes) {
+            uint8_t *hn = w->h + w->o_ref + ref2_bytes(n_pos);
+            w->ref_has_n = copy_ref_planes(*p->pool, rp, n_pos, nullptr, hn);
+            J.ref2 = rp->plane2; J.refn = w->ref_has_n ? hn : nullptr; J.ref_codes = true;
+        } else if (reads) {
             uint8_t *h2 = w->h + w->o_ref, *hn = h2 + ref2_bytes(n_pos);
             w->ref_has_n = rp ? copy_ref_planes(*p->pool, rp, n_pos, h2, hn) : isxenc::pack_ref_planes(*p->pool, ref, n_pos, h2, hn);
             J.ref2 = h2; J.refn = w->ref_has_n ? hn : nullptr;
@@ -1465,6 +1524,10 @@
         if (w->win_bytes > ((size_t)n_pos / 64 + 2) * sizeof(uint2) || win.size() > (size_t)p->pp.max_pos / 64 + 2) { isx_set_error("internal: window directory larger than its region"); return ISX_ERR_STATE; }
         memcpy(w->h + w->o_win, win.data(), w->win_bytes);
     }
+    if (ref_codes) {
+        w->ref_inline = w->packed != 0;
+        if (!w->ref_inline) { isx_ref_planes only2 = *rp; only2.nplane = nullptr; (void)copy_ref_planes(*p->pool, &only2, n_pos, w->h + w->o_ref, nullptr); }
+    }
     w->stage_ms = (float)(now_ms() - t0);
     *out = w.release();
     return ISX_OK;
@@ -1504,7 +1567,7 @@
 int isx_wire_keep_reference(isx_pipe *p, isx_wire *w)
 {
     if (!p || !w || w->pipe != p) { isx_set_error("isx_wire_keep_reference: bad argument"); return ISX_ERR_ARG; }
-    if (w->d_ref || !w->ref_bytes) return ISX_OK;
+    if (w->d_ref || !w->ref_bytes || w->ref_inline) return ISX_OK;
     isx_ctx *c = p->ctx;
     HIP_TRY(hipSetDevice(c->device));
     uint8_t *d = nullptr;
@@ -1515,7 +1578,8 @@
     return ISX_OK;
 }
 
-int64_t isx_wire_bytes(const isx_wire *w) { return w ? (int64_t)(w->bounds_bytes + w->win_bytes + (w->d_ref ? 0 : w->ref_bytes) + w->gbase_bytes + w->pairs_bytes + w->rec_bytes) : 0; }
+static size_t wire_ref_bytes(const isx_wire *w) { return w->ref_inline ? (w->ref_has_n ? refn_bytes(w->n_pos) : 0) : (w->d_ref ? 0 : w->ref_bytes); }
+int64_t isx_wire_bytes(const isx_wire *w) { return w ? (int64_t)(w->bounds_bytes + w->win_bytes + wire_ref_bytes(w) + w->gbase_bytes + w->pairs_bytes + w->rec_bytes) : 0; }
 
 int isx_pipe_submit_wire(isx_pipe *p, const isx_wire *w, int64_t *ticket)
 {
@@ -1532,13 +1596,16 @@
     b->n_pairs = w->n_pairs;
     s.ref_has_n = w->ref_has_n;
     b->packed = w->packed; b->W = w->W;
+    b->ref_inline = w->ref_inline;
     b->n_win = (int)(w->win_bytes / sizeof(uint2));
     if ((rc = slot_shape_pass(p, s)) != ISX_OK) return rc;
     slot_bind_inputs(p, s, w->d_ref);
     HIP_TRY(hipEventRecord(s.ev_h2d0, H2D(p, s)));
     HIP_TRY(hipMemcpyAsync(s.d_in + s.off_bounds, w->h + w->o_bounds, w->bounds_bytes, hipMemcpyHostToDevice, H2D(p, s)));
     HIP_TRY(hipMemcpyAsync(s.d_in + s.off_win, w->h + w->o_win, w->win_bytes, hipMemcpyHostToDevice, H2D(p, s)));
-    if (!w->d_ref) HIP_TRY(hipMemcpyAsync(s.d_in + s.off_ref, w->h + w->o_ref, w->ref_bytes, hipMemcpyHostToDevice, H2D(p, s)));
+    if (w->ref_inline) {
+        if (w->ref_has_n) HIP_TRY(hipMemcpyAsync(s.d_in + s.off_ref + ref2_bytes(w->n_pos), w->h + w->o_ref + ref2_bytes(w->n_pos), refn_bytes(w->n_pos), hipMemcpyHostToDevice, H2D(p, s)));
+    } else if (!w->d_ref) HIP_TRY(hipMemcpyAsync(s.d_in + s.off_ref, w->h + w->o_ref, w->ref_bytes, hipMemcpyHostToDevice, H2D(p, s)));
     HIP_TRY(hipMemcpyAsync(s.d_in + s.off_gbase, w->h + w->o_gbase, w->gbase_bytes, hipMemcpyHostToDevice, H2D(p, s)));
     if (w->pairs_bytes) HIP_TRY(hipMemcpyAsync(s.d_in + s.off_pairs, w->h + w->o_pairs, w->pairs_bytes, hipMemcpyHostToDevice, H2D(p, s)));
     HIP_TRY(hipMemcpyAsync(s.d_in + s.off_rec, w->h + w->o_rec, w->rec_bytes, hipMemcpyHostToDevice, H2D(p, s)));
diff --git a/instrain_amd/csrc/seg_encode.cpp b/instrain_amd/csrc/seg_encode.cpp
--- a/instrain_amd/csrc/seg_encode.cpp
+++ b/instrain_amd/csrc/seg_encode.cpp
@@ -1054,8 +1054,23 @@
     return isx_encode_planes_mm(reads, ref, n_pos, 1, host_threads, slack_groups, cap_rec, ring_records, rec, gbase, n_rec, need_slack);
 }
 
+static int encode_planes_host(const isx_read_planes *reads, const isx_ref_planes *ref, int64_t n_pos, int32_t n_mm_bins, bool ref_codes, int32_t host_threads,
+                              int32_t slack_groups, int64_t cap_rec, int64_t ring_records, uint32_t *rec, uint32_t *gbase, int64_t *n_rec, int64_t *need_slack);
+
 int isx_encode_planes_mm(const isx_read_planes *reads, const isx_ref_planes *ref, int64_t n_pos, int32_t n_mm_bins, int32_t host_threads, int32_t slack_groups,
                          int64_t cap_rec, int64_t ring_records, uint32_t *rec, uint32_t *gbase, int64_t *n_rec, int64_t *need_slack)
+{
+    return encode_planes_host(reads, ref, n_pos, n_mm_bins, false, host_threads, slack_groups, cap_rec, ring_records, rec, gbase, n_rec, need_slack);
+}
+
+int isx_encode_planes_ref(const isx_read_planes *reads, const isx_ref_planes *ref, int64_t n_pos, int32_t host_threads, int32_t slack_groups,
+                          int64_t cap_rec, int64_t ring_records, uint32_t *rec, uint32_t *gbase, int64_t *n_rec, int64_t *need_slack)
+{
+    return encode_planes_host(reads, ref, n_pos, 1, true, host_threads, slack_groups, cap_rec, ring_records, rec, gbase, n_rec, need_slack);
+}
+
+static int encode_planes_host(const isx_read_planes *reads, const isx_ref_planes *ref, int64_t n_pos, int32_t n_mm_bins, bool ref_codes, int32_t host_threads,
+                              int32_t slack_groups, int64_t cap_rec, int64_t ring_records, uint32_t *rec, uint32_t *gbase, int64_t *n_rec, int64_t *need_slack)
 {
     if (n_mm_bins < 1 || n_mm_bins > 128) { isx_set_error("isx_encode_planes: n_mm_bins must be in [1, 128]"); return ISX_ERR_ARG; }
     if (!reads || !ref || !ref->plane2 || !rec || !gbase || !n_rec || reads->n_seg < 0 || cap_rec < ISX_DREC_GROUP || (cap_rec % ISX_DREC_GROUP) || n_pos <= 0 ||
@@ -1071,6 +1086,7 @@
     isxenc::SegJob J;
     J.in2 = *reads; J.n_seg = reads->n_seg; J.n_pos = n_pos; J.n_mm_bins = n_mm_bins;
     J.ref2 = ref->plane2; J.refn = ref->nplane; J.slack_groups = std::max(1, slack_groups);
+    J.ref_codes = ref_codes;
     J.rec = rec; J.gbase = gbase; J.pair_out = nullptr;
     J.cmin = cmin.data(); J.cmax = cmax.data(); J.cany = cany.data(); J.cap_rec = cap_rec;
     if (ring_records) {
diff --git a/instrain_amd/csrc/seg_encode.h b/instrain_amd/csrc/seg_encode.h
--- a/instrain_amd/csrc/seg_encode.h
+++ b/instrain_amd/csrc/seg_encode.h
@@ -20,6 +20,7 @@
     isx_read_planes in2{};
     std::function<void(int64_t first, int64_t count, uint32_t *gpos, uint8_t *len, uint8_t *mm, uint32_t *pair, uint64_t *planes)> produce_planes;
     const uint8_t *ref2 = nullptr, *refn = nullptr;
+    bool ref_codes = false;
     int64_t n_seg = 0, n_pos = 0;
     int n_mm_bins = 1;
     bool want_pairs = false;
diff --git a/instrain_amd/csrc/seg_planes.inc b/instrain_amd/csrc/seg_planes.inc
--- a/instrain_amd/csrc/seg_planes.inc
+++ b/instrain_amd/csrc/seg_planes.inc
@@ -91,17 +91,17 @@
         return o;
     };
     uint32_t hdr_hi = 0;
-    auto add_full = [&](uint32_t start, uint32_t len, uint32_t pid, uint64_t s0, uint64_t s1, uint64_t s2, uint32_t exc) __attribute__((always_inline)) {
+    auto add_full = [&](uint32_t start, uint32_t len, uint32_t pid, uint64_t s0, uint64_t s1, uint64_t s2, uint32_t exc, uint32_t hx) __attribute__((always_inline)) {
         bool fill;
         uint32_t *o = place(start, len, false, fill);
-        const uint64_t v0 = (uint64_t)((start - G.lo) | (len << 16) | hdr_hi) | (s0 << 32), v1 = (s0 >> 32) | ((uint64_t)exc << 32);
+        const uint64_t v0 = (uint64_t)((start - G.lo) | (len << 16) | hdr_hi | hx) | (s0 << 32), v1 = (s0 >> 32) | ((uint64_t)exc << 32);
         const uint64_t v3 = (s2 & 0xFFFFFFFFull) | ((uint64_t)pid << 32);
         memcpy(o, &v0, 8); memcpy(o + 2, &v1, 8); memcpy(o + 4, &s1, 8); memcpy(o + 6, &v3, 8);
     };
-    auto add_plain = [&](uint32_t start, uint32_t len, uint32_t pid, uint32_t exc0, uint32_t exc1) __attribute__((always_inline)) {
+    auto add_plain = [&](uint32_t start, uint32_t len, uint32_t pid, uint32_t exc0, uint32_t exc1, uint32_t hx) __attribute__((always_inline)) {
         bool fill;
         uint32_t *o = place(start, len, true, fill);
-        const uint64_t v0 = (uint64_t)((start - G.lo) | (len << 16) | hdr_hi | ISX_DREC_DUAL) | ((uint64_t)pid << 32), v1 = (uint64_t)exc0 | ((uint64_t)exc1 << 32);
+        const uint64_t v0 = (uint64_t)((start - G.lo) | (len << 16) | hdr_hi | hx | ISX_DREC_DUAL) | ((uint64_t)pid << 32), v1 = (uint64_t)exc0 | ((uint64_t)exc1 << 32);
         memcpy(o, &v0, 8); memcpy(o + 2, &v1, 8);
         if (!fill) {
             const uint64_t v2 = (uint64_t)ISX_DREC_DUAL, v3 = (uint64_t)ISX_DREC_NO_EXC | ((uint64_t)ISX_DREC_NO_EXC << 32);
@@ -112,6 +112,9 @@
     const __m256i rec_idx = _mm256_setr_epi32(8, 0, 1, 8, 2, 3, 4, 8);
 #endif
     const bool mm_on = J.n_mm_bins > 1;
+    const bool rx = J.ref_codes && !mm_on;
+    const uint32_t exc_plain = rx ? ISX_DREC_EXC_REF : ISX_DREC_EXC;
+    const uint32_t last_pos = (uint32_t)(n_pos - 1);
     const int64_t pf_end = K.e - PLANES_PREFETCH;
     for (int64_t s = K.a; s < K.e; s++) {
         const uint32_t L = ln[s], p = gp[s];
@@ -201,8 +204,12 @@
             const uint32_t m0 = 0u - (uint32_t)(ex[0] == 0), m01 = m0 & (0u - (uint32_t)(ex[1] == 0));
             const uint32_t col = t0 + (t1 & m0) + (t2 & m01);
             const uint32_t code = (uint32_t)(P[col >> 5] >> (2 * (col & 31u))) & 3u;
-            const uint32_t w0 = 0x3FFFFC00u | ((col | (code << 8) | (0u - (uint32_t)(n_exc == 0))) & 0x3FFu);
-            if (__builtin_expect(plain, 0)) { add_plain(p, L, pid, w0, ISX_DREC_NO_EXC); continue; }
+            uint32_t w0 = 0x3FFFFC00u | ((col | (code << 8) | (0u - (uint32_t)(n_exc == 0))) & 0x3FFu);
+            if (rx) {
+                const uint32_t at = std::min(p + col, last_pos);
+                w0 |= (((uint32_t)ref2[at >> 2] >> (2 * (at & 3u))) & 3u & (0u - (uint32_t)(n_exc != 0))) << ISX_DREC_REF_SHIFT0;
+            }
+            if (__builtin_expect(plain, 0)) { add_plain(p, L, pid, w0, ISX_DREC_NO_EXC, 0u); continue; }
 #if ISX_PLANES_VARIANT == 2
             if (__builtin_expect(in_regs, 1)) {
                 bool fill;
@@ -214,30 +221,34 @@
                 continue;
             }
 #endif
-            add_full(p, L, pid, s0, s1, s2, w0);
+            add_full(p, L, pid, s0, s1, s2, w0, 0u);
             continue;
         }
-        const uint32_t max_exc = plain ? ISX_DREC_EXC : ISX_DREC_EXC_FULL;
+        const uint32_t max_exc = plain ? exc_plain : ISX_DREC_EXC_FULL;
         if (__builtin_expect(n_exc <= max_exc, 1)) {
             uint64_t fields = 0;
+            uint32_t rcodes = 0;
             for (uint32_t i = 0; i < n_exc; i++) {
                 const int k = ex[0] ? 0 : (ex[1] ? 1 : 2);
                 const uint32_t col = (uint32_t)(64 * k + __builtin_ctzll(ex[k]));
                 ex[k] &= ex[k] - 1;
                 const uint64_t code = (P[col >> 5] >> (2 * (col & 31u))) & 3u;
                 fields |= ((uint64_t)col | (code << 8)) << (10 * i);
+                if (rx) rcodes |= (((uint32_t)ref2[(p + col) >> 2] >> (2 * ((p + col) & 3u))) & 3u) << (2 * i);
             }
             const uint64_t all = (fields | (0x0FFFFFFFFFFFFFFFull << (10 * n_exc))) & 0x0FFFFFFFFFFFFFFFull;
-            const uint32_t w0 = (uint32_t)all & ISX_DREC_NO_EXC, w1 = (uint32_t)(all >> 30) & ISX_DREC_NO_EXC;
-            if (plain) add_plain(p, L, pid, w0, w1);
-            else add_full(p, L, pid, s0, s1, s2, w0);
+            const uint32_t w0 = ((uint32_t)all & ISX_DREC_NO_EXC) | ((rcodes & 3u) << ISX_DREC_REF_SHIFT0);
+            const uint32_t w1 = ((uint32_t)(all >> 30) & ISX_DREC_NO_EXC) | (((rcodes >> 6) & 3u) << ISX_DREC_REF_SHIFT0);
+            const uint32_t hx = (((rcodes >> 2) & 0xFu) << ISX_DREC_REF_SHIFT1) | (((rcodes >> 8) & 3u) << ISX_DREC_REF_SHIFT4);
+            if (plain) add_plain(p, L, pid, w0, w1, hx);
+            else add_full(p, L, pid, s0, s1, s2, w0, hx);
             continue;
         }
         const uint64_t sk[3] = {s0, s1, s2};
         uint32_t b = 0;
         while (b < L) {
             uint32_t w[2] = {ISX_DREC_NO_EXC, ISX_DREC_NO_EXC};
-            uint32_t nf = 0, end = L;
+            uint32_t nf = 0, end = L, hx = 0;
             for (int k = 0; k < 3; k++) {
                 while (ex[k]) {
                     const uint32_t col = (uint32_t)(64 * k + __builtin_ctzll(ex[k]));
@@ -247,16 +258,21 @@
                     const uint32_t f = ((col - b) & 0xFFu) | (code << 8);
                     const int wi = (int)(nf / 3), shf = 10 * (int)(nf % 3);
                     w[wi] = (w[wi] & ~(0x3FFu << shf)) | (f << shf);
+                    if (rx) {
+                        const uint32_t rc = ((uint32_t)ref2[(p + col) >> 2] >> (2 * ((p + col) & 3u))) & 3u;
+                        if (nf % 3 == 0) w[wi] |= rc << ISX_DREC_REF_SHIFT0;
+                        else hx |= rc << (nf == 1 ? ISX_DREC_REF_SHIFT1 : (nf == 2 ? ISX_DREC_REF_SHIFT2 : ISX_DREC_REF_SHIFT4));
+                    }
                     nf++;
                 }
             }
         cut:
-            if (plain) add_plain(p + b, end - b, pid, w[0], w[1]);
-            else if (b == 0 && end == L) add_full(p, L, pid, s0, s1, s2, w[0]);
+            if (plain) add_plain(p + b, end - b, pid, w[0], w[1], hx);
+            else if (b == 0 && end == L) add_full(p, L, pid, s0, s1, s2, w[0], hx);
             else {
                 uint64_t msk[3];
                 window160(sk, b, end - b, msk);
-                add_full(p + b, end - b, pid, msk[0], msk[1], msk[2], w[0]);
+                add_full(p + b, end - b, pid, msk[0], msk[1], msk[2], w[0], hx);
             }
             b = end;
         }
diff --git a/instrain_amd/engine.py b/instrain_amd/engine.py
--- a/instrain_amd/engine.py
+++ b/instrain_amd/engine.py
@@ -765,7 +765,7 @@
         return rec[:n], gbase[:n // 32], None, slack_groups
 
 
-def encode_planes(reads, ref_planes, threads=1, slack_groups=1, cap_rec=None, ring_records=0, retry=True, n_mm_bins=1):
+def encode_planes(reads, ref_planes, threads=1, slack_groups=1, cap_rec=None, ring_records=0, retry=True, n_mm_bins=1, ref_codes=False):
     lib = _lib.load()
     while True:
         cap = cap_rec if cap_rec is not None else int(lib.isx_delta_records_needed(reads.gpos.ctypes.data if reads.n_seg else None, reads.n_seg, int(threads), int(slack_groups)))
@@ -773,8 +773,12 @@
         gbase = np.empty(cap // 32, dtype=np.uint32)
         n_rec, need = C.c_int64(0), C.c_int64(0)
         cr, cf = reads.c(), ref_planes.c()
-        rc = lib.isx_encode_planes_mm(C.byref(cr), C.byref(cf), ref_planes.n_pos, int(n_mm_bins), int(threads), int(slack_groups), cap, int(ring_records),
-                                      rec.ctypes.data, gbase.ctypes.data, C.byref(n_rec), C.byref(need))
+        if ref_codes:
+            rc = lib.isx_encode_planes_ref(C.byref(cr), C.byref(cf), ref_planes.n_pos, int(threads), int(slack_groups), cap, int(ring_records),
+                                           rec.ctypes.data, gbase.ctypes.data, C.byref(n_rec), C.byref(need))
+        else:
+            rc = lib.isx_encode_planes_mm(C.byref(cr), C.byref(cf), ref_planes.n_pos, int(n_mm_bins), int(threads), int(slack_groups), cap, int(ring_records),
+                                          rec.ctypes.data, gbase.ctypes.data, C.byref(n_rec), C.byref(need))
         if rc == _lib.ERR_CAPACITY and retry and need.value > slack_groups and cap_rec is None:
             slack_groups = int(need.value)
             continue
```
